# klindsay28/NK_ocn_tracer_jacobian_precond

Hardware: AMD Instinct MI355X
Metric: precond_solve_throughput_1deg_ocean_jacobian (higher is better)
Workload: dtype f64

## Files before the change

### include/nkp.h

```cpp
#ifndef NKP_H
#define NKP_H

#include <stdint.h>

#ifdef __cplusplus
extern "C" {
#endif

#define NKP_VERSION 1

typedef struct nkp_solver nkp_solver;

enum nkp_precond {
   NKP_PRECOND_NONE = 0,
   NKP_PRECOND_COLUMN_JACOBI = 1,
   NKP_PRECOND_MULTILEVEL = 3
};

enum nkp_krylov { NKP_KRYLOV_FGMRES = 0, NKP_KRYLOV_BICGSTAB = 1 };

enum {
   NKP_OK = 0,
   NKP_NOT_CONVERGED = 1,
   NKP_BREAKDOWN = 2,
   NKP_OK_BERR = 3,
   NKP_EINVAL = -1,
   NKP_ENOMEM = -2,
   NKP_EDEVICE = -3,
   NKP_ESINGULAR = -4,
   NKP_ECOMM = -5
};

typedef struct nkp_tuning {
   int struct_size;
   int ml_split;
   int ml_pocket;
   int ml_big_from;
   int ml_coarsest_rows;
   int ml_dense_max;
   double ml_theta;
   double ml_tau;
   int64_t ml_device_min;
   int ml_smooth_coarse;
   int ml_coarse_from;
   int ml_gamma_from, ml_gamma_to;
   int ml_f32;
   int ml_host_inverse;
   int ml_fused;
   int ml_fused_max_cols;
   int ml_wave_fused;
   int ml_coarsest_sweeps;
   int64_t ml_tail_rows;
   double ml_omega;
   int col_ldsres;
   int col_stream;
   int col_stream_min;
   int col_stream_gw;
   int col_wave_max;
   int col_w3;
   int col_group;
   int col_pipe_min;
   int col_ldsres_early;
   int col_ldsres_packed;
   int spmv_variant;
   int spmv_compress;
   int spmv_pipe_min;
   int spmv_run;
   int spmv_wgs;
   int rhs_batch;
   int precond_steps;
   int equil;
   int dist_overlap;
   int dist_ras;
   int force_dist;
   int setup_threads;
   int plan_times;
   int ml_drop_intertracer;
   int dist_one_reduce;
   int ml_huge_from;
   int col_ldsres_min;
   int col_sort_groups;
   int batch_spmv_rows;
   int dist_ras_rings;
   int ml_diag;
   int spmv_diag;
   int ml_lane_fused;
} nkp_tuning;

int nkp_default_tuning (nkp_tuning *t);

typedef struct nkp_options {
   int struct_size;
   int precond;
   int krylov;
   int restart;
   int max_iters;
   double rtol;
   double atol;
   int device;
   int verbose;
   int rank;
   int reorth;
   int ml_levels;
   int ml_smooth;
   int basis_f32;
   int precond_steps;
   int equil;
   int reserved[4];
   const int32_t *col_i;
   const int32_t *col_j;
   const int32_t *col_t;
   const nkp_tuning *tuning;
} nkp_options;

int nkp_default_options (nkp_options *opt);

int nkp_device_count (void);

int nkp_create (nkp_solver **out, const nkp_options *opt, int64_t n, int64_t nnz,
                const int32_t *rowptr, const int32_t *colind, const double *val,
                const int32_t *blk_start, int64_t nblk, int coupled_tracer_cnt);

int nkp_create64 (nkp_solver **out, const nkp_options *opt, int64_t n, const int64_t *rowptr ,
                  const int32_t *colind, const double *val, const int32_t *blk_start, int64_t nblk, int coupled_tracer_cnt);

int nkp_solve (nkp_solver *s, double *b_in_x_out, int nrhs, int64_t ldb,
               double *berr, int *iters, double *relres);

int nkp_solve_batch_device (nkp_solver *s, int nrhs, const void *d_B, void *d_X, int64_t ldb, double *berr, int *iters, double *relres);

int nkp_solve_device (nkp_solver *s, const void *d_b, void *d_x, int use_guess,
                      double *berr, int *iters, double *relres);

int nkp_spmv (nkp_solver *s, const double *x, double *y);
int nkp_spmv_device (nkp_solver *s, const void *d_x, void *d_y);

int nkp_precond_apply (nkp_solver *s, const double *r, double *z);

int nkp_multi_dot (nkp_solver *s, const double *V, int64_t ld, int k, const double *w, double *out);

int nkp_time_kernel (nkp_solver *s, int which, int arg, int reps, double *avg_ms);

int64_t nkp_get_int (nkp_solver *s, const char *key);

#define NKP_REFACTOR_REBUILD 1
int nkp_refactor (nkp_solver *s, const double *val, int flags);
int nkp_refactor_device (nkp_solver *s, const void *d_val, int flags);

int nkp_refactor_dist (nkp_solver *s, const double *val_loc, int flags);
int nkp_refactor_dist_device (nkp_solver *s, const void *d_val_loc, int flags);

int nkp_set_stream (nkp_solver *s, void *hip_stream);

void nkp_destroy (nkp_solver *s);

const char *nkp_last_error (void);


typedef struct nkp_comm_ops {
   void *ctx;
   int rank, nranks;
   int (*allreduce) (void *ctx, void *dev_buf, int count, int op, void *hip_stream);
   int (*alltoallv) (void *ctx, const void *dev_send, const int *send_counts, void *dev_recv, const int *recv_counts, void *hip_stream);
   int (*alltoallv_i32_host) (void *ctx, const int32_t *send, const int *send_counts, int32_t *recv, const int *recv_counts);
   int (*allgather_i64_host) (void *ctx, int64_t mine, int64_t *all );
} nkp_comm_ops;

int nkp_comm_unique_id (void *id128);
int nkp_comm_rccl_init (nkp_comm_ops *ops, const void *id128, int rank, int nranks);
void nkp_comm_rccl_free (nkp_comm_ops *ops);
int nkp_comm_file_init (nkp_comm_ops *ops, const char *dir, int rank, int nranks);
void nkp_comm_file_free (nkp_comm_ops *ops);

int nkp_create_dist (nkp_solver **out, const nkp_options *opt, int64_t n_global, int64_t fst_row,
                     int64_t m_loc, int64_t nnz_loc, const int32_t *rowptr_loc,
                     const int32_t *colind_glob, const double *val,
                     const int32_t *blk_start_loc, int64_t nblk_loc, int coupled_tracer_cnt,
                     const nkp_comm_ops *comm);

int nkp_cell_major_order (int64_t nblk, const int32_t *blk_start, int cnt, int32_t *perm, int32_t *blk_start_new,
                          int32_t *col_t, int32_t *col_src);
int nkp_permuted_rows (int64_t n, const int32_t *rowptr, const int32_t *colind, const double *val, const int32_t *perm,
                       const int32_t *inv, int64_t r0, int64_t r1, int32_t *rowptr_loc, int32_t *colind_loc, double *val_loc);

int nkp_clone (nkp_solver *src, nkp_solver **out);

int nkp_transpose (nkp_solver *s, nkp_solver **out);

int nkp_transpose_dist (nkp_solver *s, nkp_solver **out);

int nkp_value_gradient_device (nkp_solver *s, int nrhs, const void *d_lambda, const void *d_x, int64_t ld, double alpha, int accumulate, void *d_gval);
int nkp_value_gradient (nkp_solver *s, int nrhs, const double *lambda, const double *x, int64_t ld, double alpha, int accumulate, double *gval);

int nkp_values_product_device (nkp_solver *s, int nrhs, const void *d_val, const void *d_x, int64_t ldx, double alpha, int accumulate, void *d_y, int64_t ldy);
int nkp_values_product (nkp_solver *s, int nrhs, const double *val, const double *x, int64_t ldx, double alpha, int accumulate, double *y, int64_t ldy);

int nkp_solve_tangent_device (nkp_solver *s, int nrhs, const void *d_dval, const void *d_x, int64_t ldx, const void *d_db, void *d_dx, int64_t ld,
                              double *berr, int *iters, double *relres);

int nkp_set_device (int device);

int nkp_gather_root (nkp_solver *s, const double *x_loc, double *x_global);

typedef struct nkp_dist_plan nkp_dist_plan;
int nkp_dist_overlap_plan_host (nkp_dist_plan **out, const nkp_options *opt, int64_t n_global, int64_t fst_row, int64_t m_loc,
                                int64_t nnz_loc, const int32_t *rowptr_loc, const int32_t *colind_glob, const double *val,
                                const int32_t *blk_start_loc, int64_t nblk_loc, int coupled_tracer_cnt, const nkp_comm_ops *comm);
int64_t nkp_dist_plan_size (const nkp_dist_plan *p, const char *what);
int nkp_dist_plan_copy (const nkp_dist_plan *p, const char *what, void *dst);
void nkp_dist_plan_free (nkp_dist_plan *p);

int nkp_dist_plan_host (int64_t m_loc, int64_t nnz_loc, const int32_t *rowptr_loc, const int32_t *colind_glob,
                        int rank, int nranks, const int64_t *starts, int32_t *colind_ext, int32_t *halo_rows,
                        int64_t *n_halo, int32_t *need_counts);

int64_t nkp_ml_level_array (nkp_solver *s, int level, const char *what, void *dst, int64_t capacity_bytes);

int64_t nkp_matrix_array (nkp_solver *s, const char *what, void *dst, int64_t capacity_bytes);

int nkp_ml_plan_host (int64_t n, const int32_t *rowptr, const int32_t *colind, const double *val, const int32_t *blk_start,
                      int64_t nblk, const int32_t *col_i, const int32_t *col_j, int coupled_tracer_cnt, int max_levels,
                      int coarsest_rows, int64_t capacity, int *n_levels, int64_t *rows, int32_t *cmap, int32_t *col_of);

#ifdef __cplusplus
}
#endif
#endif
```

### nk_ocn_tracer_jacobian_precond_amd/csrc/blas1.hip

```cpp
#include "nkp_dev.h"

#include <stdint.h>

#define B1_THREADS 256

__device__ __forceinline__ double wave_sum (double v)
{
#pragma unroll
   for (int off = NKP_WAVE / 2; off > 0; off >>= 1) v += __shfl_down (v, off);
   return v;
}

__device__ __forceinline__ double block_sum (double v, double *sh )
{
   v = wave_sum (v);
   const int lane = threadIdx.x & (NKP_WAVE - 1), wv = threadIdx.x / NKP_WAVE;
   __syncthreads ();
   if (lane == 0) sh[wv] = v;
   __syncthreads ();
   double s = 0.0;
   if (threadIdx.x == 0) {
#pragma unroll
      for (int w = 0; w < B1_THREADS / NKP_WAVE; w++) s += sh[w];
   }
   return s;
}

static inline int red_grid (int64_t n)
{
   int64_t g = (n + 2 * B1_THREADS - 1) / (2 * B1_THREADS);
   if (g < 1) g = 1;
   if (g > NKP_RED_BLOCKS) g = NKP_RED_BLOCKS;
   return (int) g;
}

template <class VT, class VT2>
__device__ __forceinline__ void multi_dot_body (const VT *__restrict__ V, int64_t ld, int k, const double *__restrict__ w,
                                                int64_t n, double *__restrict__ partial, double *sh)
{
   const int chunk = blockIdx.y;
   const int j0 = chunk * NKP_DOT_CHUNK;
   const int kc = (k - j0) < NKP_DOT_CHUNK ? (k - j0) : NKP_DOT_CHUNK;
   const VT *Vc = V + (int64_t) j0 * ld;
   double acc[NKP_DOT_CHUNK];
#pragma unroll
   for (int c = 0; c < NKP_DOT_CHUNK; c++) acc[c] = 0.0;
   double accw = 0.0;
   const int64_t stride = (int64_t) gridDim.x * B1_THREADS * 2;
   for (int64_t i = ((int64_t) blockIdx.x * B1_THREADS + threadIdx.x) * 2; i < n; i += stride) {
      if (i + 1 < n) {
         const double2 w2 = *reinterpret_cast<const double2 *> (w + i);
         accw += w2.x * w2.x + w2.y * w2.y;
#pragma unroll
         for (int c = 0; c < NKP_DOT_CHUNK; c++)
            if (c < kc) {
               const VT2 v2 = *reinterpret_cast<const VT2 *> (Vc + (int64_t) c * ld + i);
               acc[c] += (double) v2.x * w2.x + (double) v2.y * w2.y;
            }
      } else {
         const double w1 = w[i];
         accw += w1 * w1;
#pragma unroll
         for (int c = 0; c < NKP_DOT_CHUNK; c++)
            if (c < kc) acc[c] += (double) Vc[(int64_t) c * ld + i] * w1;
      }
   }
   double *out = partial + ((int64_t) chunk * gridDim.x + blockIdx.x) * (NKP_DOT_CHUNK + 1);
#pragma unroll
   for (int c = 0; c < NKP_DOT_CHUNK; c++) {
      const double s = block_sum (acc[c], sh);
      if (threadIdx.x == 0) out[c] = s;
   }
   const double sw = block_sum (accw, sh);
   if (threadIdx.x == 0) out[NKP_DOT_CHUNK] = sw;
}

template <class VT, class VT2>
__global__ __launch_bounds__ (B1_THREADS)
void multi_dot_kernel (const VT *__restrict__ V, int64_t ld, int k, const double *__restrict__ w,
                       int64_t n, double *__restrict__ partial)
{
   __shared__ double sh[B1_THREADS / NKP_WAVE];
   multi_dot_body<VT, VT2> (V, ld, k, w, n, partial, sh);
}

__global__ __launch_bounds__ (B1_THREADS)
void multi_dot_group_kernel (GsGroup G, int64_t ld, int k, int64_t n)
{
   __shared__ double sh[B1_THREADS / NKP_WAVE];
   const int r = blockIdx.z;
   multi_dot_body<double, double2> (G.V[r], ld, k, G.w[r], n, G.partial[r], sh);
}

__device__ __forceinline__ void multi_dot_finish_body (const double *__restrict__ partial, int nblk, int k, double *__restrict__ out)
{
   const int j = blockIdx.x;
   const int chunk = (j < k) ? j / NKP_DOT_CHUNK : 0;
   const int c = (j < k) ? j % NKP_DOT_CHUNK : NKP_DOT_CHUNK;
   const double *p = partial + (int64_t) chunk * nblk * (NKP_DOT_CHUNK + 1) + c;
   double s = 0.0;
   for (int b = threadIdx.x; b < nblk; b += NKP_WAVE) s += p[(int64_t) b * (NKP_DOT_CHUNK + 1)];
   s = wave_sum (s);
   if (threadIdx.x == 0) out[j] = s;
}

__global__ __launch_bounds__ (NKP_WAVE)
void multi_dot_finish_kernel (const double *__restrict__ partial, int nblk, int k, double *__restrict__ out)
{
   multi_dot_finish_body (partial, nblk, k, out);
}

__global__ __launch_bounds__ (NKP_WAVE)
void multi_dot_finish_group_kernel (GsGroup G, int nblk, int k, double *__restrict__ msg)
{
   multi_dot_finish_body (G.partial[blockIdx.y], nblk, k, msg + (int64_t) blockIdx.y * (k + 1));
}

void launch_multi_dot (const void *V, int v_f32, int64_t ld, int k, const double *w, int64_t n, double *partial, double *out, hipStream_t st)
{
   const int g = red_grid (n);
   const int nchunk = k > 0 ? (k + NKP_DOT_CHUNK - 1) / NKP_DOT_CHUNK : 1;
   if (v_f32) hipLaunchKernelGGL ((multi_dot_kernel<float, float2>), dim3 (g, nchunk), dim3 (B1_THREADS), 0, st, (const float *) V, ld, k, w, n, partial);
   else hipLaunchKernelGGL ((multi_dot_kernel<double, double2>), dim3 (g, nchunk), dim3 (B1_THREADS), 0, st, (const double *) V, ld, k, w, n, partial);
   hipLaunchKernelGGL (multi_dot_finish_kernel, dim3 (k + 1), dim3 (NKP_WAVE), 0, st, partial, g, k, out);
}

void launch_multi_dot_group (int R, const GsGroup &G, int64_t ld, int k, int64_t n, double *msg, hipStream_t st)
{
   if (R <= 0) return;
   const int g = red_grid (n);
   const int nchunk = k > 0 ? (k + NKP_DOT_CHUNK - 1) / NKP_DOT_CHUNK : 1;
   hipLaunchKernelGGL (multi_dot_group_kernel, dim3 (g, nchunk, R), dim3 (B1_THREADS), 0, st, G, ld, k, n);
   hipLaunchKernelGGL (multi_dot_finish_group_kernel, dim3 (k + 1, R), dim3 (NKP_WAVE), 0, st, G, g, k, msg);
}

#define B1_MAX_K NKP_MAX_K
template <class VT, class VT2>
__device__ __forceinline__ void update_w_body (const VT *__restrict__ V, int64_t ld, int k, const double *__restrict__ h,
                                               double *__restrict__ w, int64_t n, double *__restrict__ partial, double sign, double *hs, double *sh)
{
   for (int j = threadIdx.x; j < k; j += B1_THREADS) hs[j] = sign * h[j];
   __syncthreads ();
   double nrm = 0.0;
   const int64_t stride = (int64_t) gridDim.x * B1_THREADS * 2;
   for (int64_t i = ((int64_t) blockIdx.x * B1_THREADS + threadIdx.x) * 2; i < n; i += stride) {
      if (i + 1 < n) {
         double2 a = *reinterpret_cast<const double2 *> (w + i);
         int j = 0;
         for (; j + 4 <= k; j += 4) {
            const VT2 v0 = *reinterpret_cast<const VT2 *> (V + (int64_t) (j + 0) * ld + i);
            const VT2 v1 = *reinterpret_cast<const VT2 *> (V + (int64_t) (j + 1) * ld + i);
            const VT2 v2 = *reinterpret_cast<const VT2 *> (V + (int64_t) (j + 2) * ld + i);
            const VT2 v3 = *reinterpret_cast<const VT2 *> (V + (int64_t) (j + 3) * ld + i);
            a.x += hs[j] * v0.x; a.y += hs[j] * v0.y;
            a.x += hs[j + 1] * v1.x; a.y += hs[j + 1] * v1.y;
            a.x += hs[j + 2] * v2.x; a.y += hs[j + 2] * v2.y;
            a.x += hs[j + 3] * v3.x; a.y += hs[j + 3] * v3.y;
         }
         for (; j < k; j++) {
            const VT2 v0 = *reinterpret_cast<const VT2 *> (V + (int64_t) j * ld + i);
            a.x += hs[j] * v0.x; a.y += hs[j] * v0.y;
         }
         *reinterpret_cast<double2 *> (w + i) = a;
         nrm += a.x * a.x + a.y * a.y;
      } else {
         double a = w[i];
         for (int j = 0; j < k; j++) a += hs[j] * V[(int64_t) j * ld + i];
         w[i] = a;
         nrm += a * a;
      }
   }
   if (partial) {
      const double s = block_sum (nrm, sh);
      if (threadIdx.x == 0) partial[blockIdx.x] = s;
   }
}

template <class VT, class VT2>
__global__ __launch_bounds__ (B1_THREADS)
void update_w_kernel (const VT *__restrict__ V, int64_t ld, int k, const double *__restrict__ h,
                      double *__restrict__ w, int64_t n, double *__restrict__ partial, double sign)
{
   __shared__ double hs[B1_MAX_K];
   __shared__ double sh[B1_THREADS / NKP_WAVE];
   update_w_body<VT, VT2> (V, ld, k, h, w, n, partial, sign, hs, sh);
}

__global__ __launch_bounds__ (B1_THREADS)
void update_w_group_kernel (GsGroup G, int64_t ld, int k, const double *__restrict__ msg, int64_t n)
{
   __shared__ double hs[B1_MAX_K];
   __shared__ double sh[B1_THREADS / NKP_WAVE];
   const int r = blockIdx.y;
   update_w_body<double, double2> (G.V[r], ld, k, msg + (int64_t) r * (k + 1), G.w[r], n, G.partial[r], -1.0, hs, sh);
}

__device__ __forceinline__ void sum_partials_body (const double *__restrict__ partial, int nblk, double *__restrict__ out)
{
   double s = 0.0;
   for (int b = threadIdx.x; b < nblk; b += NKP_WAVE) s += partial[b];
   s = wave_sum (s);
   if (threadIdx.x == 0) out[0] = s;
}

__global__ __launch_bounds__ (NKP_WAVE)
void sum_partials_kernel (const double *__restrict__ partial, int nblk, double *__restrict__ out)
{
   sum_partials_body (partial, nblk, out);
}

__global__ __launch_bounds__ (NKP_WAVE)
void sum_partials_group_kernel (GsGroup G, int nblk, double *__restrict__ out)
{
   sum_partials_body (G.partial[blockIdx.x], nblk, out + blockIdx.x);
}

void launch_update_w (const void *V, int v_f32, int64_t ld, int k, const double *h, double *w, int64_t n, double *partial, double *out_nrm2, hipStream_t st)
{
   const int g = red_grid (n);
   if (v_f32) hipLaunchKernelGGL ((update_w_kernel<float, float2>), dim3 (g), dim3 (B1_THREADS), 0, st, (const float *) V, ld, k, h, w, n, partial, -1.0);
   else hipLaunchKernelGGL ((update_w_kernel<double, double2>), dim3 (g), dim3 (B1_THREADS), 0, st, (const double *) V, ld, k, h, w, n, partial, -1.0);
   hipLaunchKernelGGL (sum_partials_kernel, dim3 (1), dim3 (NKP_WAVE), 0, st, partial, g, out_nrm2);
}

void launch_update_w_group (int R, const GsGroup &G, int64_t ld, int k, const double *msg, int64_t n, double *nrm2, hipStream_t st)
{
   if (R <= 0) return;
   const int g = red_grid (n);
   hipLaunchKernelGGL (update_w_group_kernel, dim3 (g, R), dim3 (B1_THREADS), 0, st, G, ld, k, msg, n);
   hipLaunchKernelGGL (sum_partials_group_kernel, dim3 (R), dim3 (NKP_WAVE), 0, st, G, g, nrm2);
}

void launch_axpy_multi (const double *Z, int64_t ld, int k, const double *c, double *x, int64_t n, hipStream_t st)
{
   const int g = red_grid (n);
   hipLaunchKernelGGL ((update_w_kernel<double, double2>), dim3 (g), dim3 (B1_THREADS), 0, st, Z, ld, k, c, x, n, (double *) nullptr, 1.0);
}

__device__ __forceinline__ void scale_to_body (const double *__restrict__ x, const double *__restrict__ alpha, double *__restrict__ y, float *__restrict__ yf, int64_t n)
{
   const double a = alpha[0];
   const int64_t stride = (int64_t) gridDim.x * B1_THREADS * 2;
   for (int64_t i = ((int64_t) blockIdx.x * B1_THREADS + threadIdx.x) * 2; i < n; i += stride) {
      if (i + 1 < n) {
         double2 v = *reinterpret_cast<const double2 *> (x + i);
         v.x *= a; v.y *= a;
         *reinterpret_cast<double2 *> (y + i) = v;
         if (yf) *reinterpret_cast<float2 *> (yf + i) = make_float2 ((float) v.x, (float) v.y);
      } else {
         y[i] = a * x[i];
         if (yf) yf[i] = (float) (a * x[i]);
      }
   }
}

__global__ __launch_bounds__ (B1_THREADS)
void scale_to_kernel (const double *__restrict__ x, const double *__restrict__ alpha, double *__restrict__ y, float *__restrict__ yf, int64_t n)
{
   scale_to_body (x, alpha, y, yf, n);
}

__global__ __launch_bounds__ (B1_THREADS)
void scale_to_group_kernel (GsGroup G, const double *__restrict__ inv, int64_t n)
{
   const int r = blockIdx.y;
   scale_to_body (G.w[r], inv + r, G.vnext[r], nullptr, n);
}

void launch_scale_to (const double *x, const double *alpha_dev, double *y, float *yf, int64_t n, hipStream_t st)
{
   hipLaunchKernelGGL (scale_to_kernel, dim3 (red_grid (n)), dim3 (B1_THREADS), 0, st, x, alpha_dev, y, yf, n);
}

void launch_scale_to_group (int R, const GsGroup &G, const double *inv, int64_t n, hipStream_t st)
{
   if (R > 0) hipLaunchKernelGGL (scale_to_group_kernel, dim3 (red_grid (n), R), dim3 (B1_THREADS), 0, st, G, inv, n);
}

__global__ __launch_bounds__ (B1_THREADS)
void axpby_kernel (double a, const double *__restrict__ x, double b, double *__restrict__ y, int64_t n)
{
   const int64_t stride = (int64_t) gridDim.x * B1_THREADS;
   for (int64_t i = (int64_t) blockIdx.x * B1_THREADS + threadIdx.x; i < n; i += stride)
      y[i] = (b == 0.0 ? 0.0 : b * y[i]) + (x ? a * x[i] : a);
}

void launch_axpby (double a, const double *x, double b, double *y, int64_t n, hipStream_t st)
{
   hipLaunchKernelGGL (axpby_kernel, dim3 (red_grid (n) * 2), dim3 (B1_THREADS), 0, st, a, x, b, y, n);
}

__global__ __launch_bounds__ (B1_THREADS)
void vmul_kernel (const double *x, const double *__restrict__ w, double *y, int64_t n)
{
   const int64_t stride = (int64_t) gridDim.x * B1_THREADS;
   for (int64_t i = (int64_t) blockIdx.x * B1_THREADS + threadIdx.x; i < n; i += stride) y[i] = x[i] * w[i];
}

void launch_vmul (const double *x, const double *w, double *y, int64_t n, hipStream_t st)
{
   hipLaunchKernelGGL (vmul_kernel, dim3 (red_grid (n) * 2), dim3 (B1_THREADS), 0, st, x, w, y, n);
}

void launch_copy (const double *x, double *y, int64_t n, hipStream_t st)
{
   (void) hipMemcpyAsync (y, x, (size_t) n * sizeof (double), hipMemcpyDeviceToDevice, st);
}

__global__ __launch_bounds__ (B1_THREADS)
void zero_kernel (double *__restrict__ y, int64_t n)
{
   const int64_t stride = (int64_t) gridDim.x * B1_THREADS * 2;
   for (int64_t i = ((int64_t) blockIdx.x * B1_THREADS + threadIdx.x) * 2; i < n; i += stride) {
      if (i + 1 < n) *reinterpret_cast<double2 *> (y + i) = make_double2 (0.0, 0.0);
      else y[i] = 0.0;
   }
}

void launch_fill (double *y, double v, int64_t n, hipStream_t st)
{
   if (n <= 0) return;
   if (v == 0.0) {
      if ((reinterpret_cast<uintptr_t> (y) & 15) == 0) hipLaunchKernelGGL (zero_kernel, dim3 (red_grid (n) * 2), dim3 (B1_THREADS), 0, st, y, n);
      else (void) hipMemsetAsync (y, 0, (size_t) n * sizeof (double), st);
   } else
      launch_axpby (v, nullptr, 0.0, y, n, st);
}

__global__ __launch_bounds__ (B1_THREADS)
void dot_kernel (const double *__restrict__ x, const double *__restrict__ y, int64_t n, double *__restrict__ partial)
{
   __shared__ double sh[B1_THREADS / NKP_WAVE];
   double acc = 0.0;
   const int64_t stride = (int64_t) gridDim.x * B1_THREADS * 2;
   for (int64_t i = ((int64_t) blockIdx.x * B1_THREADS + threadIdx.x) * 2; i < n; i += stride) {
      if (i + 1 < n) {
         const double2 a = *reinterpret_cast<const double2 *> (x + i);
         const double2 b = *reinterpret_cast<const double2 *> (y + i);
         acc += a.x * b.x + a.y * b.y;
      } else
         acc += x[i] * y[i];
   }
   const double s = block_sum (acc, sh);
   if (threadIdx.x == 0) partial[blockIdx.x] = s;
}

void launch_dot (const double *x, const double *y, int64_t n, double *partial, double *out, hipStream_t st)
{
   const int g = red_grid (n);
   hipLaunchKernelGGL (dot_kernel, dim3 (g), dim3 (B1_THREADS), 0, st, x, y, n, partial);
   hipLaunchKernelGGL (sum_partials_kernel, dim3 (1), dim3 (NKP_WAVE), 0, st, partial, g, out);
}

__global__ __launch_bounds__ (B1_THREADS)
void berr_kernel (const double *__restrict__ r, const double *__restrict__ den, int64_t n, double *__restrict__ partial)
{
   __shared__ double sh[B1_THREADS / NKP_WAVE];
   double m = 0.0;
   const int64_t stride = (int64_t) gridDim.x * B1_THREADS;
   for (int64_t i = (int64_t) blockIdx.x * B1_THREADS + threadIdx.x; i < n; i += stride) {
      const double a = fabs (r[i]), d = den[i];
      const double q = (d > 0.0) ? a / d : (a > 0.0 ? 1.0e300 : 0.0);
      m = q > m ? q : m;
   }
   for (int off = NKP_WAVE / 2; off > 0; off >>= 1) {
      const double o = __shfl_down (m, off);
      m = o > m ? o : m;
   }
   const int lane = threadIdx.x & (NKP_WAVE - 1), wv = threadIdx.x / NKP_WAVE;
   if (lane == 0) sh[wv] = m;
   __syncthreads ();
   if (threadIdx.x == 0) {
      for (int w = 1; w < B1_THREADS / NKP_WAVE; w++) m = sh[w] > m ? sh[w] : m;
      partial[blockIdx.x] = m;
   }
}

__global__ __launch_bounds__ (NKP_WAVE)
void max_partials_kernel (const double *__restrict__ partial, int nblk, double *__restrict__ out)
{
   double m = 0.0;
   for (int b = threadIdx.x; b < nblk; b += NKP_WAVE) m = partial[b] > m ? partial[b] : m;
   for (int off = NKP_WAVE / 2; off > 0; off >>= 1) {
      const double o = __shfl_down (m, off);
      m = o > m ? o : m;
   }
   if (threadIdx.x == 0) out[0] = m;
}

void launch_berr (const double *r, const double *den, int64_t n, double *partial, double *out, hipStream_t st)
{
   const int g = red_grid (n);
   hipLaunchKernelGGL (berr_kernel, dim3 (g), dim3 (B1_THREADS), 0, st, r, den, n, partial);
   hipLaunchKernelGGL (max_partials_kernel, dim3 (1), dim3 (NKP_WAVE), 0, st, partial, g, out);
}

__device__ __forceinline__ void finish_column_body (double *__restrict__ h, const double *__restrict__ h2, int k,
                                                    const double *__restrict__ nrm2, double *__restrict__ inv)
{
   if (h2)
      for (int j = threadIdx.x; j < k; j += NKP_WAVE) h[j] += h2[j];
   if (threadIdx.x == 0) {
      const double t = sqrt (nrm2[0]);
      h[k] = t;
      inv[0] = (t > 0.0) ? 1.0 / t : 0.0;
   }
}

__global__ __launch_bounds__ (NKP_WAVE)
void finish_column_kernel (double *__restrict__ h, const double *__restrict__ h2, int k,
                           const double *__restrict__ nrm2, double *__restrict__ inv)
{
   finish_column_body (h, h2, k, nrm2, inv);
}

__device__ __forceinline__ void finish_column_pythagoras_body (double *__restrict__ h, int k, double *__restrict__ inv)
{
   double s = 0.0;
   for (int j = threadIdx.x; j < k; j += NKP_WAVE) s += h[j] * h[j];
   for (int off = NKP_WAVE / 2; off > 0; off >>= 1) s += __shfl_down (s, off);
   if (threadIdx.x == 0) {
      const double ww = h[k];
      double t2 = ww - s;
      const bool weak = !(t2 >= 1e-8 * ww);
      if (!(t2 > 0.0)) t2 = 0.0;
      const double t = sqrt (t2);
      h[k] = weak ? -t : t;
      inv[0] = (t > 0.0) ? 1.0 / t : 0.0;
   }
}

__global__ __launch_bounds__ (NKP_WAVE)
void finish_column_pythagoras_kernel (double *__restrict__ h, int k, double *__restrict__ inv)
{
   finish_column_pythagoras_body (h, k, inv);
}

__global__ __launch_bounds__ (NKP_WAVE)
void finish_column_group_kernel (double *__restrict__ msg, const double *__restrict__ msg2, int k, const double *__restrict__ nrm2, double *__restrict__ inv)
{
   const int64_t r = blockIdx.x;
   if (nrm2) finish_column_body (msg + r * (k + 1), msg2 ? msg2 + r * (k + 1) : nullptr, k, nrm2 + r, inv + r);
   else finish_column_pythagoras_body (msg + r * (k + 1), k, inv + r);
}

void launch_finish_column_group (int R, double *msg, const double *msg2, int k, const double *nrm2, double *inv, hipStream_t st)
{
   if (R > 0) hipLaunchKernelGGL (finish_column_group_kernel, dim3 (R), dim3 (NKP_WAVE), 0, st, msg, msg2, k, nrm2, inv);
}

void launch_finish_column_pythagoras (double *h, int k, double *inv, hipStream_t st)
{
   hipLaunchKernelGGL (finish_column_pythagoras_kernel, dim3 (1), dim3 (NKP_WAVE), 0, st, h, k, inv);
}

void launch_finish_column (double *h, const double *h2, int k, const double *nrm2, double *inv, hipStream_t st)
{
   hipLaunchKernelGGL (finish_column_kernel, dim3 (1), dim3 (NKP_WAVE), 0, st, h, h2, k, nrm2, inv);
}

__global__ __launch_bounds__ (B1_THREADS)
void restrict_sum_kernel (const int *__restrict__ rptr, const int *__restrict__ ridx, const double *__restrict__ fine,
                          double *__restrict__ coarse, int64_t nc)
{
   const int64_t stride = (int64_t) gridDim.x * B1_THREADS;
   for (int64_t I = (int64_t) blockIdx.x * B1_THREADS + threadIdx.x; I < nc; I += stride) {
      double acc = 0.0;
      for (int q = rptr[I]; q < rptr[I + 1]; q++) acc += fine[ridx[q]];
      coarse[I] = acc;
   }
}

void launch_restrict_sum (const int *rptr, const int *ridx, const double *fine, double *coarse, int64_t nc, hipStream_t st)
{
   if (nc <= 0) return;
   hipLaunchKernelGGL (restrict_sum_kernel, dim3 (red_grid (nc) * 2), dim3 (B1_THREADS), 0, st, rptr, ridx, fine, coarse, nc);
}

__global__ __launch_bounds__ (B1_THREADS)
void prolong_add_kernel (const int *__restrict__ cmap, const double *__restrict__ coarse, double *__restrict__ fine, int64_t nf, double omega)
{
   const int64_t stride = (int64_t) gridDim.x * B1_THREADS;
   for (int64_t i = (int64_t) blockIdx.x * B1_THREADS + threadIdx.x; i < nf; i += stride) fine[i] += omega * coarse[cmap[i]];
}

void launch_prolong_add (const int *cmap, const double *coarse, double *fine, int64_t nf, double omega, hipStream_t st)
{
   if (nf <= 0) return;
   hipLaunchKernelGGL (prolong_add_kernel, dim3 (red_grid (nf) * 2), dim3 (B1_THREADS), 0, st, cmap, coarse, fine, nf, omega);
}

__global__ __launch_bounds__ (B1_THREADS)
void gather_kernel (const int *__restrict__ perm, const double *__restrict__ in, double *__restrict__ out, int64_t n, int scatter)
{
   const int64_t stride = (int64_t) gridDim.x * B1_THREADS;
   for (int64_t i = (int64_t) blockIdx.x * B1_THREADS + threadIdx.x; i < n; i += stride) {
      if (scatter) out[perm[i]] = in[i];
      else out[i] = in[perm[i]];
   }
}

void launch_gather (const int *perm, const double *in, double *out, int64_t n, hipStream_t st)
{
   if (n <= 0) return;
   hipLaunchKernelGGL (gather_kernel, dim3 (red_grid (n) * 2), dim3 (B1_THREADS), 0, st, perm, in, out, n, 0);
}

void launch_scatter (const int *perm, const double *in, double *out, int64_t n, hipStream_t st)
{
   if (n <= 0) return;
   hipLaunchKernelGGL (gather_kernel, dim3 (red_grid (n) * 2), dim3 (B1_THREADS), 0, st, perm, in, out, n, 1);
}

__global__ __launch_bounds__ (B1_THREADS)
void dense_matvec_kernel (const double *__restrict__ M, const double *__restrict__ x, double *__restrict__ y, int n)
{
   const int row = (int) ((blockIdx.x * B1_THREADS + threadIdx.x) / NKP_WAVE);
   const int lane = threadIdx.x & (NKP_WAVE - 1);
   if (row >= n) return;
   const double *m = M + (int64_t) row * n;
   double acc = 0.0;
   for (int c = lane; c < n; c += NKP_WAVE) acc += m[c] * x[c];
   acc = wave_sum (acc);
   if (lane == 0) y[row] = acc;
}

void launch_dense_matvec (const double *Minv, const double *x, double *y, int n, hipStream_t st)
{
   if (n <= 0) return;
   const int waves_per_block = B1_THREADS / NKP_WAVE;
   hipLaunchKernelGGL (dense_matvec_kernel, dim3 ((n + waves_per_block - 1) / waves_per_block), dim3 (B1_THREADS), 0, st, Minv, x, y, n);
}
```

### nk_ocn_tracer_jacobian_precond_amd/csrc/create.hip

```cpp
#include "solver_impl.h"

#include <limits.h>
#include <math.h>
#include <stdlib.h>
#include <string.h>
#include <time.h>

#include <algorithm>
#include <thread>
#include <vector>

void drop_intertracer (int64_t n, int tracer_cnt, const int32_t *rowptr, const int32_t *colind, const double *val,
                       std::vector<int32_t> &f_rowptr, std::vector<int32_t> &f_colind, std::vector<double> &f_val)
{
   const int64_t tsl = n / tracer_cnt;
   f_rowptr.assign ((size_t) n + 1, 0);
   for (int64_t i = 0; i < n; i++) {
      for (int32_t e = rowptr[i]; e < rowptr[i + 1]; e++)
         if (colind[e] / tsl == i / tsl) { f_colind.push_back (colind[e]); f_val.push_back (val[e]); }
      f_rowptr[(size_t) i + 1] = (int32_t) f_colind.size ();
   }
}

static int alloc_work_vectors (nkp_solver *s, bool member = false)
{
   const size_t ld = (size_t) s->ld, m = (size_t) s->m, nscal = 3 * (m + 2) + 16 + 8;
   const struct { double **p; size_t count; } vec[] = {
      { &s->V, ld * (m + 1) }, { &s->vcur, ld }, { &s->Z, ld * m }, { &s->w, ld }, { &s->r, ld }, { &s->x, ld }, { &s->b, ld }, { &s->t1, ld }, { &s->t2, ld },
      { &s->p1, s->precond_steps > 1 ? ld : 0 }, { &s->p2, s->precond_steps > 1 && !member ? ld : 0 }, { &s->eqtmp, s->equil && !member ? ld : 0 },
      { &s->partial, ((m + 1 + NKP_DOT_CHUNK) / NKP_DOT_CHUNK + 1) * NKP_RED_BLOCKS * (NKP_DOT_CHUNK + 1) }, { &s->dscal, nscal } };
   int rc = NKP_OK;
   for (const auto &v : vec)
      if (v.count && (rc = dev_alloc (s, v.p, v.count))) return rc;
   if ((rc = dev_alloc (s, &s->dint, 8))) return rc;
   HIPCHK (hipHostMalloc ((void **) &s->hpin, (m + 16) * sizeof (double), hipHostMallocDefault));
   HIPCHK (hipMemset (s->dscal, 0, nscal * sizeof (double)));
   return NKP_OK;
}

static void build_matrix_diagonals (nkp_solver *s, const int32_t *blk_start, int64_t nblk)
{
   const int64_t n = s->n;
   if (s->tune.spmv_diag <= 0 || !blk_start || nblk <= 0 || nblk >= INT_MAX || n <= 0 || blk_start[0] != 0 || blk_start[nblk] != n) return;
   int max_len = 0;
   for (int64_t c = 0; c < nblk; c++) {
      const int len = blk_start[c + 1] - blk_start[c];
      if (len <= 0) return;
      max_len = std::max (max_len, len);
   }
   void *d_blk = nullptr;
   const size_t bytes = ((size_t) nblk + 1) * sizeof (int);
   if (hipMalloc (&d_blk, bytes) != hipSuccess || hipMemcpy (d_blk, blk_start, bytes, hipMemcpyHostToDevice) != hipSuccess) {
      if (d_blk) (void) hipFree (d_blk);
      (void) hipGetLastError ();
      return;
   }
   int color_tile[3];
   (void) diag_build (s->A, blk_start, (const int *) d_blk, (int) nblk, (int) nblk, max_len, s->tune.spmv_diag, color_tile, &s->device_bytes, s->stream);
   (void) hipFree (d_blk);
}

static int check_arguments (const nkp_options *opt_in, int64_t n, int64_t nnz, const int32_t *rowptr, const int32_t *colind, const double *val,
                            nkp_options &opt, nkp_tuning &tune)
{
   if (opt_in) {
      if (opt_in->struct_size != (int) sizeof (nkp_options)) return fail (NKP_EINVAL, "nkp_create: nkp_options.struct_size mismatch (%d != %zu)", opt_in->struct_size, sizeof (nkp_options));
      opt = *opt_in;
   } else
      nkp_default_options (&opt);
   if (n < 0 || nnz < 0 || !rowptr || (nnz > 0 && (!colind || !val))) return fail (NKP_EINVAL, "nkp_create: bad matrix arguments");
   if (n >= 2147483647LL || nnz >= 2147483647LL) return fail (NKP_EINVAL, "nkp_create: n/nnz exceed the int32 index schema");
   if (rowptr[0] != 0 || rowptr[n] != nnz) return fail (NKP_EINVAL, "nkp_create: rowptr[0]=%d rowptr[n]=%d inconsistent with nnz=%lld", rowptr[0], rowptr[n], (long long) nnz);
   if (opt.restart < 1) opt.restart = 1;
   if (opt.restart > NKP_MAX_K - 2) opt.restart = NKP_MAX_K - 2;
   if (opt.precond != NKP_PRECOND_NONE && opt.precond != NKP_PRECOND_COLUMN_JACOBI && opt.precond != NKP_PRECOND_MULTILEVEL)
      return fail (NKP_EINVAL, "nkp_create: unknown preconditioner %d", opt.precond);
   { const int trc = resolve_tuning (&opt, &tune); if (trc) return trc; }
   opt.tuning = nullptr;
   return NKP_OK;
}

static int check_rows (const nkp_options &opt, int64_t n, const int32_t *rowptr, const int32_t *colind, const double *val)
{
   struct Bad { int64_t row = -1; int kind = 0; int col = 0; };
   const int nt = (n >= 200000) ? (int) std::min (16u, std::max (1u, std::thread::hardware_concurrency ())) : 1;
   std::vector<Bad> bad ((size_t) nt);
   auto check = [&] (int t) {
      const int64_t r0 = n * t / nt, r1 = n * (t + 1) / nt;
      for (int64_t r = r0; r < r1 && bad[(size_t) t].row < 0; r++) {
         Bad b;
         if (rowptr[r + 1] < rowptr[r]) b.kind = 1;
         else {
            double diag = 0.0;
            for (int e = rowptr[r]; e < rowptr[r + 1] && !b.kind; e++) {
               if (colind[e] < 0 || colind[e] >= n) { b.kind = 2; b.col = colind[e]; }
               else if (opt.precond == NKP_PRECOND_MULTILEVEL && e > rowptr[r] && colind[e] <= colind[e - 1]) b.kind = 4;
               else if (colind[e] == r) diag += val[e];
            }
            if (!b.kind && opt.precond != NKP_PRECOND_NONE && !(diag != 0.0)) b.kind = 3;
         }
         if (b.kind) { b.row = r; bad[(size_t) t] = b; }
      }
   };
   if (nt == 1) check (0);
   else {
      std::vector<std::thread> pool;
      for (int t = 0; t < nt; t++) pool.emplace_back (check, t);
      for (std::thread &th : pool) th.join ();
   }
   for (const Bad &b : bad) {
      if (b.row < 0) continue;
      if (b.kind == 1) return fail (NKP_EINVAL, "nkp_create: rowptr decreases at row %lld", (long long) b.row);
      if (b.kind == 2) return fail (NKP_EINVAL, "nkp_create: column index %d out of range in row %lld", b.col, (long long) b.row);
      if (b.kind == 3) return fail (NKP_ESINGULAR, "nkp_create: row %lld has no (or a zero) diagonal entry; the water-column preconditioners need one (the reference only reports this: src/matrix.c:3692-3727)", (long long) b.row);
      return fail (NKP_EINVAL, "nkp_create: row %lld is not sorted by column (the multilevel setup needs the sorted rows gen_A writes)", (long long) b.row);
   }
   return NKP_OK;
}

static int check_blocks (const nkp_options &opt, int64_t n, const int32_t *&blk_start, int64_t &nblk, std::vector<int> &blk_default)
{
   if (opt.precond == NKP_PRECOND_NONE) return NKP_OK;
   if (!blk_start) {
      for (int64_t r = 0; r < n; r += NKP_WAVE) blk_default.push_back ((int) r);
      blk_default.push_back ((int) n);
      blk_start = blk_default.data ();
      nblk = (int64_t) blk_default.size () - 1;
   }
   if (nblk < 0 || blk_start[0] != 0 || blk_start[nblk] != n) return fail (NKP_EINVAL, "nkp_create: blk_start must run from 0 to n");
   for (int64_t b = 0; b < nblk; b++) {
      int len = blk_start[b + 1] - blk_start[b];
      if (len <= 0) return fail (NKP_EINVAL, "nkp_create: empty or descending block %lld", (long long) b);
      if (len > 2 * NKP_WAVE) return fail (NKP_EINVAL, "nkp_create: block %lld has %d rows; this build supports water columns of at most %d levels", (long long) b, len, 2 * NKP_WAVE);
   }
   return NKP_OK;
}

static int new_solver_on_device (const nkp_options &opt, const nkp_tuning &tune, nkp_solver **out)
{
   int ndev = 0;
   if (hipGetDeviceCount (&ndev) != hipSuccess || ndev == 0) return fail (NKP_EDEVICE, "nkp_create: no HIP device available (this library has no CPU fallback)");
   nkp_solver *s = new nkp_solver;
   s->opt = opt;
   s->tune = tune;
   s->A.tune = &s->tune;
   s->B.tune = &s->tune;
   if (opt.device >= 0) {
      if (opt.device >= ndev) { delete s; return fail (NKP_EDEVICE, "nkp_create: device %d of %d does not exist", opt.device, ndev); }
      if (hipSetDevice (opt.device) != hipSuccess) { delete s; return fail (NKP_EDEVICE, "hipSetDevice(%d) failed", opt.device); }
   }
   (void) hipGetDevice (&s->device);
   {
      hipDeviceProp_t prop;
      if (hipGetDeviceProperties (&prop, s->device) == hipSuccess && strncmp (prop.gcnArchName, "gfx950", 6) != 0)
         msg (s, 1, "warning: device %d is %s, kernels are built and tuned for gfx950\n", s->device, prop.gcnArchName);
   }
   *out = s;
   return NKP_OK;
}

#define TRY(x) do { rc = (x); if (rc != NKP_OK) { solver_free (s); return rc; } } while (0)
#define TRYHIP(call) do { hipError_t e_ = (call); if (e_ != hipSuccess) { rc = fail (NKP_EDEVICE, "%s failed: %s", #call, hipGetErrorString (e_)); solver_free (s); return rc; } } while (0)

static int configure (nkp_solver *s, int64_t n)
{
   const nkp_options &opt = s->opt;
   const nkp_tuning &tune = s->tune;
   int rc = NKP_OK;
   TRYHIP (hipStreamCreateWithFlags (&s->stream, hipStreamNonBlocking));
   s->own_stream = true;
   s->n = n;
   s->ld = (n + 63) & ~(int64_t) 63;
   if (s->ld == 0) s->ld = 64;
   s->m = opt.restart;
   s->precond_steps = 1;
   if (opt.precond_steps > 0) s->precond_steps = opt.precond_steps;
   if (tune.precond_steps > 0) s->precond_steps = tune.precond_steps;
   s->steps_now = s->precond_steps;
   s->equil = opt.equil > 0;
   if (tune.equil >= 0 && opt.equil == 0) s->equil = tune.equil != 0;
   if (opt.krylov != NKP_KRYLOV_FGMRES) s->equil = false;
   return rc;
}

static void segmented_rowblocks (nkp_solver *s, const SpmvMatrixHost &M, int **rb, int *nrb)
{
   const int64_t n = s->n;
   int64_t lo = 0, hi = 0, run0 = 0;
// ... 104 lines not shown
   TRYHIP (hipMemcpy (s->B.blk_start, blk_start, ((size_t) nblk + 1) * sizeof (int), hipMemcpyHostToDevice));
   TRYHIP (hipMemsetAsync (s->dint, 0, 8 * sizeof (int), s->stream));
   launch_colblock_measure (s->A, s->B, s->dint, s->stream);
   int meas[3] = { 0, 0, 0 };
   TRYHIP (hipMemcpyAsync (meas, s->dint, sizeof meas, hipMemcpyDeviceToHost, s->stream));
   TRYHIP (hipStreamSynchronize (s->stream));
   if (meas[1] > 0) {
      rc = fail (NKP_ESINGULAR, "nkp_create: %d rows have no (or a zero) diagonal entry; the column-block preconditioner needs one (the reference only reports this: src/matrix.c:3692-3727)", meas[1]);
      solver_free (s);
      return rc;
   }
   s->B.max_len = meas[2];
   s->B.P = meas[0] <= 1 ? 1 : meas[0] <= 2 ? 2 : 4;
   TRY (dev_alloc (s, &s->B.fac, (size_t) (2 * s->B.P + 1) * (size_t) n));
   TRYHIP (hipMemsetAsync (s->dint, 0, 8 * sizeof (int), s->stream));
   launch_colblock_factor (s->A, s->B, s->dint, s->stream);
   int st2[2] = { 0, 0 };
   TRYHIP (hipMemcpyAsync (st2, s->dint, sizeof st2, hipMemcpyDeviceToHost, s->stream));
   TRYHIP (hipStreamSynchronize (s->stream));
   if (st2[0] != 0) {
      rc = fail (NKP_ESINGULAR, "nkp_create: zero pivot at row %d while factoring its water-column block", st2[0] - 1);
      solver_free (s);
      return rc;
   }
   s->B.dropped = st2[1];
   {
      const int ranges[2] = { 0, (int) nblk };
      int grp_first[2];
      const int lrc = colblock_build_lane_layout (s->B, blk_start, ranges, 1, grp_first, &s->device_bytes, s->stream);
      if (lrc != 0) {
         rc = fail (NKP_EDEVICE, "nkp_create: lane layout of the column blocks failed (HIP error %d)", lrc);
         solver_free (s);
         return rc;
      }
   }
   msg (s, 1, "column blocks: %lld blocks, longest %d rows, in-block half bandwidth %d stored as %d%s\n", (long long) nblk,
        s->B.max_len, meas[0], s->B.P, s->B.dropped ? " (entries beyond the band dropped)" : "");
   return NKP_OK;
}

int create_impl (nkp_solver **out, const nkp_options *opt_in, int64_t n, int64_t nnz,
                 const int32_t *rowptr, const int32_t *colind, const double *val,
                 const int32_t *blk_start, int64_t nblk, int coupled_tracer_cnt, const SpmvMatrixHost *spmv_mat,
                 const PrecondMatrixHost *pm)
{
   if (!out) return fail (NKP_EINVAL, "nkp_create: out is NULL");
   *out = nullptr;
   nkp_options opt;
   nkp_tuning tune;
   std::vector<int> blk_default;
   int rc;
   if ((rc = check_arguments (opt_in, n, nnz, rowptr, colind, val, opt, tune))) return rc;
   if ((rc = check_rows (opt, n, rowptr, colind, val))) return rc;
   if ((rc = check_blocks (opt, n, blk_start, nblk, blk_default))) return rc;

   nkp_solver *s = nullptr;
   if ((rc = new_solver_on_device (opt, tune, &s))) return rc;
   struct timespec ts0_;
   clock_gettime (CLOCK_MONOTONIC, &ts0_);
   auto since0 = [&] () { struct timespec t; clock_gettime (CLOCK_MONOTONIC, &t); return (double) (t.tv_sec - ts0_.tv_sec) + 1e-9 * (double) (t.tv_nsec - ts0_.tv_nsec); };
   if ((rc = configure (s, n))) return rc;

   const SpmvMatrixHost own = { nnz, n, rowptr, colind, val };
   const SpmvMatrixHost &M = spmv_mat ? *spmv_mat : own;
   if ((rc = upload_matrix (s, M, spmv_mat != nullptr))) return rc;
   if (!spmv_mat && blk_default.empty ()) build_matrix_diagonals (s, blk_start, nblk);
   if (s->equil && (rc = upload_row_scales (s, M))) return rc;

   const double t_matrix = since0 ();
   s->vf32 = opt.basis_f32 != 0;
   TRY (alloc_work_vectors (s));

   const double t_work = since0 ();
   if (opt.precond != NKP_PRECOND_NONE && !pm) {
      s->h_blk.assign (blk_start, blk_start + nblk + 1);
      s->tracer_cnt = coupled_tracer_cnt;
      if (blk_default.empty ()) {
         if (opt.col_i) s->h_col_i.assign (opt.col_i, opt.col_i + nblk);
         if (opt.col_j) s->h_col_j.assign (opt.col_j, opt.col_j + nblk);
         if (opt.col_t) s->h_col_t.assign (opt.col_t, opt.col_t + nblk);
      }
   }
   if (opt.precond == NKP_PRECOND_MULTILEVEL &&
       (rc = build_hierarchy (s, n, rowptr, colind, val, blk_start, nblk, blk_default.empty (), coupled_tracer_cnt, !spmv_mat, pm))) return rc;
   if (opt.precond == NKP_PRECOND_COLUMN_JACOBI && (rc = factor_columns (s, blk_start, nblk))) return rc;
   TRYHIP (hipStreamSynchronize (s->stream));
   TRYHIP (hipGetLastError ());
   msg (s, 1, "nkp_create: n = %lld, nnz = %lld, %d SpMV row blocks, %.1f MB on device %d; %.2f s matrix upload + row blocks, %.2f s work vectors, %.2f s preconditioner\n",
        (long long) n, (long long) M.nnz, s->A.nrowblk, (double) s->device_bytes / 1.0e6, s->device, t_matrix, t_work - t_matrix, since0 () - t_work);
   s->create_seconds = since0 ();
   *out = s;
   return NKP_OK;
}

extern "C" int nkp_create (nkp_solver **out, const nkp_options *opt, int64_t n, int64_t nnz,
                           const int32_t *rowptr, const int32_t *colind, const double *val,
                           const int32_t *blk_start, int64_t nblk, int coupled_tracer_cnt)
{
   return create_impl (out, opt, n, nnz, rowptr, colind, val, blk_start, nblk, coupled_tracer_cnt, nullptr);
}

extern "C" int nkp_create64 (nkp_solver **out, const nkp_options *opt, int64_t n, const int64_t *rowptr, const int32_t *colind, const double *val,
                             const int32_t *blk_start, int64_t nblk, int coupled_tracer_cnt)
{
   if (!out) return fail (NKP_EINVAL, "nkp_create64: out is NULL");
   *out = nullptr;
   if (n < 0 || !rowptr) return fail (NKP_EINVAL, "nkp_create64: bad matrix arguments");
   if (n >= 2147483647LL || rowptr[n] >= 2147483647LL || rowptr[n] < 0)
      return fail (NKP_EINVAL, "nkp_create64: %lld rows / %lld entries: one GPU stores entry offsets in 32 bits (at most 2^31 - 1 rows and entries); "
                   "row-partition the system with nkp_create_dist, where the limit applies per rank", (long long) n, (long long) rowptr[n]);
   std::vector<int32_t> rp ((size_t) n + 1);
   for (int64_t r = 0; r <= n; r++) {
      if (rowptr[r] < 0 || rowptr[r] > rowptr[n]) return fail (NKP_EINVAL, "nkp_create64: rowptr[%lld] = %lld out of range", (long long) r, (long long) rowptr[r]);
      rp[(size_t) r] = (int32_t) rowptr[r];
   }
   return create_impl (out, opt, n, rowptr[n], rp.data (), colind, val, blk_start, nblk, coupled_tracer_cnt, nullptr);
}

int clone_impl (nkp_solver *src, nkp_solver **out, bool member)
{
   if (!src || !out) return fail (NKP_EINVAL, "nkp_clone: NULL argument");
   *out = nullptr;
   if (src->dist.on && !member) return fail (NKP_EINVAL, "nkp_clone: not available for the row-distributed flavour");
   if (src->borrowed) return fail (NKP_EINVAL, "nkp_clone: clone the original solver, not a clone");
   if (src->trans_of && !member) return fail (NKP_EINVAL, "nkp_clone: not available on a transposed solver (its owner may free it at a refactor)");
   HIPCHK (hipSetDevice (src->device));
   nkp_solver *s = new (std::nothrow) nkp_solver (*src);
   if (!s) return fail (NKP_ENOMEM, "nkp_clone: out of host memory");
   s->borrowed = true;
   s->rf = nullptr;
   s->shared->clones++;
   s->stagnated = false;
   s->batch_members.clear ();
   s->bvin = s->bz = s->bw = nullptr;
   s->batch_K = 0;
   s->dist.bxe = s->dist.bsend = s->dist.gmsg = s->dist.ghpin = s->dist.bras_send = s->dist.bras_recv = nullptr;
   s->dist.bK = s->dist.agreed_K = 0;
   s->dplan = nullptr;
   s->trans = s->trans_of = nullptr;
   s->trans_src = nullptr;
   s->trans_val = nullptr;
   s->trans_map_bytes = 0;
   s->trans_ship = nullptr;
   s->trans_send = s->trans_recv = nullptr;
   s->vg = decltype (s->vg) ();
   s->vp = decltype (s->vp) ();
   s->A.tune = &s->tune;
   s->B.tune = &s->tune;
   s->ml.tune = &s->tune;
   for (MlLevel &L : s->ml.lev) L.L.tune = L.B.tune = &s->tune;
   s->stream = nullptr;
   s->own_stream = false;
   s->device_bytes = 0;
   s->V = s->vcur = s->Z = s->w = s->r = s->x = s->b = s->t1 = s->t2 = s->p1 = s->p2 = s->eqtmp = s->partial = s->dscal = s->hpin = nullptr;
   s->dint = nullptr;
   for (MlLevel &L : s->ml.lev) L.x = L.x2 = L.b = L.r = nullptr;
   int rc = NKP_OK;
   TRYHIP (hipStreamCreateWithFlags (&s->stream, hipStreamNonBlocking));
   s->own_stream = true;
   TRY (alloc_work_vectors (s, member));
   for (MlLevel &L : s->ml.lev) {
      TRY (dev_alloc (s, &L.x, (size_t) L.n));
      TRY (dev_alloc (s, &L.x2, (size_t) L.n));
      TRY (dev_alloc (s, &L.b, (size_t) L.n));
      TRY (dev_alloc (s, &L.r, (size_t) L.n));
      TRYHIP (hipMemset (L.x, 0, (size_t) (L.n ? L.n : 1) * sizeof (double)));
      TRYHIP (hipMemset (L.x2, 0, (size_t) (L.n ? L.n : 1) * sizeof (double)));
      TRYHIP (hipMemset (L.b, 0, (size_t) (L.n ? L.n : 1) * sizeof (double)));
      TRYHIP (hipMemset (L.r, 0, (size_t) (L.n ? L.n : 1) * sizeof (double)));
   }
   *out = s;
   return NKP_OK;
}

#undef TRY
#undef TRYHIP

extern "C" int nkp_clone (nkp_solver *src, nkp_solver **out) { return clone_impl (src, out, false); }
```

### nk_ocn_tracer_jacobian_precond_amd/csrc/inspect.hip

```cpp
#include "solver_impl.h"

#include <string.h>

#include <vector>

extern "C" int64_t nkp_ml_level_array (nkp_solver *s, int level, const char *what, void *dst, int64_t capacity_bytes)
{
   if (!s || !what || s->opt.precond != NKP_PRECOND_MULTILEVEL || level < 0 || level >= (int) s->ml.lev.size ()) return fail (NKP_EINVAL, "nkp_ml_level_array: bad argument");
   const MlLevel &V = s->ml.lev[(size_t) level];
   const bool last = level == (int) s->ml.lev.size () - 1;
   const void *src = nullptr;
   int64_t count = 0;
   size_t elem = 4;
   bool host = false;
   int col_kernel[11];
   if (!strcmp (what, "rowptr")) { src = V.L.rowptr; count = V.n + 1; }
   else if (!strcmp (what, "colind")) { src = V.L.colind; count = V.L.nnz; }
   else if (!strcmp (what, "valf")) { src = V.L.valf; count = V.L.valf ? V.L.nnz : 0; }
   else if (!strcmp (what, "val")) { src = V.L.val; count = V.L.val ? V.L.nnz : 0; elem = 8; }
   else if (!strcmp (what, "dg_ptr")) { src = V.L.dg_ptr; count = src ? V.L.dg_ncol + 1 : 0; }
   else if (!strcmp (what, "dg_key")) { src = V.L.dg_key; count = src ? (int64_t) V.L.dg_nkey : 0; }
   else if (!strcmp (what, "dg_voff")) { src = V.L.dg_voff; count = src ? V.L.dg_ncol : 0; elem = 8; }
   else if (!strcmp (what, "dg_val")) { src = V.L.dg_val; count = src ? V.L.dg_nval : 0; }
   else if (!strcmp (what, "dg_gptr")) { src = V.L.dg_gptr; count = src ? V.L.dg_ncol + 1 : 0; }
   else if (!strcmp (what, "dg_grp")) { src = V.L.dg_grp; count = src ? 2 * (int64_t) V.L.dg_ngrp : 0; }
   else if (!strcmp (what, "cmap")) { src = V.cmap; count = V.cmap ? V.n : 0; }
   else if (!strcmp (what, "rptr")) { src = V.rptr; count = V.rptr ? V.nc + 1 : 0; }
   else if (!strcmp (what, "ridx")) { src = V.ridx; count = V.ridx ? V.n : 0; }
   else if (!strcmp (what, "blk_start")) { src = V.B.blk_start; count = V.B.blk_start ? V.B.nblk + 1 : 0; }
   else if (!strcmp (what, "fac")) { src = V.B.fac; count = V.B.fac ? (int64_t) (2 * V.B.P + 1) * V.n : 0; elem = 8; }
   else if (!strcmp (what, "perm0")) { src = level == 0 ? s->ml.perm0 : nullptr; count = src ? V.n : 0; }
   else if (!strcmp (what, "coarse_inv")) { src = last ? s->ml.coarse_inv : nullptr; count = src ? V.n * V.n : 0; elem = 8; }
   else if (!strcmp (what, "color_blk")) { src = V.B.blk_start ? V.color_blk : nullptr; count = src ? 3 : 0; host = true; }
   else if (!strcmp (what, "col_kernel")) {
      const ColBlocksDev &B = V.B;
      const int v[11] = { V.wave_columns ? 1 : 0, V.wave_fused ? 1 : 0, B.stream ? 1 : 0, B.ldsres, B.gw, B.P, B.dropped, B.max_len, B.gs_ok, B.ngrp, B.lds_doubles };
      memcpy (col_kernel, v, sizeof v);
      src = B.blk_start ? col_kernel : nullptr; count = src ? 11 : 0; host = true;
   }
   else if (!strcmp (what, "wave_diag")) { src = &V.wave_diag; count = 1; host = true; }
   else if (!strcmp (what, "lane_diag")) { src = &V.lane_diag; count = 1; host = true; }
   else if (!strcmp (what, "grp_tile")) { src = V.B.grp_tile; count = src ? (int64_t) V.B.ngrp * V.B.gw : 0; }
   else return fail (NKP_EINVAL, "nkp_ml_level_array: unknown array '%s'", what);
   if (!dst) return count;
   if (count * (int64_t) elem > capacity_bytes) return fail (NKP_EINVAL, "nkp_ml_level_array: buffer too small");
   if (host) {
      if (count) memcpy (dst, src, (size_t) count * elem);
      return count;
   }
   HIPCHK (hipSetDevice (s->device));
   HIPCHK (hipStreamSynchronize (s->stream));
   if (count) HIPCHK (hipMemcpy (dst, src, (size_t) count * elem, hipMemcpyDeviceToHost));
   return count;
}

extern "C" int64_t nkp_matrix_array (nkp_solver *s, const char *what, void *dst, int64_t capacity_bytes)
{
   if (!s || !what) return fail (NKP_EINVAL, "nkp_matrix_array: bad argument");
   const CsrDev &A = s->A;
   const bool have = A.dg_vald != nullptr;
   const void *src = nullptr;
   int64_t count = 0;
   size_t elem = 4;
   if (!strcmp (what, "dg_ptr")) { src = A.dg_ptr; count = have ? A.dg_ncol + 1 : 0; }
   else if (!strcmp (what, "dg_key")) { src = A.dg_key; count = have ? (int64_t) A.dg_nkey : 0; }
   else if (!strcmp (what, "dg_voff")) { src = A.dg_voff; count = have ? A.dg_ncol : 0; elem = 8; }
   else if (!strcmp (what, "dg_val")) { src = A.dg_vald; count = have ? A.dg_nval : 0; elem = 8; }
   else if (!strcmp (what, "dg_gptr")) { src = A.dg_gptr; count = have ? A.dg_ncol + 1 : 0; }
   else if (!strcmp (what, "dg_grp")) { src = A.dg_grp; count = have ? 2 * (int64_t) A.dg_ngrp : 0; }
   else if (!strcmp (what, "rowptr")) { src = A.rowptr; count = src ? A.n + 1 : 0; }
   else if (!strcmp (what, "colind")) { src = A.colind; count = src ? A.nnz : 0; }
   else if (!strcmp (what, "val")) { src = A.val; count = src ? A.nnz : 0; elem = 8; }
   else if (!strcmp (what, "fac")) { src = s->opt.precond == NKP_PRECOND_COLUMN_JACOBI ? s->B.fac : nullptr; count = src ? (int64_t) (2 * s->B.P + 1) * s->B.n : 0; elem = 8; }
   else return fail (NKP_EINVAL, "nkp_matrix_array: unknown array '%s'", what);
   if (!dst) return count;
   if (count * (int64_t) elem > capacity_bytes) return fail (NKP_EINVAL, "nkp_matrix_array: buffer too small");
   HIPCHK (hipSetDevice (s->device));
   HIPCHK (hipStreamSynchronize (s->stream));
   if (count) HIPCHK (hipMemcpy (dst, src, (size_t) count * elem, hipMemcpyDeviceToHost));
   return count;
}

extern "C" int nkp_spmv_device (nkp_solver *s, const void *d_x, void *d_y)
{
   if (!s || !d_x || !d_y) return fail (NKP_EINVAL, "nkp_spmv_device: NULL argument");
   HIPCHK (hipSetDevice (s->device));
   spmv_op (s, (const double *) d_x, (double *) d_y, nullptr, 0);
   HIPCHK (hipStreamSynchronize (s->stream));
   HIPCHK (hipGetLastError ());
   return NKP_OK;
}

extern "C" int nkp_spmv (nkp_solver *s, const double *x, double *y)
{
   if (!s || !x || !y) return fail (NKP_EINVAL, "nkp_spmv: NULL argument");
   HIPCHK (hipSetDevice (s->device));
   const size_t bytes = (size_t) s->n * sizeof (double);
   HIPCHK (hipMemcpyAsync (s->t1, x, bytes, hipMemcpyHostToDevice, s->stream));
   spmv_op (s, s->t1, s->t2, nullptr, 0);
   HIPCHK (hipMemcpyAsync (y, s->t2, bytes, hipMemcpyDeviceToHost, s->stream));
   HIPCHK (hipStreamSynchronize (s->stream));
   HIPCHK (hipGetLastError ());
   return NKP_OK;
}

extern "C" int nkp_precond_apply (nkp_solver *s, const double *r, double *z)
{
   if (!s || !r || !z) return fail (NKP_EINVAL, "nkp_precond_apply: NULL argument");
   if (s->shared->broken) return refactor_broken (s);
   HIPCHK (hipSetDevice (s->device));
   const size_t bytes = (size_t) s->n * sizeof (double);
   HIPCHK (hipMemcpyAsync (s->t1, r, bytes, hipMemcpyHostToDevice, s->stream));
   apply_precond_once (s, s->t1, s->t2);
   HIPCHK (hipMemcpyAsync (z, s->t2, bytes, hipMemcpyDeviceToHost, s->stream));
   HIPCHK (hipStreamSynchronize (s->stream));
   HIPCHK (hipGetLastError ());
   return NKP_OK;
}

extern "C" int nkp_multi_dot (nkp_solver *s, const double *V, int64_t ld, int k, const double *w, double *out)
{
   if (!s || !V || !w || !out || k < 0 || k > s->m + 1 || ld < s->n) return fail (NKP_EINVAL, "nkp_multi_dot: bad argument (k must be <= restart+1)");
   HIPCHK (hipSetDevice (s->device));
   std::vector<float> vf;
   for (int j = 0; j < k; j++) {
      if (s->vf32) {
         vf.assign (V + (int64_t) j * ld, V + (int64_t) j * ld + s->n);
         HIPCHK (hipMemcpyAsync ((float *) s->V + (int64_t) j * s->ld, vf.data (), (size_t) s->n * sizeof (float), hipMemcpyHostToDevice, s->stream));
         HIPCHK (hipStreamSynchronize (s->stream));
      } else
         HIPCHK (hipMemcpyAsync (s->V + (int64_t) j * s->ld, V + (int64_t) j * ld, (size_t) s->n * sizeof (double), hipMemcpyHostToDevice, s->stream));
   }
   HIPCHK (hipMemcpyAsync (s->w, w, (size_t) s->n * sizeof (double), hipMemcpyHostToDevice, s->stream));
   launch_multi_dot (s->V, s->vf32, s->ld, k, s->w, s->n, s->partial, s->h_dev (), s->stream);
   allreduce_dev (s, s->h_dev (), k + 1, 0);
   HIPCHK (hipMemcpyAsync (out, s->h_dev (), (size_t) (k + 1) * sizeof (double), hipMemcpyDeviceToHost, s->stream));
   HIPCHK (hipStreamSynchronize (s->stream));
   HIPCHK (hipGetLastError ());
   return NKP_OK;
}

extern "C" int nkp_time_kernel (nkp_solver *s, int which, int arg, int reps, double *avg_ms)
{
   if (!s || !avg_ms || reps < 1) return fail (NKP_EINVAL, "nkp_time_kernel: bad argument");
   if (which == 8 && !s->A.dg_vald) return fail (NKP_EINVAL, "nkp_time_kernel: the matrix has no per-column diagonals (tuning spmv_diag)");
   HIPCHK (hipSetDevice (s->device));
   if (which == 5) {
      const int prc = valgrad_time_prepare (s, arg);
      if (prc) return prc;
   }
   if (which == 6 || which == 7) {
      const int prc = valprod_time_prepare (s, arg, which);
      if (prc) return prc;
   }
   hipEvent_t e0, e1;
   HIPCHK (hipEventCreate (&e0));
   HIPCHK (hipEventCreate (&e1));
   launch_fill (s->t1, 1.0, s->n, s->stream);
   if (which == 2) {
      if (arg < 0 || arg >= s->m) return fail (NKP_EINVAL, "nkp_time_kernel: restart position out of range");
      for (int j = 0; j <= arg + 1; j++) {
         launch_fill (s->t2, 1.0 / (1.0 + j), s->n, s->stream);
         s->hpin[0] = 1.0;
         HIPCHK (hipMemcpyAsync (s->misc_dev () + 1, s->hpin, sizeof (double), hipMemcpyHostToDevice, s->stream));
         if (s->vf32) launch_scale_to (s->t2, s->misc_dev () + 1, s->vcur, (float *) s->V + (int64_t) j * s->ld, s->n, s->stream);
         else launch_scale_to (s->t2, s->misc_dev () + 1, s->V + (int64_t) j * s->ld, nullptr, s->n, s->stream);
         HIPCHK (hipStreamSynchronize (s->stream));
      }
   }
   for (int pass = 0; pass < 2; pass++) {
      const int cnt = pass == 0 ? (reps < 3 ? reps : 3) : reps;
      HIPCHK (hipEventRecord (e0, s->stream));
      for (int i = 0; i < cnt; i++) {
         if (which == 0 && s->A.dg_vald) launch_csr_spmv (s->A, s->t1, s->t2, nullptr, 0, s->stream);
         else if (which == 0) spmv_op (s, s->t1, s->t2, nullptr, 0);
         else if (which == 8) launch_diag_spmv (s->A, s->t1, s->t2, nullptr, 0, s->stream);
         else if (which == 1) apply_precond_once (s, s->t1, s->t2);
         else if (which == 2) arnoldi_step_device (s, arg);
         else if (which == 5) valgrad_time_launch (s, arg);
         else if (which == 6) valprod_time_launch (s, arg);
         else if (which == 7) valprod_time_composition (s, arg);
         else if (s->opt.precond == NKP_PRECOND_MULTILEVEL) ml_time_piece (s->ml, which - 3, s->stream);
      }
      HIPCHK (hipEventRecord (e1, s->stream));
      HIPCHK (hipEventSynchronize (e1));
      float ms = 0.f;
      HIPCHK (hipEventElapsedTime (&ms, e0, e1));
      *avg_ms = (double) ms / cnt;
   }
   (void) hipEventDestroy (e0);
   (void) hipEventDestroy (e1);
   HIPCHK (hipGetLastError ());
   return NKP_OK;
}
```

### nk_ocn_tracer_jacobian_precond_amd/csrc/krylov.hip

```cpp
#include "solver_impl.h"

#include <math.h>

void apply_precond_once (nkp_solver *s, const double *rin, double *zout)
{
   if (s->opt.precond == NKP_PRECOND_NONE) launch_copy (rin, zout, s->n, s->stream);
   else if (s->opt.precond == NKP_PRECOND_MULTILEVEL && s->dist.ras) {
      if (s->dist.ras_sep) {
         if (s->dist.ras_nsend) launch_gather (s->dist.ras_send_idx, rin, s->dist.ras_sendbuf, s->dist.ras_nsend, s->stream);
         alltoallv_dev (s, s->dist.ras_sendbuf, s->dist.ras_send_counts.data (), s->dist.rext + s->n, s->dist.ras_recv_counts.data (), s->stream);
         launch_copy (rin, s->dist.rext, s->n, s->stream);
      } else {
         if (s->dist.nsend) launch_gather (s->dist.send_idx, rin, s->dist.sendbuf, s->dist.nsend, s->stream);
         alltoallv_dev (s, s->dist.sendbuf, s->dist.send_counts.data (), s->dist.xe + s->n, s->dist.recv_counts.data (), s->stream);
         launch_copy (rin, s->dist.rext, s->n, s->stream);
         if (s->dist.n_sel) launch_gather (s->dist.sel_idx, s->dist.xe + s->n, s->dist.rext + s->n, s->dist.n_sel, s->stream);
      }
      ml_apply (s->ml, s->dist.rext, s->dist.zext, s->stream);
      launch_copy (s->dist.zext, zout, s->n, s->stream);
   } else if (s->opt.precond == NKP_PRECOND_MULTILEVEL) ml_apply (s->ml, rin, zout, s->stream);
   else launch_colblock_apply_lanes (s->B, 0, s->B.ngrp, rin, zout, 0, s->stream);
}

void apply_precond (nkp_solver *s, const double *rin, double *zout)
{
   apply_precond_once (s, rin, zout);
   for (int k = 1; k < s->steps_now && s->p1 && s->p2; k++) {
      spmv_op (s, zout, s->p1, rin, 1);
      apply_precond_once (s, s->p1, s->p2);
      launch_axpby (1.0, s->p2, 1.0, zout, s->n, s->stream);
   }
}

void spmv_op (nkp_solver *s, const double *x, double *y, const double *b, int mode)
{
   const double *xin = x;
   if (s->dist.on) {
      launch_copy (x, s->dist.xe, s->n, s->stream);
      if (s->dist.nsend) launch_gather (s->dist.send_idx, x, s->dist.sendbuf, s->dist.nsend, s->stream);
      xin = s->dist.xe;
      if (s->dist.overlap) {
         (void) hipEventRecord (s->dist.ev_packed, s->stream);
         (void) hipStreamWaitEvent (s->dist.comm_stream, s->dist.ev_packed, 0);
         alltoallv_dev (s, s->dist.sendbuf, s->dist.send_counts.data (), s->dist.xe + s->n, s->dist.recv_counts.data (), s->dist.comm_stream);
         (void) hipEventRecord (s->dist.ev_halo, s->dist.comm_stream);
         launch_csr_spmv_range (s->A, s->dist.seg_rb[1], s->dist.seg_rb[2], xin, y, b, mode, s->stream);
         (void) hipStreamWaitEvent (s->stream, s->dist.ev_halo, 0);
         launch_csr_spmv_range (s->A, s->dist.seg_rb[0], s->dist.seg_rb[1], xin, y, b, mode, s->stream);
         launch_csr_spmv_range (s->A, s->dist.seg_rb[2], s->dist.seg_rb[3], xin, y, b, mode, s->stream);
         return;
      }
      alltoallv_dev (s, s->dist.sendbuf, s->dist.send_counts.data (), s->dist.xe + s->n, s->dist.recv_counts.data (), s->stream);
   }
   if (mode == 2) launch_csr_abs_spmv (s->A, xin, b, y, s->stream);
   else if (s->A.dg_vald) launch_diag_spmv (s->A, xin, y, b, mode, s->stream);
   else launch_csr_spmv (s->A, xin, y, b, mode, s->stream);
}

static int dot_host (nkp_solver *s, const double *x, const double *y, double *out)
{
   launch_dot (x, y, s->n, s->partial, s->misc_dev () + 2, s->stream);
   allreduce_dev (s, s->misc_dev () + 2, 1, 0);
   HIPCHK (hipMemcpyAsync (s->hpin, s->misc_dev () + 2, sizeof (double), hipMemcpyDeviceToHost, s->stream));
   HIPCHK (hipStreamSynchronize (s->stream));
   if (s->comm_failed) return fail (NKP_ECOMM, "nkp_solve: a collective of the distributed solve failed");
   *out = s->hpin[0];
   return NKP_OK;
}

void arnoldi_apply (nkp_solver *s, int j)
{
   const int64_t ld = s->ld;
   double *zj = s->Z + (int64_t) j * ld;
   const double *vj = s->vf32 ? s->vcur : s->V + (int64_t) j * ld;
   if (s->equil) {
      launch_vmul (vj, s->rinv, s->eqtmp, s->n, s->stream);
      apply_precond (s, s->eqtmp, zj);
      spmv_op (s, zj, s->w, nullptr, 0);
      launch_vmul (s->w, s->rscale, s->w, s->n, s->stream);
   } else {
      apply_precond (s, vj, zj);
      spmv_op (s, zj, s->w, nullptr, 0);
   }
}

void arnoldi_orthogonalise (nkp_solver *s, int j)
{
   const int64_t ld = s->ld;
   launch_multi_dot (s->V, s->vf32, ld, j + 1, s->w, s->n, s->partial, s->h_dev (), s->stream);
   allreduce_dev (s, s->h_dev (), j + 2, 0);
   launch_update_w (s->V, s->vf32, ld, j + 1, s->h_dev (), s->w, s->n, s->partial, s->misc_dev (), s->stream);
   if (s->opt.reorth) {
      launch_multi_dot (s->V, s->vf32, ld, j + 1, s->w, s->n, s->partial, s->h2_dev (), s->stream);
      allreduce_dev (s, s->h2_dev (), j + 2, 0);
      launch_update_w (s->V, s->vf32, ld, j + 1, s->h2_dev (), s->w, s->n, s->partial, s->misc_dev (), s->stream);
      allreduce_dev (s, s->misc_dev (), 1, 0);
      launch_finish_column (s->h_dev (), s->h2_dev (), j + 1, s->misc_dev (), s->misc_dev () + 1, s->stream);
   } else if (s->dist.on && s->tune.dist_one_reduce) {
      launch_finish_column_pythagoras (s->h_dev (), j + 1, s->misc_dev () + 1, s->stream);
   } else {
      allreduce_dev (s, s->misc_dev (), 1, 0);
      launch_finish_column (s->h_dev (), nullptr, j + 1, s->misc_dev (), s->misc_dev () + 1, s->stream);
   }
   if (s->vf32) launch_scale_to (s->w, s->misc_dev () + 1, s->vcur, (float *) s->V + (int64_t) (j + 1) * ld, s->n, s->stream);
   else launch_scale_to (s->w, s->misc_dev () + 1, s->V + (int64_t) (j + 1) * ld, nullptr, s->n, s->stream);
}

void arnoldi_step_device (nkp_solver *s, int j)
{
   arnoldi_apply (s, j);
   arnoldi_orthogonalise (s, j);
}

int fg_begin (nkp_solver *s, FgmresState &F)
{
   fg_init (F, s->m);
   double bnorm2 = 0.0;
   int rc = dot_host (s, s->b, s->b, &bnorm2);
   if (rc) return rc;
   F.bnorm = sqrt (bnorm2);
   s->stagnated = false;
   s->steps_now = s->precond_steps;
   if (!(F.bnorm > 0.0)) {
      launch_fill (s->x, 0.0, s->n, s->stream);
      F.finished = true;
      F.status = NKP_OK;
      F.relres = 0.0;
      return NKP_OK;
   }
   F.target = fmax (s->opt.rtol * F.bnorm, s->opt.atol);
   return NKP_OK;
}

int fg_restart (nkp_solver *s, FgmresState &F)
{
   hipStream_t st = s->stream;
   const int64_t n = s->n;
   int rc;
   spmv_op (s, s->x, s->r, s->b, 1);
   double r2 = 0.0;
   if ((rc = dot_host (s, s->r, s->r, &r2))) return rc;
   const double beta = sqrt (r2);
   const int todo = fg_restart_verdict (F, beta, s->opt.max_iters, s->steps_now);
   msg (s, 2, "fgmres: its = %d, true relres = %.3e\n", F.its, F.relres);
   if (s->comm_failed) return fail (NKP_ECOMM, "nkp_solve: a collective of the distributed solve failed");
   if (todo & FG_LOWER_STEPS) {
      msg (s, 1, "fgmres: no progress over a restart cycle with %d preconditioner cycles per iteration; continuing with one\n", s->steps_now);
      s->steps_now = 1;
   }
   if (todo & FG_STAGNATED) s->stagnated = true;
   if (todo & FG_STOP) return NKP_OK;
   if (s->equil) {
      launch_vmul (s->r, s->rscale, s->r, n, st);
      double q2 = 0.0;
      if ((rc = dot_host (s, s->r, s->r, &q2))) return rc;
      F.beta_it = sqrt (q2);
      if (!(F.beta_it > 0.0)) { F.status = NKP_BREAKDOWN; F.finished = true; return NKP_OK; }
      F.target_it = F.target * (F.beta_it / beta);
   }
   s->hpin[0] = 1.0 / F.beta_it;
   HIPCHK (hipMemcpyAsync (s->misc_dev () + 1, s->hpin, sizeof (double), hipMemcpyHostToDevice, st));
   if (s->vf32) launch_scale_to (s->r, s->misc_dev () + 1, s->vcur, (float *) s->V, n, st);
   else launch_scale_to (s->r, s->misc_dev () + 1, s->V, nullptr, n, st);
   HIPCHK (hipStreamSynchronize (st));
   fg_start_cycle (F);
   return NKP_OK;
}

bool fg_post_step (nkp_solver *s, FgmresState &F)
{
   const bool ends = fg_column_step (F, s->hpin, s->opt.max_iters);
   if (!F.breakdown_in_cycle) msg (s, 3, "fgmres: its = %d, est relres = %.3e\n", F.its, F.est / F.bnorm);
   return ends;
}

int fg_end_cycle (nkp_solver *s, FgmresState &F)
{
   const int k = F.j;
   hipStream_t st = s->stream;
   fg_back_substitute (F);
   for (int i = 0; i < k; i++) s->hpin[i] = F.y[i];
   HIPCHK (hipMemcpyAsync (s->y_dev (), s->hpin, (size_t) k * sizeof (double), hipMemcpyHostToDevice, st));
   launch_axpy_multi (s->Z, s->ld, k, s->y_dev (), s->x, s->n, st);
   HIPCHK (hipStreamSynchronize (st));
   if (F.breakdown_in_cycle) {
      int rc;
      double r2 = 0.0;
      spmv_op (s, s->x, s->r, s->b, 1);
      if ((rc = dot_host (s, s->r, s->r, &r2))) return rc;
      F.relres = sqrt (r2) / F.bnorm;
      F.status = sqrt (r2) <= F.target ? NKP_OK : NKP_BREAKDOWN;
      F.finished = true;
   }
   return NKP_OK;
}

static int fgmres (nkp_solver *s, int *iters_out, double *relres_out)
{
   FgmresState F;
   int rc = fg_begin (s, F);
   if (rc) return rc;
   while (!F.finished) {
      if ((rc = fg_restart (s, F))) return rc;
      if (F.finished) break;
      for (;;) {
         arnoldi_step_device (s, F.j);
         HIPCHK (hipMemcpyAsync (s->hpin, s->h_dev (), (size_t) (F.j + 2) * sizeof (double), hipMemcpyDeviceToHost, s->stream));
         HIPCHK (hipStreamSynchronize (s->stream));
         if (s->comm_failed) return fail (NKP_ECOMM, "nkp_solve: a collective of the distributed solve failed (Arnoldi step %d)", F.its + 1);
         if (fg_post_step (s, F)) break;
      }
      if ((rc = fg_end_cycle (s, F))) return rc;
   }
   HIPCHK (hipGetLastError ());
   *iters_out = F.its;
   *relres_out = F.relres;
   return F.status;
}

static int bicgstab (nkp_solver *s, int *iters_out, double *relres_out)
{
   const int64_t n = s->n, ld = s->ld;
   hipStream_t st = s->stream;
   if (s->m < 2) return fail (NKP_EINVAL, "bicgstab needs restart >= 2 (it borrows the Krylov basis storage)");
   double *r = s->r, *r0 = s->V, *p = s->V + ld, *v = s->V + 2 * ld;
   double *ph = s->Z, *sh = s->Z + ld, *t = s->t2, *sv = s->t1;
   int rc;
   double bnorm2, rho = 1.0, alpha = 1.0, omega = 1.0, tmp;
   if ((rc = dot_host (s, s->b, s->b, &bnorm2))) return rc;
   const double bnorm = sqrt (bnorm2);
   if (!(bnorm > 0.0)) { launch_fill (s->x, 0.0, n, st); *iters_out = 0; *relres_out = 0.0; return NKP_OK; }
   const double target = fmax (s->opt.rtol * bnorm, s->opt.atol);
   spmv_op (s, s->x, r, s->b, 1);
   launch_copy (r, r0, n, st);
   launch_fill (p, 0.0, n, st);
   launch_fill (v, 0.0, n, st);
   int its = 0, status = NKP_NOT_CONVERGED;
   double rn2;
   if ((rc = dot_host (s, r, r, &rn2))) return rc;
   double relres = sqrt (rn2) / bnorm;
   while (its < s->opt.max_iters) {
      if (sqrt (rn2) <= target) { status = NKP_OK; break; }
      double rho_new;
      if ((rc = dot_host (s, r0, r, &rho_new))) return rc;
      if (rho_new == 0.0 || !(rho_new == rho_new)) { status = NKP_BREAKDOWN; break; }
      const double beta = (rho_new / rho) * (alpha / omega);
      launch_axpby (-omega, v, 1.0, p, n, st);
      launch_axpby (1.0, r, beta, p, n, st);
      apply_precond (s, p, ph);
      spmv_op (s, ph, v, nullptr, 0);
      if ((rc = dot_host (s, r0, v, &tmp))) return rc;
      if (tmp == 0.0 || !(tmp == tmp)) { status = NKP_BREAKDOWN; break; }
      alpha = rho_new / tmp;
      launch_copy (r, sv, n, st);
      launch_axpby (-alpha, v, 1.0, sv, n, st);
      apply_precond (s, sv, sh);
      spmv_op (s, sh, t, nullptr, 0);
      double ts, tt;
      if ((rc = dot_host (s, t, sv, &ts))) return rc;
      if ((rc = dot_host (s, t, t, &tt))) return rc;
      if (tt == 0.0 || !(tt == tt)) { status = NKP_BREAKDOWN; break; }
      omega = ts / tt;
      launch_axpby (alpha, ph, 1.0, s->x, n, st);
      launch_axpby (omega, sh, 1.0, s->x, n, st);
      launch_copy (sv, r, n, st);
      launch_axpby (-omega, t, 1.0, r, n, st);
      rho = rho_new;
      its++;
      if ((rc = dot_host (s, r, r, &rn2))) return rc;
      relres = sqrt (rn2) / bnorm;
      msg (s, 3, "bicgstab: its = %d, recurrence relres = %.3e\n", its, relres);
      if (omega == 0.0) { status = NKP_BREAKDOWN; break; }
   }
   spmv_op (s, s->x, r, s->b, 1);
   if ((rc = dot_host (s, r, r, &rn2))) return rc;
   relres = sqrt (rn2) / bnorm;
   if (sqrt (rn2) <= target * 1.0001) status = NKP_OK;
   else if (status == NKP_OK) status = NKP_NOT_CONVERGED;
   HIPCHK (hipGetLastError ());
   *iters_out = its;
   *relres_out = relres;
   return status;
}

int backward_error (nkp_solver *s, double *berr)
{
   spmv_op (s, s->x, s->r, s->b, 1);
   spmv_op (s, s->x, s->t1, s->b, 2);
   launch_berr (s->r, s->t1, s->n, s->partial, s->misc_dev () + 3, s->stream);
   allreduce_dev (s, s->misc_dev () + 3, 1, 1);
   HIPCHK (hipMemcpyAsync (s->hpin, s->misc_dev () + 3, sizeof (double), hipMemcpyDeviceToHost, s->stream));
   HIPCHK (hipStreamSynchronize (s->stream));
   *berr = s->hpin[0];
   return NKP_OK;
}

static int solve_resident (nkp_solver *s, double *berr, int *iters, double *relres)
{
   if (s->shared->broken) return refactor_broken (s);
   int it = 0;
   double rr = 0.0;
   s->stagnated = false;
   int status = (s->opt.krylov == NKP_KRYLOV_BICGSTAB) ? bicgstab (s, &it, &rr) : fgmres (s, &it, &rr);
   if (status < 0) return status;
   double be = 0.0;
   if (berr || s->stagnated) {
      int rc = backward_error (s, &be);
      if (rc) return rc;
      if (berr) *berr = be;
   }
   if (s->comm_failed) return fail (NKP_ECOMM, "nkp_solve: a collective of the distributed solve failed");
   if (status == NKP_NOT_CONVERGED && s->stagnated && be <= fmax (NKP_BERR_ROUNDING_LEVEL, 1.0e-2 * s->opt.rtol)) {
      msg (s, 1, "nkp_solve: residual stagnated at %.3e (rtol %.1e) with backward error %.3e: NKP_OK_BERR\n", rr, s->opt.rtol, be);
      status = NKP_OK_BERR;
   }
   if (iters) *iters = it;
   if (relres) *relres = rr;
   msg (s, 1, "nkp_solve: %s after %d iterations, ||b-Ax||/||b|| = %.3e\n", status == NKP_OK ? "converged" : status == NKP_OK_BERR ? "at the attainable accuracy (backward error accepted)" : status == NKP_BREAKDOWN ? "breakdown" : "NOT converged", it, rr);
   if (status == NKP_OK_BERR) fail (status, "nkp_solve: ||b-Ax||/||b|| = %.3e stopped above rtol %.1e at the attainable accuracy after %d iterations; componentwise backward error %.3e", rr, s->opt.rtol, it, be);
   else if (status != NKP_OK) fail (status, "nkp_solve: %s after %d iterations (relres %.3e, rtol %.1e)", status == NKP_BREAKDOWN ? "breakdown" : s->stagnated ? "stagnated at the attainable accuracy, not converged" : "not converged", it, rr, s->opt.rtol);
   return status;
}

extern "C" int nkp_solve_device (nkp_solver *s, const void *d_b, void *d_x, int use_guess, double *berr, int *iters, double *relres)
{
   if (!s || !d_b || !d_x) return fail (NKP_EINVAL, "nkp_solve_device: NULL argument");
   HIPCHK (hipSetDevice (s->device));
   const size_t bytes = (size_t) s->n * sizeof (double);
   if (use_guess) HIPCHK (hipMemcpyAsync (s->x, d_x, bytes, hipMemcpyDeviceToDevice, s->stream));
   else HIPCHK (hipMemsetAsync (s->x, 0, bytes, s->stream));
   HIPCHK (hipMemcpyAsync (s->b, d_b, bytes, hipMemcpyDeviceToDevice, s->stream));
   int status = solve_resident (s, berr, iters, relres);
   if (status < 0) return status;
   HIPCHK (hipMemcpyAsync (d_x, s->x, bytes, hipMemcpyDeviceToDevice, s->stream));
   HIPCHK (hipStreamSynchronize (s->stream));
   return status;
}

extern "C" int nkp_solve (nkp_solver *s, double *b_in_x_out, int nrhs, int64_t ldb, double *berr, int *iters, double *relres)
{
   if (!s || (nrhs > 0 && !b_in_x_out)) return fail (NKP_EINVAL, "nkp_solve: NULL argument");
   if (nrhs < 0 || (nrhs > 0 && ldb < s->n)) return fail (NKP_EINVAL, "nkp_solve: bad nrhs/ldb");
   HIPCHK (hipSetDevice (s->device));
   const size_t bytes = (size_t) s->n * sizeof (double);
   int worst = NKP_OK;
   if (nrhs >= 2 && s->tune.rhs_batch && !batch_unsupported (s)) {
      double *dB = nullptr;
      const int64_t ldd = s->ld;
      int status = NKP_OK;
      if (hipMalloc ((void **) &dB, (size_t) ldd * (size_t) nrhs * sizeof (double)) != hipSuccess) {
         dB = nullptr;
         (void) hipGetLastError ();
         status = fail (NKP_ENOMEM, "nkp_solve: device memory for %d right-hand sides", nrhs);
      }
      for (int c = 0; c < nrhs && status == NKP_OK; c++)
         if (hipMemcpy (dB + (size_t) c * (size_t) ldd, b_in_x_out + (size_t) c * (size_t) ldb, bytes, hipMemcpyHostToDevice) != hipSuccess) status = fail (NKP_EDEVICE, "nkp_solve: upload of right-hand side %d failed", c);
      if (s->dist.on) status = dist_agree (s, status, "nkp_solve", "staging the right-hand sides on the device");
      if (status != NKP_OK) { if (dB) (void) hipFree (dB); return status; }
// ... 21 lines not shown
```

### nk_ocn_tracer_jacobian_precond_amd/csrc/mlcycle.hip

```cpp
#include "nkp_dev.h"
#include "multilevel.h"

static void column_solves (const MlHierarchy &H, MlLevel &V, int c, const double *rhs, double *x, int accumulate, hipStream_t st)
{
   if (V.wave_columns) {
      if (H.f32) launch_colblock_apply_range_r32 (V.B, V.color_blk[c], V.color_blk[c + 1], rhs, x, accumulate, st);
      else launch_colblock_apply_range (V.B, V.color_blk[c], V.color_blk[c + 1], rhs, x, accumulate, st);
   } else
      launch_colblock_apply_lanes (V.B, V.color_grp[c], V.color_grp[c + 1], rhs, x, accumulate, st);
}

static void gs_half (const MlHierarchy &H, MlLevel &V, int c, bool fused, hipStream_t st)
{
   if (fused) {
      const int out = (V.cur[0] != V.cur[1]) ? V.cur[1 - c] : 1 - V.cur[c];
      const int rows0 = (int) V.rows0;
      if (V.wave_diag) launch_gs_wave_diag (V.L, V.B, V.color_tile[c], V.color_tile[c + 1], V.xbuf (V.cur[0]), V.xbuf (V.cur[1]), rows0, V.b, V.xbuf (out), H.f32, st);
      else if (V.lane_diag) launch_gs_lanes_diag (V.L, V.B, V.color_grp[c], V.color_grp[c + 1], V.xbuf (V.cur[0]), V.xbuf (V.cur[1]), rows0, V.b, V.xbuf (out), st);
      else if (V.wave_fused) launch_gs_wave (V.L, V.B, V.color_blk[c], V.color_blk[c + 1], V.xbuf (V.cur[0]), V.xbuf (V.cur[1]), rows0, V.b, V.xbuf (out), H.f32, st);
      else (void) launch_gs_fused (V.L, V.B, V.color_grp[c], V.color_grp[c + 1], V.xbuf (V.cur[0]), V.xbuf (V.cur[1]), rows0, V.b, V.xbuf (out), st);
      V.cur[c] = out;
      return;
   }
   if (V.L.dg_val) launch_diag_residual (V.L, V.color_tile[c], V.color_tile[c + 1], V.x, V.b, V.r, st);
   else launch_csr_residual_range (V.L, V.color_rb[c], V.color_rb[c + 1], V.x, V.b, V.r, st);
   column_solves (H, V, c, V.r, V.x, 1, st);
}

static void gs_sweep (const MlHierarchy &H, MlLevel &V, bool reverse, bool fused, hipStream_t st)
{
   for (int step = 0; step < 2; step++) gs_half (H, V, reverse ? 1 - step : step, fused, st);
}

static void ml_cycle (MlHierarchy &H, int l, hipStream_t st)
{
   MlLevel &V = H.lev[l];
   V.cur[0] = V.cur[1] = 0;
   if (l == H.tail_from && H.coarse_inv && H.gamma_to <= H.gamma_from && ml_tail_launch (H, l, st) == 0) return;
   if (l == (int) H.lev.size () - 1) {
      if (H.coarse_inv) {
         if (H.coarse_invf) launch_dense_matvec_f32 (H.coarse_invf, H.coarse_ldf, V.b, V.x, (int) V.n, st);
         else launch_dense_matvec (H.coarse_inv, V.b, V.x, (int) V.n, st);
         return;
      }
      const int sweeps = H.tune->ml_coarsest_sweeps > 0 ? H.tune->ml_coarsest_sweeps : 30;
      launch_fill (V.x, 0.0, V.n, st);
      column_solves (H, V, 0, V.b, V.x, 0, st);
      gs_half (H, V, 1, false, st);
      for (int s = 1; s < sweeps; s++) gs_sweep (H, V, s & 1, false, st);
      return;
   }
   const bool fused = ml_level_fused (H, V);
   launch_fill (V.x, 0.0, V.n, st);
   if (fused) {
      if (V.wave_fused) column_solves (H, V, 0, V.b, V.x2, 0, st);
      else launch_colblock_apply_lanes (V.B, V.color_grp[0], V.color_grp[1], V.b, V.x2, 0, st);
      V.cur[0] = 1;
      gs_half (H, V, 1, true, st);
   } else {
      column_solves (H, V, 0, V.b, V.x, 0, st);
      gs_half (H, V, 1, false, st);
   }
   const int nu = (l >= H.coarse_from) ? H.nu_coarse : H.nu;
   for (int s = 1; s < nu; s++) gs_sweep (H, V, false, fused, st);
   MlLevel &C = H.lev[l + 1];
   const int gamma = (l >= H.gamma_from && l < H.gamma_to) ? 2 : 1;
   for (int g = 0; g < gamma; g++) {
      if (V.L.dg_val) launch_diag_residual (V.L, V.color_tile[0], V.color_tile[2], V.xnow (), V.b, V.r, st);
      else launch_csr_spmv (V.L, V.xnow (), V.r, V.b, 1, st);
      launch_restrict_sum (V.rptr, V.ridx, V.r, C.b, V.nc, st);
      ml_cycle (H, l + 1, st);
      launch_prolong_add (V.cmap, C.xnow (), V.xnow (), V.n, H.omega, st);
   }
   for (int s = 0; s < nu; s++) gs_sweep (H, V, true, fused, st);
}

void ml_apply (MlHierarchy &H, const double *r, double *z, hipStream_t st)
{
   MlLevel &V = H.lev[0];
   launch_gather (H.perm0, r, V.b, V.n, st);
   ml_cycle (H, 0, st);
   launch_scatter (H.perm0, V.xnow (), z, V.n, st);
}

int ml_batch_prepare (MlHierarchy &H, int K)
{
   if (K != 2 && K != 4 && K != 8) return -1;
   if (H.batch_K >= K) return 0;
   auto drop = [&H] () {
      for (MlLevel &V : H.lev)
         for (double **p : { &V.bx, &V.bx2, &V.bb, &V.br })
            if (*p) {
               (void) hipFree (*p);
               *p = nullptr;
               H.device_bytes -= (size_t) (V.n ? V.n : 1) * (size_t) H.batch_K * sizeof (double);
            }
      H.batch_K = 0;
   };
   drop ();
   for (MlLevel &V : H.lev) {
      for (double **p : { &V.bx, &V.bx2, &V.bb, &V.br }) {
         const size_t bytes = (size_t) (V.n ? V.n : 1) * (size_t) K * sizeof (double);
         void *q = nullptr;
         if (hipMalloc (&q, bytes) != hipSuccess || hipMemset (q, 0, bytes) != hipSuccess) {
            if (q) (void) hipFree (q);
            H.batch_K = K;
            drop ();
            (void) hipGetLastError ();
            return -2;
         }
         *p = (double *) q;
         H.device_bytes += bytes;
      }
   }
   H.batch_K = K;
   return 0;
}

static void column_solves_batch (const MlHierarchy &H, MlLevel &V, int K, int c, const double *rhs, double *x, int accumulate, hipStream_t st)
{
   if (launch_colblock_apply_lanes_batch (K, V.B, V.color_grp[c], V.color_grp[c + 1], rhs, x, accumulate, st) != 0)
      launch_colblock_apply_wave_batch (K, V.B, V.color_blk[c], V.color_blk[c + 1], rhs, x, accumulate, H.f32, st);
}

static void gs_half_batch (const MlHierarchy &H, MlLevel &V, int K, int c, hipStream_t st)
{
   if (V.wave_fused) {
      const int out = (V.bcur[0] != V.bcur[1]) ? V.bcur[1 - c] : 1 - V.bcur[c];
      launch_gs_wave_batch (K, V.L, V.B, V.color_blk[c], V.color_blk[c + 1], V.bxbuf (V.bcur[0]), V.bxbuf (V.bcur[1]), (int) V.rows0, V.bb, V.bxbuf (out), H.f32, st);
      V.bcur[c] = out;
      return;
   }
   launch_csr_spmv_batch (K, V.L, V.color_rb[c], V.color_rb[c + 1], V.bx, V.br, V.bb, 1, st);
   column_solves_batch (H, V, K, c, V.br, V.bx, 1, st);
}

static void ml_cycle_batch (MlHierarchy &H, int K, int l, hipStream_t st)
{
   MlLevel &V = H.lev[l];
   const int64_t nk = V.n * K;
   V.bcur[0] = V.bcur[1] = 0;
   if (l == (int) H.lev.size () - 1) {
      if (H.coarse_inv) {
         if (H.coarse_invf) launch_dense_matvec_f32_batch (K, H.coarse_invf, H.coarse_ldf, V.bb, V.bx, (int) V.n, st);
         else launch_dense_matvec_batch (K, H.coarse_inv, V.bb, V.bx, (int) V.n, st);
         return;
      }
      const int sweeps = H.tune->ml_coarsest_sweeps > 0 ? H.tune->ml_coarsest_sweeps : 30;
      launch_fill (V.bx, 0.0, nk, st);
      column_solves_batch (H, V, K, 0, V.bb, V.bx, 0, st);
      launch_csr_spmv_batch (K, V.L, V.color_rb[1], V.color_rb[2], V.bx, V.br, V.bb, 1, st);
      column_solves_batch (H, V, K, 1, V.br, V.bx, 1, st);
      for (int s = 1; s < sweeps; s++)
         for (int step = 0; step < 2; step++) {
            const int c = (s & 1) ? 1 - step : step;
            launch_csr_spmv_batch (K, V.L, V.color_rb[c], V.color_rb[c + 1], V.bx, V.br, V.bb, 1, st);
            column_solves_batch (H, V, K, c, V.br, V.bx, 1, st);
         }
      return;
   }
   launch_fill (V.bx, 0.0, nk, st);
   if (V.wave_fused) {
      column_solves_batch (H, V, K, 0, V.bb, V.bx2, 0, st);
      V.bcur[0] = 1;
      gs_half_batch (H, V, K, 1, st);
   } else {
      column_solves_batch (H, V, K, 0, V.bb, V.bx, 0, st);
      gs_half_batch (H, V, K, 1, st);
   }
   const int nu = (l >= H.coarse_from) ? H.nu_coarse : H.nu;
   for (int s = 1; s < nu; s++) { gs_half_batch (H, V, K, 0, st); gs_half_batch (H, V, K, 1, st); }
   MlLevel &C = H.lev[l + 1];
   const int gamma = (l >= H.gamma_from && l < H.gamma_to) ? 2 : 1;
   for (int g = 0; g < gamma; g++) {
      launch_csr_spmv_batch (K, V.L, 0, V.L.nrowblk, V.bxnow (), V.br, V.bb, 1, st);
      launch_restrict_sum_batch (K, V.rptr, V.ridx, V.br, C.bb, V.nc, st);
      ml_cycle_batch (H, K, l + 1, st);
      launch_prolong_add_batch (K, V.cmap, C.bxnow (), V.bxnow (), V.n, H.omega, st);
   }
   for (int s = 0; s < nu; s++) { gs_half_batch (H, V, K, 1, st); gs_half_batch (H, V, K, 0, st); }
}

void ml_apply_batch (MlHierarchy &H, int K, const double *r, double *z, hipStream_t st)
{
   MlLevel &V = H.lev[0];
   launch_gather_batch (K, H.perm0, r, V.bb, V.n, st);
   ml_cycle_batch (H, K, 0, st);
   launch_scatter_batch (K, H.perm0, V.bxnow (), z, V.n, st);
}

void ml_apply_batch_split (MlHierarchy &H, int K, const double *const *src, double *z, double *const *dst, hipStream_t st, const double *src_scale)
{
   MlLevel &V = H.lev[0];
   launch_gather_interleave (K, H.perm0, src, V.bb, V.n, st, src_scale);
   ml_cycle_batch (H, K, 0, st);
   launch_scatter_split (K, H.perm0, V.bxnow (), z, dst, V.n, st);
}

void ml_apply_batch_split_ext (MlHierarchy &H, int K, const double *const *src, const double *halo, const int *sel, int64_t n_own, double *z,
                               double *const *dst, hipStream_t st)
{
   MlLevel &V = H.lev[0];
   if (sel) launch_gather_interleave_ext (K, H.perm0, src, halo, sel, n_own, V.bb, V.n, st);
   else launch_gather_interleave_ext_block (K, H.perm0, src, halo, n_own, V.bb, V.n, st);
   ml_cycle_batch (H, K, 0, st);
   launch_scatter_split_own (K, H.perm0, V.bxnow (), z, dst, n_own, V.n, st);
}

void ml_time_piece (MlHierarchy &H, int which, hipStream_t st)
{
   MlLevel &V = H.lev[0];
   if (H.lev.size () < 2) return;
   if (which == 0) {
      if (V.L.dg_val) launch_diag_residual (V.L, V.color_tile[0], V.color_tile[1], V.x, V.b, V.r, st);
      else launch_csr_residual_range (V.L, V.color_rb[0], V.color_rb[1], V.x, V.b, V.r, st);
   }
   else launch_colblock_apply_lanes (V.B, V.color_grp[0], V.color_grp[1], V.r, V.x, 1, st);
}

int64_t ml_bytes (const MlHierarchy &H, int which)
{
   if (H.lev.size () < 2) return 0;
   auto level_piece = [&] (const MlLevel &V, int colour, int what) -> int64_t {
      const int64_t rows = colour == 0 ? V.rows0 : V.n - V.rows0;
      const int64_t vb = V.L.valf ? 4 : 8, fb = V.B.fac_tf ? 4 : 8;
      if (what == 0 && V.L.dg_val) {
         const double share = V.n ? (double) rows / (double) V.n : 0.0;
         return (int64_t) (share * ((double) V.L.dg_nval * 4.0 + (double) V.L.dg_ntile * (double) sizeof (DgTile) + (double) V.L.dg_ngrp * (double) sizeof (DgGroup))) + rows * (8 + 8) + V.n * 8;
      }
      if (what == 0) {
         const double per_row = V.n ? (double) V.L.nnz / (double) V.n : 0.0;
         return (int64_t) (per_row * (double) rows * (double) (vb + 4)) + rows * (4 + 8 + 8) + V.n * 8;
      }
      return rows * ((2 * V.B.P + 1) * fb + 8 + 8 + 8);
// ... 25 lines not shown
```

### nk_ocn_tracer_jacobian_precond_amd/csrc/nkp_dev.h

```cpp
#pragma once
#include <hip/hip_runtime.h>
#include <stdint.h>

#include "../../include/nkp.h"
#include "col_plan.h"
#include "tuning.h"

#include <type_traits>
#include <utility>
#include <vector>

#define NKP_WAVE 64
#define NKP_MAX_K 512
#define NKP_SPMV_LDS_NNZ 2048
#define NKP_SPMV_MAX_ROWS 256

struct alignas (16) DgTile {
   int row0, rows;
   int kl0, len;
   int k0, nk;
   int g0, ng;
   long long voff;
};
struct DgGroup {
// ... 62 lines not shown
   double *fac_t = nullptr;
   float *fac_tf = nullptr;
   int lds_doubles = 0;
   int gw = 64;
   int rhs_slots = 0;
   int stream = 0;
   int ldsres = 0;
   int gs_ok = 0;
   int gs_lds_bytes = 0;
   int *gs_rb_ptr = nullptr;
   int *gs_rb = nullptr;
   int *wave_desc = nullptr;
   int *grp_tile = nullptr;
   int grp_tile_cnt = 0;
   const nkp_tuning *tune = nullptr;
   int ml_level = 0;
   ColKernel kern;
   std::vector<int> *grp_cols = nullptr;
};


template <int V> using int_tag = std::integral_constant<int, V>;
template <int V0, int... Vs, class F>
inline auto with_int (int v, F &&f)
{
   if constexpr (sizeof... (Vs) == 0) return f (int_tag<V0> ());
   else {
      if (v == V0) return f (int_tag<V0> ());
      return with_int<Vs...> (v, f);
   }
}
template <class F> inline auto with_band (int P, F &&f) { return with_int<1, 2, 4> (P, f); }
template <class F> inline auto with_k (int K, F &&f) { return with_int<2, 4, 8> (K, f); }
template <class F> inline auto with_bool (bool b, F &&f) { return b ? f (std::true_type ()) : f (std::false_type ()); }
template <class F> inline auto with_storage (const float *vf, const double *vd, F &&f) { return vf ? f (vf) : f (vd); }
template <class PTR> using elem_t = std::remove_cv_t<std::remove_pointer_t<PTR>>;
template <class F>
inline auto with_band_rows (const ColBlocksDev &B, F &&f)
{
   return with_band (B.P, [&] (auto p) { return with_int<1, 2> (B.max_len <= NKP_WAVE ? 1 : 2, [&] (auto rpl) { return f (p, rpl); }); });
}

template <int... Is, class F>
__device__ __forceinline__ void static_for_seq (std::integer_sequence<int, Is...>, F &&f) { (f (int_tag<Is> ()), ...); }
template <int N, class F>
__device__ __forceinline__ void static_for (F &&f) { static_for_seq (std::make_integer_sequence<int, N> (), f); }

template <int LANE>
__device__ __forceinline__ double readlane_const_f64 (double v)
{
   int lo = __double2loint (v), hi = __double2hiint (v);
   lo = __builtin_amdgcn_readlane (lo, LANE);
   hi = __builtin_amdgcn_readlane (hi, LANE);
   return __hiloint2double (hi, lo);
}

template <int P, int RPL, int K>
__device__ __forceinline__ void wave_band_sweeps (int len, int lane, double (&y)[RPL][K], const double (&invd)[RPL], const double (&L)[RPL][P],
                                                  const double (&U)[RPL][P])
{
   constexpr int ROWS = RPL * NKP_WAVE;
   len = __builtin_amdgcn_readfirstlane (len);
   double bc[K];
#pragma unroll
   for (int j = 0; j < K; j++) bc[j] = readlane_const_f64<0> (y[0][j]);
   static_for<ROWS - 1> ([&] (auto kc) __attribute__ ((always_inline)) {
      constexpr int k = decltype (kc)::value;
      if (__builtin_expect (k < len - 1, 1)) {
         constexpr int s1 = (k + 1) / NKP_WAVE, l1 = (k + 1) % NKP_WAVE;
         double t[K], nb[K];
#pragma unroll
         for (int j = 0; j < K; j++) {
            t[j] = y[s1][j] - L[s1][0] * bc[j];
            nb[j] = readlane_const_f64<l1> (t[j]);
         }
#pragma unroll
         for (int j = 0; j < K; j++) y[s1][j] = lane == l1 ? t[j] : y[s1][j];
#pragma unroll
         for (int q = 2; q <= P; q++)
            if (k + q < ROWS) {
               const int s = (k + q) / NKP_WAVE, l = (k + q) % NKP_WAVE;
#pragma unroll
               for (int j = 0; j < K; j++) {
                  const double u = y[s][j] - L[s][q - 1] * bc[j];
                  y[s][j] = lane == l ? u : y[s][j];
               }
            }
#pragma unroll
         for (int j = 0; j < K; j++) bc[j] = nb[j];
      }
   });
   asm volatile ("" : "+s" (len));
   double c[K];
#pragma unroll
   for (int j = 0; j < K; j++) {
      c[j] = y[0][j];
      if (RPL == 2 && len > NKP_WAVE) c[j] = y[RPL - 1][j];
   }
   static_for<ROWS> ([&] (auto ic) __attribute__ ((always_inline)) {
      constexpr int k = ROWS - 1 - decltype (ic)::value;
      if (__builtin_expect (k < len, 1)) {
         constexpr int s0 = k / NKP_WAVE, l0 = k % NKP_WAVE;
         double v[K];
#pragma unroll
         for (int j = 0; j < K; j++) {
            v[j] = c[j] * invd[s0];
            bc[j] = readlane_const_f64<l0> (v[j]);
         }
         if (k > 0) {
            constexpr int s1 = (k > 0 ? k - 1 : 0) / NKP_WAVE;
#pragma unroll
            for (int j = 0; j < K; j++) c[j] = y[s1][j] - U[s1][0] * bc[j];
         }
#pragma unroll
         for (int j = 0; j < K; j++) y[s0][j] = lane == l0 ? v[j] : y[s0][j];
#pragma unroll
         for (int q = 2; q <= P; q++)
            if (k - q >= 0) {
               const int s = (k - q) / NKP_WAVE, l = (k - q) % NKP_WAVE;
#pragma unroll
               for (int j = 0; j < K; j++) {
                  const double u = y[s][j] - U[s][q - 1] * bc[j];
                  y[s][j] = lane == l ? u : y[s][j];
               }
            }
      }
   });
}

int colblock_build_lane_layout (ColBlocksDev &B, const int *h_blk_start, const int *ranges, int nranges,
                                int *grp_first, size_t *device_bytes, hipStream_t st, int f32 = 0, const int *h_rowptr = nullptr);
int colblock_repack_lane_layout (const ColBlocksDev &B, const int *d_gcols, hipStream_t st);
int launch_gs_fused (const CsrDev &L, const ColBlocksDev &B, int g0, int g1, const double *xa, const double *xb, int split,
                     const double *b, double *xout, hipStream_t st);
void launch_colblock_apply_lanes (const ColBlocksDev &B, int g0, int g1, const double *r, double *z, int accumulate, hipStream_t st);

void launch_colblock_measure (const CsrDev &A, const ColBlocksDev &B, int *d_out2 , hipStream_t st);
void launch_colblock_factor (const CsrDev &A, ColBlocksDev &B, int *d_status, hipStream_t st);
void launch_colblock_apply (const ColBlocksDev &B, const double *r, double *z, hipStream_t st);
void launch_colblock_apply_range (const ColBlocksDev &B, int b0, int b1, const double *r, double *z, int accumulate, hipStream_t st);
void launch_colblock_apply_range_r32 (const ColBlocksDev &B, int b0, int b1, const double *r, double *z, int accumulate, hipStream_t st);
void launch_build_wave_desc (const CsrDev &L, ColBlocksDev &B, hipStream_t st);
void launch_gs_wave (const CsrDev &L, const ColBlocksDev &B, int b0, int b1, const double *xa, const double *xb, int split, const double *b, double *xout,
                     int r32, hipStream_t st);
void launch_gs_wave_diag (const CsrDev &L, const ColBlocksDev &B, int tile0, int tile1, const double *xa, const double *xb, int split, const double *b,
                          double *xout, int r32, hipStream_t st);
void launch_gs_lanes_diag (const CsrDev &L, const ColBlocksDev &B, int g0, int g1, const double *xa, const double *xb, int split, const double *b,
                           double *xout, hipStream_t st);

#define NKP_BATCH_MAX 8
#define NKP_RED_BLOCKS 1024
#define NKP_DOT_CHUNK 8

void launch_multi_dot (const void *V, int v_f32, int64_t ld, int k, const double *w, int64_t n, double *partial, double *out, hipStream_t st);
void launch_update_w (const void *V, int v_f32, int64_t ld, int k, const double *h, double *w, int64_t n, double *partial, double *out_nrm2, hipStream_t st);
void launch_scale_to (const double *x, const double *alpha_dev, double *y, float *yf, int64_t n, hipStream_t st);
void launch_axpy_multi (const double *Z, int64_t ld, int k, const double *c, double *x, int64_t n, hipStream_t st);
void launch_dot (const double *x, const double *y, int64_t n, double *partial, double *out, hipStream_t st);
void launch_berr (const double *r, const double *den, int64_t n, double *partial, double *out, hipStream_t st);
void launch_finish_column (double *h, const double *h2, int k, const double *nrm2, double *inv, hipStream_t st);
void launch_finish_column_pythagoras (double *h, int k, double *inv, hipStream_t st);
struct GsGroup {
   const double *V[NKP_BATCH_MAX];
   double *w[NKP_BATCH_MAX];
   double *partial[NKP_BATCH_MAX];
   double *vnext[NKP_BATCH_MAX];
};
void launch_multi_dot_group (int R, const GsGroup &G, int64_t ld, int k, int64_t n, double *msg, hipStream_t st);
void launch_update_w_group (int R, const GsGroup &G, int64_t ld, int k, const double *msg, int64_t n, double *nrm2, hipStream_t st);
void launch_finish_column_group (int R, double *msg, const double *msg2, int k, const double *nrm2, double *inv, hipStream_t st);
void launch_scale_to_group (int R, const GsGroup &G, const double *inv, int64_t n, hipStream_t st);
void launch_axpby (double a, const double *x, double b, double *y, int64_t n, hipStream_t st);
void launch_copy (const double *x, double *y, int64_t n, hipStream_t st);
void launch_vmul (const double *x, const double *w, double *y, int64_t n, hipStream_t st);
void launch_fill (double *y, double v, int64_t n, hipStream_t st);

void launch_restrict_sum (const int *rptr, const int *ridx, const double *fine, double *coarse, int64_t nc, hipStream_t st);
void launch_prolong_add (const int *cmap, const double *coarse, double *fine, int64_t nf, double omega, hipStream_t st);
void launch_gather (const int *perm, const double *in, double *out, int64_t n, hipStream_t st);
void launch_scatter (const int *perm, const double *in, double *out, int64_t n, hipStream_t st);
void launch_dense_matvec (const double *Minv, const double *x, double *y, int n, hipStream_t st);
void launch_dense_matvec_f32 (const float *Minv, int ld, const double *x, double *y, int n, hipStream_t st);
void launch_dense_matvec_f32_batch (int K, const float *Minv, int ld, const double *x, double *y, int n, hipStream_t st);
int dense_inverse_blocked_device (int n, const int *h_rowptr, const int *h_col, const double *h_val, double **inv_out, float **invf_out, int *ldf_out,
                                  size_t *bytes, hipStream_t st);
bool dense_inverse_device (int n, const std::vector<double> &host_a, double **inv_out, size_t *bytes, hipStream_t st);

void launch_interleave (int K, const double *const *src , double *X, int64_t n, hipStream_t st, const double *scale = nullptr);
void launch_deinterleave (int K, const double *X, double *const *dst , int64_t n, hipStream_t st);
void launch_csr_spmv_batch (int K, const CsrDev &A, int rb0, int rb1, const double *x, double *y, const double *b, int mode, hipStream_t st,
                            const double *scale = nullptr );
void launch_restrict_sum_batch (int K, const int *rptr, const int *ridx, const double *fine, double *coarse, int64_t nc, hipStream_t st);
void launch_prolong_add_batch (int K, const int *cmap, const double *coarse, double *fine, int64_t nf, double omega, hipStream_t st);
void launch_gather_batch (int K, const int *perm, const double *in, double *out, int64_t n, hipStream_t st);
void launch_scatter_batch (int K, const int *perm, const double *in, double *out, int64_t n, hipStream_t st);
void launch_gather_interleave (int K, const int *perm, const double *const *src, double *out, int64_t n, hipStream_t st, const double *scale = nullptr);
void launch_scatter_split (int K, const int *perm, const double *in, double *z, double *const *dst, int64_t n, hipStream_t st);
void launch_csr_spmv_batch_split (int K, const CsrDev &A, const double *x, double *const *dst, hipStream_t st, const double *scale = nullptr);
void launch_csr_spmv_batch_split_range (int K, const CsrDev &A, int rb0, int rb1, const double *x, double *const *dst, hipStream_t st, const double *scale = nullptr);
void launch_csr_residual_batch_split_range (int K, const CsrDev &A, int rb0, int rb1, const double *x, const double *const *b, const double *bscale,
                                            double *const *dst, hipStream_t st);
void launch_add_split (int K, const double *p, double *z, double *const *dst, int64_t n, hipStream_t st);
void launch_pack_rows_split (int K, const int *idx, const double *const *src, double *out, int64_t nrows, hipStream_t st);
void launch_gather_interleave_ext (int K, const int *perm, const double *const *src, const double *halo, const int *sel, int64_t n_own, double *out, int64_t n,
                                   hipStream_t st);
void launch_gather_interleave_ext_block (int K, const int *perm, const double *const *src, const double *recv, int64_t n_own, double *out, int64_t n, hipStream_t st);
void launch_scatter_split_own (int K, const int *perm, const double *in, double *z, double *const *dst, int64_t n_own, int64_t n, hipStream_t st);
void launch_dense_matvec_batch (int K, const double *Minv, const double *x, double *y, int n, hipStream_t st);
void launch_colblock_apply_wave_batch (int K, const ColBlocksDev &B, int b0, int b1, const double *r, double *z, int accumulate, int r32, hipStream_t st);
void launch_gs_wave_batch (int K, const CsrDev &L, const ColBlocksDev &B, int b0, int b1, const double *xa, const double *xb, int split, const double *b, double *xout,
                           int r32, hipStream_t st);
int launch_colblock_apply_lanes_batch (int K, const ColBlocksDev &B, int g0, int g1, const double *r, double *z, int accumulate, hipStream_t st);
```

### nk_ocn_tracer_jacobian_precond_amd/csrc/solver.hip

```cpp
#include "solver_impl.h"

#include <stdarg.h>
#include <stdio.h>
#include <string.h>

extern "C" int nkp_device_count (void)
{
   int n = 0;
   if (hipGetDeviceCount (&n) != hipSuccess) return 0;
   return n;
}

void solver_free (nkp_solver *s)
{
   if (!s) return;
   if (s->borrowed) {
      void *own[] = { s->V, s->vcur, s->Z, s->w, s->r, s->x, s->b, s->t1, s->t2, s->p1, s->p2, s->eqtmp, s->partial, s->dscal, s->dint };
      for (void *p : own)
         if (p) (void) hipFree (p);
      for (MlLevel &L : s->ml.lev) {
         void *lv[] = { L.x, L.x2, L.b, L.r };
         for (void *p : lv)
            if (p) (void) hipFree (p);
      }
      valgrad_release (s);
      valprod_release (s);
      if (s->hpin) (void) hipHostFree (s->hpin);
      if (s->own_stream && s->stream) (void) hipStreamDestroy (s->stream);
      s->shared->clones--;
      delete s;
      return;
   }
   if (s->trans_of) trans_detach (s);
   if (s->trans) trans_release (s);
   valgrad_release (s);
   valprod_release (s);
   for (nkp_solver *c : s->batch_members) solver_free (c);
   s->batch_members.clear ();
   for (double *p : { s->bvin, s->bz, s->bw })
      if (p) (void) hipFree (p);
   void *ptrs[] = { s->A.rowptr, s->A.colind, s->A.val, s->A.rowblk, s->A.codes, s->A.dict, s->A.dict_ptr, s->A.dg_ptr, s->A.dg_key, s->A.dg_voff, s->A.dg_vald, s->A.dg_tile, s->A.dg_gptr, s->A.dg_grp, s->B.blk_start, s->B.fac, s->B.grp_b0, s->B.grp_nb, s->B.grp_maxlen, s->B.grp_base, s->B.grp_row0, s->B.col_slot, s->B.fac_t, s->B.gs_rb_ptr, s->B.gs_rb, s->V, s->vcur, s->Z, s->w, s->r,
                    s->x, s->b, s->t1, s->t2, s->p1, s->p2, s->partial, s->dscal, s->dint, s->rscale, s->rinv, s->eqtmp };
   for (void *p : ptrs)
      if (p) (void) hipFree (p);
   delete s->B.grp_cols;
   ml_free (s->ml);
   if (s->rf) { rf_free (*s->rf); delete s->rf; }
   if (s->dplan) { rf_dist_free (*s->dplan); delete s->dplan; }
   if (s->dist.send_idx) (void) hipFree (s->dist.send_idx);
   if (s->dist.sendbuf) (void) hipFree (s->dist.sendbuf);
   if (s->dist.xe) (void) hipFree (s->dist.xe);
   if (s->dist.sel_idx) (void) hipFree (s->dist.sel_idx);
   if (s->dist.ras_send_idx) (void) hipFree (s->dist.ras_send_idx);
   if (s->dist.ras_sendbuf) (void) hipFree (s->dist.ras_sendbuf);
   if (s->dist.rext) (void) hipFree (s->dist.rext);
   if (s->dist.zext) (void) hipFree (s->dist.zext);
   for (double *p : { s->dist.bxe, s->dist.bsend, s->dist.gmsg, s->dist.bras_send, s->dist.bras_recv })
      if (p) (void) hipFree (p);
   if (s->dist.ghpin) (void) hipHostFree (s->dist.ghpin);
   if (s->dist.ev_packed) (void) hipEventDestroy (s->dist.ev_packed);
   if (s->dist.ev_halo) (void) hipEventDestroy (s->dist.ev_halo);
   if (s->dist.comm_stream) (void) hipStreamDestroy (s->dist.comm_stream);
   if (s->hpin) (void) hipHostFree (s->hpin);
   if (s->own_stream && s->stream) (void) hipStreamDestroy (s->stream);
   delete s;
}

extern "C" void nkp_destroy (nkp_solver *s) { solver_free (s); }

void msg (const nkp_solver *s, int lvl, const char *fmt, ...)
{
   if (s->opt.verbose < lvl) return;
   va_list ap;
   va_start (ap, fmt);
   printf ("(%d) ", s->opt.rank);
   vprintf (fmt, ap);
   va_end (ap);
   fflush (stdout);
}

extern "C" int nkp_set_stream (nkp_solver *s, void *hip_stream)
{
   if (!s) return fail (NKP_EINVAL, "nkp_set_stream: NULL solver");
   if (s->trans_of) return fail (NKP_EINVAL, "nkp_set_stream: a transposed solver runs on the stream of the solver it was transposed from; set that one's stream");
   if (s->own_stream && s->stream) { (void) hipStreamSynchronize (s->stream); (void) hipStreamDestroy (s->stream); }
   s->stream = (hipStream_t) hip_stream;
   s->own_stream = false;
   for (nkp_solver *c : s->batch_members) c->stream = s->stream;
   trans_set_stream (s);
   return NKP_OK;
}

extern "C" int64_t nkp_get_int (nkp_solver *s, const char *key)
{
   if (!s || !key) return -1;
   if (!strcmp (key, "n")) return s->n;
   if (!strcmp (key, "nnz")) return s->A.nnz;
   if (!strcmp (key, "nblk")) return s->B.nblk;
   if (!strcmp (key, "band")) return s->B.P;
   if (!strcmp (key, "band_dropped")) return s->B.dropped;
   if (!strcmp (key, "col_stream")) return s->B.stream ? 1 : 0;
   if (!strcmp (key, "col_ldsres")) return s->B.ldsres;
   if (!strcmp (key, "col_gw")) return s->B.gw;
   if (!strcmp (key, "col_max_len")) return s->B.max_len;
   if (!strcmp (key, "col_lds_bytes")) return (int64_t) s->B.lds_doubles * (int64_t) sizeof (double);
   if (!strcmp (key, "levels")) return s->opt.precond == NKP_PRECOND_MULTILEVEL ? (int64_t) s->ml.lev.size () : 1;
   if (!strcmp (key, "ml_rows")) { int64_t t = 0; for (auto &v : s->ml.lev) t += v.n; return t; }
   if (!strcmp (key, "ml_nnz")) { int64_t t = 0; for (auto &v : s->ml.lev) t += v.L.nnz; return t; }
   if (!strcmp (key, "rowblocks")) return s->A.nrowblk;
   if (!strcmp (key, "spmv_bytes")) return 12 * s->A.nnz + 4 * (s->n + 1) + 16 * s->n;
   if (!strcmp (key, "spmv_diag")) return s->A.dg_vald ? 1 : 0;
   if (!strcmp (key, "spmv_diag_bytes"))
      return s->A.dg_vald ? 8 * s->A.dg_nval + (int64_t) s->A.dg_ntile * (int64_t) sizeof (DgTile) + (int64_t) s->A.dg_ngrp * (int64_t) sizeof (DgGroup) + 16 * s->n : 0;
   if (!strcmp (key, "precond_bytes")) return s->opt.precond == NKP_PRECOND_NONE ? 16 * s->n : (int64_t) (2 * s->B.P + 1) * 8 * s->n + 16 * s->n;
   if (!strcmp (key, "device_bytes")) return (int64_t) s->device_bytes;
   if (!strcmp (key, "precond_steps")) return s->precond_steps;
   if (!strcmp (key, "equil")) return s->equil ? 1 : 0;
   if (!strcmp (key, "dist_overlap")) return s->dist.overlap ? 1 : 0;
   if (!strcmp (key, "dist_ras")) return s->dist.ras ? 1 : 0;
   if (!strcmp (key, "dist_ras_rows")) return s->dist.n_sel;
   if (!strcmp (key, "dist_ras_rings")) return s->dist.ras ? s->dist.ras_rings : 0;
   if (!strcmp (key, "dist_halo_rows")) return s->dist.n_halo;
   if (!strcmp (key, "dist_ras_recv_rows")) return !s->dist.ras ? 0 : s->dist.ras_sep ? s->dist.n_sel : s->dist.n_halo;
   if (!strcmp (key, "dist_interior_rowblocks")) return s->dist.seg_rb[2] - s->dist.seg_rb[1];
   if (!strcmp (key, "smoother_spmv_bytes")) return s->opt.precond == NKP_PRECOND_MULTILEVEL ? ml_bytes (s->ml, 0) : 0;
   if (!strcmp (key, "column_solve_bytes")) return s->opt.precond == NKP_PRECOND_MULTILEVEL ? ml_bytes (s->ml, 1) : 0;
   if (!strcmp (key, "cycle_bytes")) return s->opt.precond == NKP_PRECOND_MULTILEVEL ? ml_bytes (s->ml, 2) : 0;
   if (!strcmp (key, "ml_levels_on_device")) return s->ml.levels_on_device;
   if (!strcmp (key, "ml_inverse_pivoted")) return s->ml.inverse_pivoted;
   if (!strcmp (key, "ml_setup_us")) return (int64_t) (s->ml.setup_seconds * 1.0e6);
   if (!strcmp (key, "create_us")) return (int64_t) (s->create_seconds * 1.0e6);
   if (!strcmp (key, "refactor_count")) return s->refactor_count;
   if (!strcmp (key, "refactor_rebuilt")) return s->refactor_rebuilt;
   if (!strcmp (key, "refactor_us")) return (int64_t) (s->refactor_seconds * 1.0e6);
   if (!strcmp (key, "refactor_halo_values")) return s->refactor_halo_values;
   if (!strcmp (key, "is_transpose")) return s->trans_of ? 1 : 0;
   if (!strcmp (key, "trans_device_bytes")) return trans_device_bytes (s);
   if (!strcmp (key, "trans_us")) return (int64_t) (s->trans_seconds * 1.0e6);
   if (!strcmp (key, "trans_kernel_us")) return (int64_t) (s->trans_kernel_seconds * 1.0e6);
   if (!strcmp (key, "trans_sent_entries")) return s->trans_sent;
   if (!strcmp (key, "trans_recv_entries")) return s->trans_received;
   if (!strcmp (key, "dist_alltoallv_calls")) return s->shared->alltoallv_calls.load ();
   if (!strcmp (key, "dist_allreduce_calls")) return s->shared->allreduce_calls.load ();
   if (!strcmp (key, "value_gradient_calls")) return s->vg.calls;
   if (!strcmp (key, "value_gradient_us")) return (int64_t) (s->vg.seconds * 1.0e6);
   if (!strcmp (key, "values_product_calls")) return s->vp.calls;
   if (!strcmp (key, "values_product_us")) return (int64_t) (s->vp.seconds * 1.0e6);
   if (!strcmp (key, "tangent_calls")) return s->vp.tangent_calls;
   if (!strcmp (key, "batch_steps")) return s->batch_steps;
   if (!strcmp (key, "batch_width")) return s->batch_width;
   if (!strcmp (key, "batch_member_bytes")) {
      size_t sum = 0;
      for (const nkp_solver *c : s->batch_members) sum += c->device_bytes;
      return (int64_t) sum;
   }
   return -1;
}

extern "C" int nkp_set_device (int device)
{
   HIPCHK (hipSetDevice (device));
   return NKP_OK;
}
```

### nk_ocn_tracer_jacobian_precond_amd/csrc/solver_impl.h

```cpp
#pragma once
#include "../../include/nkp.h"
#include "nkp_dev.h"
#include "multilevel.h"
#include "refactor.h"
#include "dist_plan.h"
#include "krylov_host.h"

#include <atomic>
#include <initializer_list>
#include <memory>
#include <string>
#include <vector>

#define HIPCHK(call)                                                                             \
   do {                                                                                          \
      hipError_t e_ = (call);                                                                    \
      if (e_ != hipSuccess) return fail (NKP_EDEVICE, "%s failed: %s (%s:%d)", #call, hipGetErrorString (e_), __FILE__, __LINE__); \
   } while (0)

struct nkp_solver {
   nkp_options opt;
   nkp_tuning tune;
   int device = 0;
   bool stagnated = false;
   bool borrowed = false;
   hipStream_t stream = nullptr;
   bool own_stream = false;
   CsrDev A;
   ColBlocksDev B;
   MlHierarchy ml;
   struct {
      bool on = false;
      nkp_comm_ops ops;
      int64_t n_global = 0, fst = 0, n_halo = 0, nsend = 0;
      std::vector<int> send_counts, recv_counts;
      int *send_idx = nullptr;
      double *sendbuf = nullptr;
      double *xe = nullptr;
      int seg_rb[4] = { 0, 0, 0, 0 };
      bool overlap = false;
      hipStream_t comm_stream = nullptr;
      hipEvent_t ev_packed = nullptr, ev_halo = nullptr;
      bool ras = false;
      int64_t n_ext = 0, n_sel = 0;
      int *sel_idx = nullptr;
      double *rext = nullptr, *zext = nullptr;
      int ras_rings = 0;
      bool ras_sep = false;
      int64_t ras_nsend = 0;
      int *ras_send_idx = nullptr;
      double *ras_sendbuf = nullptr, *bras_send = nullptr, *bras_recv = nullptr;
      std::vector<int> ras_send_counts, ras_recv_counts, ras_send_counts_k, ras_recv_counts_k;
      double *bxe = nullptr, *bsend = nullptr, *gmsg = nullptr, *ghpin = nullptr;
      int bK = 0;
      int agreed_K = 0;
      std::vector<int> send_counts_k, recv_counts_k;
      std::vector<int64_t> starts;
      std::vector<int32_t> h_halo_rows, h_send_rows, own_blk, own_ci, own_cj, own_ct;
      bool own_has_blk = false;
      int own_tracer_cnt = 1;
   } dist;
   int64_t n = 0, ld = 0;
   int m = 0;
   bool vf32 = false;
   double *vcur = nullptr;
   double *V = nullptr, *Z = nullptr, *w = nullptr, *r = nullptr, *x = nullptr, *b = nullptr, *t1 = nullptr, *t2 = nullptr;
   double *p1 = nullptr, *p2 = nullptr;
   int precond_steps = 1;
   int steps_now = 1;
   bool equil = false;
   double *rscale = nullptr, *rinv = nullptr;
   double *eqtmp = nullptr;
   bool comm_failed = false;
   double *partial = nullptr;
   double *dscal = nullptr;
   double *hpin = nullptr;
   int *dint = nullptr;
   std::vector<nkp_solver *> batch_members;
   double *bvin = nullptr, *bz = nullptr, *bw = nullptr;
   int batch_K = 0;
   int64_t batch_steps = 0;
   int batch_width = 0;
   size_t device_bytes = 0;
   double create_seconds = 0.0;
   struct Shared {
      std::atomic<int> clones { 0 };
      std::atomic<int64_t> alltoallv_calls { 0 }, allreduce_calls { 0 };
      bool broken = false;
      std::string why;
   };
   std::shared_ptr<Shared> shared = std::make_shared<Shared> ();
   RefactorWork *rf = nullptr;
   std::vector<int> h_blk, h_col_i, h_col_j, h_col_t;
   int tracer_cnt = 1;
   int64_t refactor_count = 0;
   int refactor_rebuilt = 0;
   double refactor_seconds = 0.0;
   DistRefactorPlan *dplan = nullptr;
   int64_t refactor_halo_values = 0;
   nkp_solver *trans = nullptr, *trans_of = nullptr;
   int *trans_src = nullptr;
   double *trans_val = nullptr;
   size_t trans_map_bytes = 0;
   double trans_seconds = 0.0, trans_kernel_seconds = 0.0;
   int *trans_ship = nullptr;
   double *trans_send = nullptr, *trans_recv = nullptr;
   std::vector<int> trans_send_counts, trans_recv_counts;
   int64_t trans_nnz = 0, trans_sent = 0, trans_received = 0;
   struct {
      double *lam = nullptr, *x = nullptr, *stage = nullptr, *g = nullptr;
      size_t lam_cap = 0, x_cap = 0, stage_cap = 0, g_cap = 0;
      int64_t calls = 0;
      double seconds = 0.0;
   } vg;
   struct {
      double *x = nullptr, *stage = nullptr, *r = nullptr;
      size_t x_cap = 0, stage_cap = 0, r_cap = 0;
      int64_t calls = 0, tangent_calls = 0;
      double seconds = 0.0;
   } vp;
   double *h_dev () { return dscal; }
   double *h2_dev () { return dscal + (m + 2); }
   double *misc_dev () { return dscal + 2 * (m + 2); }
   double *y_dev () { return dscal + 2 * (m + 2) + 16; }
};

template <class T>
static int dev_alloc (nkp_solver *s, T **p, size_t count)
{
   void *q = nullptr;
   size_t bytes = (count ? count : 1) * sizeof (T);
   hipError_t e = hipMalloc (&q, bytes);
   if (e != hipSuccess) return fail (NKP_ENOMEM, "hipMalloc of %zu bytes failed: %s", bytes, hipGetErrorString (e));
   *p = (T *) q;
   s->device_bytes += bytes;
   return NKP_OK;
}


struct Want {
   double **p;
   size_t *cap;
   size_t need;
};

inline int reserve (nkp_solver *s, std::initializer_list<Want> set, const char *who)
{
   double *fresh[8] = {};
   int rc = NKP_OK;
   size_t i = 0;
   for (const Want &w : set) {
      if (w.need > *w.cap) {
         void *q = nullptr;
         if (hipMalloc (&q, w.need * sizeof (double)) != hipSuccess) {
            rc = fail (NKP_ENOMEM, "%s: hipMalloc of %zu bytes of work space failed", who, w.need * sizeof (double));
            break;
         }
         fresh[i] = (double *) q;
      }
      i++;
   }
   if (rc) {
      for (double *q : fresh)
         if (q) (void) hipFree (q);
      (void) hipGetLastError ();
      return rc;
   }
   i = 0;
   for (const Want &w : set) {
      if (fresh[i]) {
         if (*w.p) {
            (void) hipFree (*w.p);
            s->device_bytes -= *w.cap * sizeof (double);
         }
         *w.p = fresh[i];
         *w.cap = w.need;
         s->device_bytes += w.need * sizeof (double);
      }
      i++;
   }
   return NKP_OK;
}

inline int width_of (int nrhs) { return nrhs <= 1 ? 1 : nrhs <= 2 ? 2 : nrhs <= 4 ? 4 : 8; }

inline void alltoallv_dev (nkp_solver *s, const double *send, const int *send_counts, double *recv, const int *recv_counts, hipStream_t st)
{
   s->shared->alltoallv_calls++;
   if (s->dist.ops.alltoallv (s->dist.ops.ctx, send, send_counts, recv, recv_counts, (void *) st)) s->comm_failed = true;
}

inline void allreduce_dev (nkp_solver *s, double *dev, int count, int op)
{
   if (!s->dist.on) return;
   s->shared->allreduce_calls++;
   if (s->dist.ops.allreduce (s->dist.ops.ctx, dev, count, op, (void *) s->stream)) s->comm_failed = true;
}

inline int refactor_broken (const nkp_solver *s) { return fail (NKP_ESINGULAR, "%s", s->shared->why.c_str ()); }

inline int sev_of (int c) { return c == NKP_OK ? 0 : c == NKP_OK_BERR ? 1 : c == NKP_NOT_CONVERGED ? 2 : 3; }

#define NKP_BERR_ROUNDING_LEVEL 1.0e-14

NKP_PRIVATE void solver_free (nkp_solver *s);
NKP_PRIVATE void msg (const nkp_solver *s, int lvl, const char *fmt, ...);
struct SpmvMatrixHost {
   int64_t nnz, ncols;
   const int32_t *rowptr, *colind;
   const double *val;
};
struct PrecondMatrixHost {
   int64_t n, nblk;
   const int32_t *rowptr, *colind;
   const double *val;
   const int32_t *blk_start, *col_i, *col_j, *col_t;
};
NKP_PRIVATE int create_impl (nkp_solver **out, const nkp_options *opt_in, int64_t n, int64_t nnz,
                             const int32_t *rowptr, const int32_t *colind, const double *val,
                             const int32_t *blk_start, int64_t nblk, int coupled_tracer_cnt, const SpmvMatrixHost *spmv_mat,
                             const PrecondMatrixHost *pm = nullptr);
NKP_PRIVATE int clone_impl (nkp_solver *src, nkp_solver **out, bool member);
NKP_PRIVATE void drop_intertracer (int64_t n, int tracer_cnt, const int32_t *rowptr, const int32_t *colind, const double *val,
                                   std::vector<int32_t> &f_rowptr, std::vector<int32_t> &f_colind, std::vector<double> &f_val);
NKP_PRIVATE void apply_precond_once (nkp_solver *s, const double *rin, double *zout);
NKP_PRIVATE void apply_precond (nkp_solver *s, const double *rin, double *zout);
NKP_PRIVATE void spmv_op (nkp_solver *s, const double *x, double *y, const double *b, int mode);
NKP_PRIVATE void arnoldi_apply (nkp_solver *s, int j);
NKP_PRIVATE void arnoldi_orthogonalise (nkp_solver *s, int j);
NKP_PRIVATE void arnoldi_step_device (nkp_solver *s, int j);
NKP_PRIVATE int fg_begin (nkp_solver *s, FgmresState &F);
NKP_PRIVATE int fg_restart (nkp_solver *s, FgmresState &F);
NKP_PRIVATE bool fg_post_step (nkp_solver *s, FgmresState &F);
NKP_PRIVATE int fg_end_cycle (nkp_solver *s, FgmresState &F);
NKP_PRIVATE int backward_error (nkp_solver *s, double *berr);
NKP_PRIVATE const char *batch_unsupported (const nkp_solver *s);
NKP_PRIVATE void note_fallback (const nkp_solver *s, const char *who, const char *why, int nrhs);
NKP_PRIVATE int batch_prepare_exchange (nkp_solver *s, int K);
NKP_PRIVATE int dist_agree (nkp_solver *s, int local_rc, const char *who, const char *where);
NKP_PRIVATE void valgrad_release (nkp_solver *s);
NKP_PRIVATE int valgrad_time_prepare (nkp_solver *s, int K);
NKP_PRIVATE void valgrad_time_launch (nkp_solver *s, int K);
NKP_PRIVATE int fetch_x_operand (nkp_solver *s, int K, const double *const *xp, double *il, const double **x_in, const char *who);
NKP_PRIVATE void valprod_release (nkp_solver *s);
NKP_PRIVATE int valprod_time_prepare (nkp_solver *s, int K, int which);
NKP_PRIVATE void valprod_time_launch (nkp_solver *s, int K);
NKP_PRIVATE void valprod_time_composition (nkp_solver *s, int K);
NKP_PRIVATE void trans_release (nkp_solver *s);
NKP_PRIVATE void trans_detach (nkp_solver *t);
NKP_PRIVATE void trans_set_stream (nkp_solver *s);
NKP_PRIVATE int64_t trans_device_bytes (const nkp_solver *s);
NKP_PRIVATE int trans_gather_values (nkp_solver *s, const double **d_valT);
NKP_PRIVATE int trans_dist_follow (nkp_solver *s, int flags, const char *who, int (*refactor) (nkp_solver *t, const void *d_val, int flags, const char *who));
```

### nk_ocn_tracer_jacobian_precond_amd/csrc/tuning.cpp

```cpp
#include "tuning.h"

#include <stdarg.h>
#include <stdio.h>
#include <stdlib.h>
#include <string.h>

static thread_local std::string g_last_error;

int fail (int code, const char *fmt, ...)
{
   char buf[512];
   va_list ap;
   va_start (ap, fmt);
   vsnprintf (buf, sizeof buf, fmt, ap);
   va_end (ap);
   g_last_error = buf;
   return code;
}

extern "C" const char *nkp_last_error (void) { return g_last_error.c_str (); }
std::string last_error_message () { return g_last_error; }
void restore_error_message (const std::string &text) { g_last_error = text; }

extern "C" int nkp_default_options (nkp_options *opt)
{
   if (!opt) return NKP_EINVAL;
   memset (opt, 0, sizeof *opt);
   opt->struct_size = (int) sizeof (nkp_options);
   opt->precond = NKP_PRECOND_MULTILEVEL;
   opt->krylov = NKP_KRYLOV_FGMRES;
   opt->restart = 200;
   opt->max_iters = 20000;
   opt->rtol = 1.0e-10;
   opt->atol = 0.0;
   opt->device = -1;
   opt->verbose = 0;
   opt->rank = 0;
   opt->reorth = 0;
   opt->ml_levels = 0;
   opt->ml_smooth = 3;
   opt->precond_steps = 0;
   opt->equil = 0;
   opt->basis_f32 = 0;
   return NKP_OK;
}

static void builtin_tuning (nkp_tuning *t)
{
   memset (t, 0, sizeof *t);
   t->struct_size = (int) sizeof (nkp_tuning);
   t->ml_split = 1; t->ml_pocket = 4; t->ml_big_from = -3; t->ml_coarsest_rows = 8000; t->ml_dense_max = 8192;
   t->ml_theta = 0.0; t->ml_tau = 0.01; t->ml_device_min = 100000;
   t->ml_smooth_coarse = 0; t->ml_coarse_from = 2; t->ml_gamma_from = 0; t->ml_gamma_to = 0; t->ml_f32 = 1; t->ml_host_inverse = 0;
   t->ml_fused = 0; t->ml_fused_max_cols = 0; t->ml_wave_fused = 1; t->ml_coarsest_sweeps = 30; t->ml_tail_rows = 0; t->ml_omega = 1.1;
   t->col_ldsres = 2; t->col_stream = 1; t->col_stream_min = -1; t->col_stream_gw = 32; t->col_wave_max = 8192; t->col_w3 = 1;
   t->col_group = 8; t->col_pipe_min = 0; t->col_ldsres_early = 0; t->col_ldsres_packed = 1; t->col_sort_groups = 1;
   t->spmv_variant = 4; t->spmv_compress = 0; t->spmv_pipe_min = 1024; t->spmv_run = 1; t->spmv_wgs = 256;
   t->rhs_batch = 1; t->batch_spmv_rows = 1; t->precond_steps = 0; t->equil = -1; t->dist_overlap = 1; t->dist_ras = 1; t->dist_one_reduce = 0; t->force_dist = 0; t->setup_threads = 0; t->plan_times = 0;
   t->ml_drop_intertracer = 0; t->ml_huge_from = -1; t->dist_ras_rings = 1; t->ml_diag = 32; t->spmv_diag = 32;
   t->ml_lane_fused = 50000;
}

const nkp_tuning &nkp_builtin_tuning ()
{
   static const nkp_tuning t = [] { nkp_tuning q; builtin_tuning (&q); return q; } ();
   return t;
}

extern "C" int nkp_default_tuning (nkp_tuning *t)
{
   if (!t) return NKP_EINVAL;
   builtin_tuning (t);
   const char *e;
#define ENV_INT(name, field) do { if ((e = getenv (name)) && *e) t->field = atoi (e); } while (0)
#define ENV_POS(name, field) do { if ((e = getenv (name)) && atoi (e) > 0) t->field = atoi (e); } while (0)
#define ENV_FLAG(name, field) do { if ((e = getenv (name)) && *e) t->field = atoi (e) != 0; } while (0)
   ENV_FLAG ("NKP_ML_SPLIT", ml_split); ENV_INT ("NKP_ML_POCKET", ml_pocket); ENV_INT ("NKP_ML_BIG_FROM", ml_big_from);
   ENV_INT ("NKP_ML_COARSEST_ROWS", ml_coarsest_rows); ENV_INT ("NKP_ML_DENSE_MAX", ml_dense_max);
   if ((e = getenv ("NKP_ML_THETA")) && *e) t->ml_theta = atof (e);
   if ((e = getenv ("NKP_ML_TAU")) && *e) t->ml_tau = atof (e);
   if ((e = getenv ("NKP_ML_DEVICE_MIN")) && *e) t->ml_device_min = atoll (e);
   ENV_POS ("NKP_ML_SMOOTH_COARSE", ml_smooth_coarse); ENV_POS ("NKP_ML_COARSE_FROM", ml_coarse_from);
   ENV_INT ("NKP_ML_GAMMA_FROM", ml_gamma_from); ENV_INT ("NKP_ML_GAMMA_TO", ml_gamma_to);
   ENV_FLAG ("NKP_ML_F32", ml_f32); ENV_FLAG ("NKP_ML_HOST_INVERSE", ml_host_inverse); ENV_FLAG ("NKP_ML_FUSED", ml_fused);
   ENV_INT ("NKP_ML_FUSED_MAX_COLS", ml_fused_max_cols); ENV_INT ("NKP_ML_WAVE_FUSED", ml_wave_fused); ENV_POS ("NKP_ML_COARSEST_SWEEPS", ml_coarsest_sweeps);
   if ((e = getenv ("NKP_ML_TAIL_ROWS")) && *e) t->ml_tail_rows = atoll (e);
   if ((e = getenv ("NKP_ML_OMEGA")) && atof (e) > 0.0) t->ml_omega = atof (e);
   ENV_INT ("NKP_COL_LDSRES", col_ldsres); ENV_FLAG ("NKP_COLSTREAM", col_stream); ENV_INT ("NKP_COLSTREAM_MIN", col_stream_min);
   if ((e = getenv ("NKP_COLSTREAM_GW")) && *e) t->col_stream_gw = atoi (e) == 64 ? 64 : 32;
   ENV_INT ("NKP_COLWAVE_MAX", col_wave_max); ENV_FLAG ("NKP_COL_W3", col_w3); ENV_INT ("NKP_COLGROUP", col_group);
   ENV_INT ("NKP_COLPIPE_MIN", col_pipe_min); ENV_FLAG ("NKP_LDSRES_EARLY", col_ldsres_early); ENV_FLAG ("NKP_COL_PACKED", col_ldsres_packed); ENV_FLAG ("NKP_COL_SORT_GROUPS", col_sort_groups); ENV_INT ("NKP_COL_LDSRES_MIN", col_ldsres_min); ENV_INT ("NKP_ML_HUGE_FROM", ml_huge_from);
   ENV_INT ("NKP_SPMV_VARIANT", spmv_variant); ENV_FLAG ("NKP_SPMV_COMPRESS", spmv_compress); ENV_INT ("NKP_SPMV_PIPE_MIN", spmv_pipe_min);
   ENV_POS ("NKP_SPMV_RUN", spmv_run); ENV_POS ("NKP_SPMV_WGS", spmv_wgs);
   ENV_INT ("NKP_RHS_BATCH", rhs_batch); ENV_FLAG ("NKP_BATCH_SPMV_ROWS", batch_spmv_rows);
   ENV_POS ("NKP_PRECOND_STEPS", precond_steps); ENV_FLAG ("NKP_EQUIL", equil);
   ENV_FLAG ("NKP_DIST_OVERLAP", dist_overlap); ENV_FLAG ("NKP_DIST_RAS", dist_ras); ENV_FLAG ("NKP_DIST_ONE_REDUCE", dist_one_reduce);
   if (getenv ("NKP_FORCE_DIST")) t->force_dist = 1;
   ENV_POS ("NKP_SETUP_THREADS", setup_threads);
   if (getenv ("NKP_ML_PLAN_TIMES")) t->plan_times = 1;
   ENV_FLAG ("NKP_ML_DROP_INTERTRACER", ml_drop_intertracer);
   ENV_INT ("NKP_DIST_RAS_RINGS", dist_ras_rings);
   ENV_INT ("NKP_ML_DIAG", ml_diag);
   ENV_INT ("NKP_SPMV_DIAG", spmv_diag);
   ENV_INT ("NKP_ML_LANE_FUSED", ml_lane_fused);
#undef ENV_INT
#undef ENV_POS
#undef ENV_FLAG
   if (t->spmv_variant < 0 || t->spmv_variant > 9) t->spmv_variant = 4;
   return NKP_OK;
}

int resolve_tuning (const nkp_options *opt, nkp_tuning *out, bool *range_error)
{
   if (range_error) *range_error = false;
   if (opt && opt->tuning) {
      if (opt->tuning->struct_size != (int) sizeof (nkp_tuning)) return fail (NKP_EINVAL, "nkp_tuning.struct_size mismatch (%d != %zu)", opt->tuning->struct_size, sizeof (nkp_tuning));
      *out = *opt->tuning;
   } else {
      const int rc = nkp_default_tuning (out);
      if (rc) return rc;
   }
   if (out->dist_ras_rings < 0 || out->dist_ras_rings > 4) {
      if (range_error) *range_error = true;
      return fail (NKP_EINVAL, "nkp_tuning.dist_ras_rings = %d is out of range (0 = default, 1 .. 4 rings)", out->dist_ras_rings);
   }
   return NKP_OK;
}
```

### nk_ocn_tracer_jacobian_precond_amd/solver.py

```python
from __future__ import annotations

import ctypes as C
import os

import numpy as np

_HERE = os.path.dirname(os.path.abspath(__file__))
HIP_LIB_PATH = os.path.join(_HERE, "csrc", "libnkp_hip.so")
HOST_LIB_PATH = os.path.join(_HERE, "host", "libnkp_host.so")

PRECOND_NONE, PRECOND_COLUMN_JACOBI, PRECOND_MULTILEVEL = 0, 1, 3
KRYLOV_FGMRES, KRYLOV_BICGSTAB = 0, 1
NKP_OK, NKP_NOT_CONVERGED, NKP_BREAKDOWN, NKP_OK_BERR = 0, 1, 2, 3
REFACTOR_REBUILD = 1

ABI_SYMBOLS = [
    "nkp_default_options", "nkp_device_count", "nkp_create", "nkp_solve", "nkp_solve_device",
    "nkp_spmv", "nkp_spmv_device", "nkp_precond_apply", "nkp_multi_dot", "nkp_time_kernel",
    "nkp_get_int", "nkp_set_stream", "nkp_destroy", "nkp_last_error", "nkp_comm_unique_id",
    "nkp_comm_rccl_init", "nkp_comm_rccl_free", "nkp_create_dist", "nkp_dist_plan_host", "nkp_set_device",
    "nkp_gather_root", "nkp_clone", "nkp_ml_plan_host", "nkp_comm_file_init", "nkp_comm_file_free",
    "nkp_create64", "nkp_cell_major_order", "nkp_permuted_rows", "nkp_dist_overlap_plan_host", "nkp_dist_plan_size",
    "nkp_dist_plan_copy", "nkp_dist_plan_free", "nkp_ml_level_array", "nkp_default_tuning", "nkp_solve_batch_device",
    "nkp_refactor", "nkp_refactor_device", "nkp_refactor_dist", "nkp_refactor_dist_device", "nkp_transpose", "nkp_transpose_dist",
    "nkp_value_gradient", "nkp_value_gradient_device",
    "nkp_values_product", "nkp_values_product_device", "nkp_solve_tangent_device", "nkp_matrix_array",
]

_ALLREDUCE_FN = C.CFUNCTYPE(C.c_int, C.c_void_p, C.c_void_p, C.c_int, C.c_int, C.c_void_p)
_ALLTOALLV_FN = C.CFUNCTYPE(C.c_int, C.c_void_p, C.c_void_p, C.POINTER(C.c_int), C.c_void_p, C.POINTER(C.c_int), C.c_void_p)
_ALLTOALLV_I32_FN = C.CFUNCTYPE(C.c_int, C.c_void_p, C.POINTER(C.c_int32), C.POINTER(C.c_int), C.POINTER(C.c_int32), C.POINTER(C.c_int))
_ALLGATHER_I64_FN = C.CFUNCTYPE(C.c_int, C.c_void_p, C.c_int64, C.POINTER(C.c_int64))


class NkpCommOps(C.Structure):
    _fields_ = [("ctx", C.c_void_p), ("rank", C.c_int), ("nranks", C.c_int), ("allreduce", _ALLREDUCE_FN),
                ("alltoallv", _ALLTOALLV_FN), ("alltoallv_i32_host", _ALLTOALLV_I32_FN),
                ("allgather_i64_host", _ALLGATHER_I64_FN)]


class NkpTuning(C.Structure):
    _fields_ = [
        ("struct_size", C.c_int), ("ml_split", C.c_int), ("ml_pocket", C.c_int), ("ml_big_from", C.c_int), ("ml_coarsest_rows", C.c_int),
        ("ml_dense_max", C.c_int), ("ml_theta", C.c_double), ("ml_tau", C.c_double), ("ml_device_min", C.c_int64),
        ("ml_smooth_coarse", C.c_int), ("ml_coarse_from", C.c_int), ("ml_gamma_from", C.c_int), ("ml_gamma_to", C.c_int), ("ml_f32", C.c_int),
        ("ml_host_inverse", C.c_int), ("ml_fused", C.c_int), ("ml_fused_max_cols", C.c_int), ("ml_wave_fused", C.c_int), ("ml_coarsest_sweeps", C.c_int),
        ("ml_tail_rows", C.c_int64), ("ml_omega", C.c_double),
        ("col_ldsres", C.c_int), ("col_stream", C.c_int), ("col_stream_min", C.c_int), ("col_stream_gw", C.c_int), ("col_wave_max", C.c_int),
        ("col_w3", C.c_int), ("col_group", C.c_int), ("col_pipe_min", C.c_int), ("col_ldsres_early", C.c_int), ("col_ldsres_packed", C.c_int),
        ("spmv_variant", C.c_int), ("spmv_compress", C.c_int), ("spmv_pipe_min", C.c_int), ("spmv_run", C.c_int), ("spmv_wgs", C.c_int),
        ("rhs_batch", C.c_int), ("precond_steps", C.c_int), ("equil", C.c_int), ("dist_overlap", C.c_int), ("dist_ras", C.c_int), ("force_dist", C.c_int),
        ("setup_threads", C.c_int), ("plan_times", C.c_int), ("ml_drop_intertracer", C.c_int), ("dist_one_reduce", C.c_int), ("ml_huge_from", C.c_int), ("col_ldsres_min", C.c_int), ("col_sort_groups", C.c_int), ("batch_spmv_rows", C.c_int),
        ("dist_ras_rings", C.c_int), ("ml_diag", C.c_int), ("spmv_diag", C.c_int), ("ml_lane_fused", C.c_int),
    ]


class NkpOptions(C.Structure):
    _fields_ = [
        ("struct_size", C.c_int), ("precond", C.c_int), ("krylov", C.c_int), ("restart", C.c_int),
        ("max_iters", C.c_int), ("rtol", C.c_double), ("atol", C.c_double), ("device", C.c_int),
        ("verbose", C.c_int), ("rank", C.c_int), ("reorth", C.c_int), ("ml_levels", C.c_int),
        ("ml_smooth", C.c_int), ("basis_f32", C.c_int), ("precond_steps", C.c_int), ("equil", C.c_int), ("reserved", C.c_int * 4),
        ("col_i", C.POINTER(C.c_int32)), ("col_j", C.POINTER(C.c_int32)), ("col_t", C.POINTER(C.c_int32)),
        ("tuning", C.POINTER(NkpTuning)),
    ]


class NkpError(RuntimeError):
    def __init__(self, code, message):
        super().__init__(f"nkp error {code}: {message}")
        self.code = code


_lib = None


def load_library(path=None):
    global _lib
    if _lib is not None and path is None:
        return _lib
    path = path or HIP_LIB_PATH
    if not os.path.exists(path):
        raise FileNotFoundError(
            f"{path} not found: build it with `python -c 'import __graft_entry__ as g; g.build()'` "
            "(there is no CPU fallback for the solve path)")
    lib = C.CDLL(path, mode=C.RTLD_GLOBAL)
    i32p, f64p, vp = C.POINTER(C.c_int32), C.POINTER(C.c_double), C.c_void_p
    lib.nkp_default_options.argtypes = [C.POINTER(NkpOptions)]
    lib.nkp_device_count.restype = C.c_int
    lib.nkp_create.argtypes = [C.POINTER(vp), C.POINTER(NkpOptions), C.c_int64, C.c_int64, i32p, i32p, f64p, i32p, C.c_int64, C.c_int]
    lib.nkp_create64.argtypes = [C.POINTER(vp), C.POINTER(NkpOptions), C.c_int64, C.POINTER(C.c_int64), i32p, f64p, i32p, C.c_int64, C.c_int]
    lib.nkp_solve.argtypes = [vp, f64p, C.c_int, C.c_int64, f64p, C.POINTER(C.c_int), f64p]
    lib.nkp_solve_device.argtypes = [vp, vp, vp, C.c_int, f64p, C.POINTER(C.c_int), f64p]
    lib.nkp_solve_batch_device.argtypes = [vp, C.c_int, vp, vp, C.c_int64, f64p, C.POINTER(C.c_int), f64p]
    lib.nkp_spmv.argtypes = [vp, f64p, f64p]
    lib.nkp_spmv_device.argtypes = [vp, vp, vp]
    lib.nkp_precond_apply.argtypes = [vp, f64p, f64p]
    lib.nkp_multi_dot.argtypes = [vp, f64p, C.c_int64, C.c_int, f64p, f64p]
    lib.nkp_time_kernel.argtypes = [vp, C.c_int, C.c_int, C.c_int, f64p]
    lib.nkp_get_int.argtypes = [vp, C.c_char_p]
    lib.nkp_get_int.restype = C.c_int64
    lib.nkp_ml_level_array.argtypes = [vp, C.c_int, C.c_char_p, vp, C.c_int64]
    lib.nkp_ml_level_array.restype = C.c_int64
    lib.nkp_matrix_array.argtypes = [vp, C.c_char_p, vp, C.c_int64]
    lib.nkp_matrix_array.restype = C.c_int64
    lib.nkp_set_stream.argtypes = [vp, vp]
    lib.nkp_destroy.argtypes = [vp]
    lib.nkp_destroy.restype = None
    lib.nkp_last_error.restype = C.c_char_p
    lib.nkp_comm_unique_id.argtypes = [vp]
    lib.nkp_comm_rccl_init.argtypes = [C.POINTER(NkpCommOps), vp, C.c_int, C.c_int]
    lib.nkp_comm_rccl_free.argtypes = [C.POINTER(NkpCommOps)]
    lib.nkp_comm_rccl_free.restype = None
    lib.nkp_create_dist.argtypes = [C.POINTER(vp), C.POINTER(NkpOptions), C.c_int64, C.c_int64, C.c_int64, C.c_int64,
                                    i32p, i32p, f64p, i32p, C.c_int64, C.c_int, C.POINTER(NkpCommOps)]
    lib.nkp_set_device.argtypes = [C.c_int]
    lib.nkp_gather_root.argtypes = [vp, f64p, f64p]
    lib.nkp_clone.argtypes = [vp, C.POINTER(vp)]
    lib.nkp_transpose.argtypes = [vp, C.POINTER(vp)]
    lib.nkp_transpose_dist.argtypes = [vp, C.POINTER(vp)]
    lib.nkp_value_gradient.argtypes = [vp, C.c_int, f64p, f64p, C.c_int64, C.c_double, C.c_int, f64p]
    lib.nkp_value_gradient_device.argtypes = [vp, C.c_int, vp, vp, C.c_int64, C.c_double, C.c_int, vp]
    lib.nkp_values_product.argtypes = [vp, C.c_int, f64p, f64p, C.c_int64, C.c_double, C.c_int, f64p, C.c_int64]
    lib.nkp_values_product_device.argtypes = [vp, C.c_int, vp, vp, C.c_int64, C.c_double, C.c_int, vp, C.c_int64]
    lib.nkp_solve_tangent_device.argtypes = [vp, C.c_int, vp, vp, C.c_int64, vp, vp, C.c_int64, f64p, C.POINTER(C.c_int), f64p]
    lib.nkp_refactor.argtypes = [vp, f64p, C.c_int]
    lib.nkp_refactor_device.argtypes = [vp, vp, C.c_int]
    lib.nkp_refactor_dist.argtypes = [vp, f64p, C.c_int]
    lib.nkp_refactor_dist_device.argtypes = [vp, vp, C.c_int]
    lib.nkp_dist_plan_host.argtypes = [C.c_int64, C.c_int64, i32p, i32p, C.c_int, C.c_int, C.POINTER(C.c_int64), i32p, i32p,
                                       C.POINTER(C.c_int64), i32p]
    lib.nkp_ml_plan_host.argtypes = [C.c_int64, i32p, i32p, f64p, i32p, C.c_int64, i32p, i32p, C.c_int, C.c_int, C.c_int, C.c_int64,
                                     C.POINTER(C.c_int), C.POINTER(C.c_int64), i32p, i32p]
    if path == HIP_LIB_PATH:
        _lib = lib
    return lib


def ml_plan_host(rowptr, colind, val, blk_start, col_i=None, col_j=None, coupled_tracer_cnt=1, max_levels=0, coarsest_rows=8000):
    lib = load_library()
    rowptr = np.ascontiguousarray(rowptr, np.int32)
    colind = np.ascontiguousarray(colind, np.int32)
    val = np.ascontiguousarray(val, np.float64)
    blk_start = np.ascontiguousarray(blk_start, np.int32)
    n = rowptr.size - 1
    ip = lambda a: None if a is None else _p(np.ascontiguousarray(a, np.int32), C.c_int32)
    ci = None if col_i is None else np.ascontiguousarray(col_i, np.int32)
    cj = None if col_j is None else np.ascontiguousarray(col_j, np.int32)
    cap = 2 * n + 64
    cmap, colof = np.empty(cap, np.int32), np.empty(cap, np.int32)
    rows = np.zeros(64, np.int64)
    nlev = C.c_int()
    rc = lib.nkp_ml_plan_host(n, _p(rowptr, C.c_int32), _p(colind, C.c_int32), _p(val, C.c_double), _p(blk_start, C.c_int32), blk_start.size - 1,
                              None if ci is None else _p(ci, C.c_int32), None if cj is None else _p(cj, C.c_int32), coupled_tracer_cnt, max_levels,
                              coarsest_rows, cap, C.byref(nlev), _p(rows, C.c_int64), _p(cmap, C.c_int32), _p(colof, C.c_int32))
    if rc != 0:
        raise NkpError(rc, "nkp_ml_plan_host failed")
    rows = rows[:nlev.value]
    cmaps, colofs, qc, qo = [], [], 0, 0
    for l in range(nlev.value - 1):
        cmaps.append(cmap[qc:qc + rows[l]].copy())
        colofs.append(colof[qo:qo + rows[l + 1]].copy())
        qc += rows[l]
        qo += rows[l + 1]
    return rows, cmaps, colofs


def default_options(**overrides):
    lib = load_library()
    o = NkpOptions()
    lib.nkp_default_options(C.byref(o))
    for k, v in overrides.items():
        if not hasattr(o, k):
            raise AttributeError(f"nkp_options has no field {k}")
        setattr(o, k, v)
    return o


def default_tuning(**overrides):
    lib = load_library()
    t = NkpTuning()
    lib.nkp_default_tuning.argtypes = [C.POINTER(NkpTuning)]
    lib.nkp_default_tuning(C.byref(t))
    for k, v in overrides.items():
        if not hasattr(t, k):
            raise AttributeError(f"nkp_tuning has no field {k}")
        setattr(t, k, v)
    return t


def _p(a, t):
    return a.ctypes.data_as(C.POINTER(t))


def cell_major_order(blk_start, coupled_tracer_cnt):
    lib = load_library()
    blk = np.ascontiguousarray(blk_start, np.int32)
    nblk, n = blk.size - 1, int(blk[-1])
    perm = np.empty(max(n, 1), np.int32)
    blk_new = np.empty(nblk + 1, np.int32)
    col_t = np.empty(max(nblk, 1), np.int32)
    col_src = np.empty(max(nblk, 1), np.int32)
    lib.nkp_cell_major_order.argtypes = [C.c_int64, C.POINTER(C.c_int32), C.c_int] + [C.POINTER(C.c_int32)] * 4
    rc = lib.nkp_cell_major_order(nblk, _p(blk, C.c_int32), int(coupled_tracer_cnt), _p(perm, C.c_int32), _p(blk_new, C.c_int32),
                                  _p(col_t, C.c_int32), _p(col_src, C.c_int32))
    if rc != 0:
# ... 336 lines not shown
```

Measured before the change: 33.95 million.

## Fold reduction finishes into last-block tickets and mirror Hessenberg column to host

Adds an iter_fold tuning knob, on by default with value 5. The multi-dot and update_w kernels gain a last-block-ticket path: the final block to finish sums the per-block partials and, for update_w, computes the norm, the subdiagonal entry and its inverse. This removes the separate finish kernels. The finished Hessenberg column is also written to coherent pinned host memory with a sequence word, so the host can poll it instead of doing a device-to-host copy and sync. Gather and restrict kernels can now zero an auxiliary vector in the same pass. This trades kernel launches and host round trips for atomics, system-scope stores and more complex memory-ordering logic.

Measured after the change: 34.25 million, median of 6. About the same (+0.9%).

```diff
diff --git a/include/nkp.h b/include/nkp.h
--- a/include/nkp.h
+++ b/include/nkp.h
@@ -85,6 +85,7 @@
    int ml_diag;
    int spmv_diag;
    int ml_lane_fused;
+   int iter_fold;
 } nkp_tuning;
 
 int nkp_default_tuning (nkp_tuning *t);
diff --git a/nk_ocn_tracer_jacobian_precond_amd/csrc/blas1.hip b/nk_ocn_tracer_jacobian_precond_amd/csrc/blas1.hip
--- a/nk_ocn_tracer_jacobian_precond_amd/csrc/blas1.hip
+++ b/nk_ocn_tracer_jacobian_precond_amd/csrc/blas1.hip
@@ -34,9 +34,43 @@
    return (int) g;
 }
 
+__device__ __forceinline__ void store_partial (double *p, double v, bool publish)
+{
+   if (publish) __hip_atomic_store (p, v, __ATOMIC_RELAXED, __HIP_MEMORY_SCOPE_AGENT);
+   else *p = v;
+}
+
+__device__ __forceinline__ bool draws_last_ticket (unsigned *ticket, unsigned count, double *sh)
+{
+   if (threadIdx.x == 0) {
+      asm volatile ("s_waitcnt vmcnt(0)" ::: "memory");
+      const bool last = __hip_atomic_fetch_add (ticket, 1u, __ATOMIC_RELAXED, __HIP_MEMORY_SCOPE_AGENT) == count - 1u;
+      if (last) __hip_atomic_store (ticket, 0u, __ATOMIC_RELAXED, __HIP_MEMORY_SCOPE_AGENT);
+      asm volatile ("" ::: "memory");
+      sh[0] = last ? 1.0 : 0.0;
+   }
+   __syncthreads ();
+   return sh[0] != 0.0;
+}
+
+__device__ __forceinline__ double lane_sum_partials (const double *p, int64_t stride, int nblk, int lane)
+{
+   double v[NKP_RED_BLOCKS / NKP_WAVE];
+#pragma unroll
+   for (int i = 0; i < NKP_RED_BLOCKS / NKP_WAVE; i++) {
+      const int b = lane + i * NKP_WAVE;
+      v[i] = b < nblk ? __hip_atomic_load (p + (int64_t) b * stride, __ATOMIC_RELAXED, __HIP_MEMORY_SCOPE_AGENT) : 0.0;
+   }
+   double s = 0.0;
+#pragma unroll
+   for (int i = 0; i < NKP_RED_BLOCKS / NKP_WAVE; i++)
+      if (lane + i * NKP_WAVE < nblk) s += v[i];
+   return s;
+}
+
 template <class VT, class VT2>
 __device__ __forceinline__ void multi_dot_body (const VT *__restrict__ V, int64_t ld, int k, const double *__restrict__ w,
-                                                int64_t n, double *__restrict__ partial, double *sh)
+                                                int64_t n, double *__restrict__ partial, double *sh, bool publish = false)
 {
    const int chunk = blockIdx.y;
    const int j0 = chunk * NKP_DOT_CHUNK;
@@ -69,19 +103,32 @@
 #pragma unroll
    for (int c = 0; c < NKP_DOT_CHUNK; c++) {
       const double s = block_sum (acc[c], sh);
-      if (threadIdx.x == 0) out[c] = s;
+      if (threadIdx.x == 0) store_partial (out + c, s, publish);
    }
    const double sw = block_sum (accw, sh);
-   if (threadIdx.x == 0) out[NKP_DOT_CHUNK] = sw;
-}
-
-template <class VT, class VT2>
+   if (threadIdx.x == 0) store_partial (out + NKP_DOT_CHUNK, sw, publish);
+}
+
+template <class VT, class VT2, bool FOLD>
 __global__ __launch_bounds__ (B1_THREADS)
 void multi_dot_kernel (const VT *__restrict__ V, int64_t ld, int k, const double *__restrict__ w,
-                       int64_t n, double *__restrict__ partial)
+                       int64_t n, double *partial, unsigned *tickets, double *out)
 {
    __shared__ double sh[B1_THREADS / NKP_WAVE];
-   multi_dot_body<VT, VT2> (V, ld, k, w, n, partial, sh);
+   multi_dot_body<VT, VT2> (V, ld, k, w, n, partial, sh, FOLD);
+   if (FOLD) {
+      const int chunk = blockIdx.y, nblk = gridDim.x;
+      if (!draws_last_ticket (tickets + chunk, (unsigned) nblk, sh)) return;
+      const int j0 = chunk * NKP_DOT_CHUNK;
+      const int kc = (k - j0) < NKP_DOT_CHUNK ? (k - j0) : NKP_DOT_CHUNK;
+      const int lane = threadIdx.x & (NKP_WAVE - 1), wv = threadIdx.x / NKP_WAVE;
+      for (int c = wv; c <= NKP_DOT_CHUNK; c += B1_THREADS / NKP_WAVE) {
+         if (c < NKP_DOT_CHUNK ? c >= kc : chunk != 0) continue;
+         const double *p = partial + (int64_t) chunk * nblk * (NKP_DOT_CHUNK + 1) + c;
+         const double s = wave_sum (lane_sum_partials (p, NKP_DOT_CHUNK + 1, nblk, lane));
+         if (lane == 0) out[c < NKP_DOT_CHUNK ? j0 + c : k] = s;
+      }
+   }
 }
 
 __global__ __launch_bounds__ (B1_THREADS)
@@ -116,12 +163,16 @@
    multi_dot_finish_body (G.partial[blockIdx.y], nblk, k, msg + (int64_t) blockIdx.y * (k + 1));
 }
 
-void launch_multi_dot (const void *V, int v_f32, int64_t ld, int k, const double *w, int64_t n, double *partial, double *out, hipStream_t st)
+void launch_multi_dot (const void *V, int v_f32, int64_t ld, int k, const double *w, int64_t n, double *partial, double *out, hipStream_t st, unsigned *tickets)
 {
    const int g = red_grid (n);
    const int nchunk = k > 0 ? (k + NKP_DOT_CHUNK - 1) / NKP_DOT_CHUNK : 1;
-   if (v_f32) hipLaunchKernelGGL ((multi_dot_kernel<float, float2>), dim3 (g, nchunk), dim3 (B1_THREADS), 0, st, (const float *) V, ld, k, w, n, partial);
-   else hipLaunchKernelGGL ((multi_dot_kernel<double, double2>), dim3 (g, nchunk), dim3 (B1_THREADS), 0, st, (const double *) V, ld, k, w, n, partial);
+   if (tickets && !v_f32) {
+      hipLaunchKernelGGL ((multi_dot_kernel<double, double2, true>), dim3 (g, nchunk), dim3 (B1_THREADS), 0, st, (const double *) V, ld, k, w, n, partial, tickets, out);
+      return;
+   }
+   if (v_f32) hipLaunchKernelGGL ((multi_dot_kernel<float, float2, false>), dim3 (g, nchunk), dim3 (B1_THREADS), 0, st, (const float *) V, ld, k, w, n, partial, (unsigned *) nullptr, (double *) nullptr);
+   else hipLaunchKernelGGL ((multi_dot_kernel<double, double2, false>), dim3 (g, nchunk), dim3 (B1_THREADS), 0, st, (const double *) V, ld, k, w, n, partial, (unsigned *) nullptr, (double *) nullptr);
    hipLaunchKernelGGL (multi_dot_finish_kernel, dim3 (k + 1), dim3 (NKP_WAVE), 0, st, partial, g, k, out);
 }
 
@@ -137,7 +188,8 @@
 #define B1_MAX_K NKP_MAX_K
 template <class VT, class VT2>
 __device__ __forceinline__ void update_w_body (const VT *__restrict__ V, int64_t ld, int k, const double *__restrict__ h,
-                                               double *__restrict__ w, int64_t n, double *__restrict__ partial, double sign, double *hs, double *sh)
+                                               double *__restrict__ w, int64_t n, double *__restrict__ partial, double sign, double *hs, double *sh,
+                                               bool publish = false)
 {
    for (int j = threadIdx.x; j < k; j += B1_THREADS) hs[j] = sign * h[j];
    __syncthreads ();
@@ -172,18 +224,42 @@
    }
    if (partial) {
       const double s = block_sum (nrm, sh);
-      if (threadIdx.x == 0) partial[blockIdx.x] = s;
-   }
-}
-
-template <class VT, class VT2>
+      if (threadIdx.x == 0) store_partial (partial + blockIdx.x, s, publish);
+   }
+}
+
+__device__ __forceinline__ void mirror_column (const double *h, int k, double hk, const ColumnMirror &M, int lane)
+{
+   for (int j = lane; j < k; j += NKP_WAVE) __hip_atomic_store (M.col + j, h[j], __ATOMIC_RELAXED, __HIP_MEMORY_SCOPE_SYSTEM);
+   if (lane == 0) __hip_atomic_store (M.col + k, hk, __ATOMIC_RELAXED, __HIP_MEMORY_SCOPE_SYSTEM);
+   asm volatile ("s_waitcnt vmcnt(0)" ::: "memory");
+   __builtin_amdgcn_fence (__ATOMIC_RELEASE, "");
+   asm volatile ("s_waitcnt vmcnt(0)" ::: "memory");
+   if (lane == 0) __hip_atomic_store (M.seq_word, M.seq, __ATOMIC_RELAXED, __HIP_MEMORY_SCOPE_SYSTEM);
+}
+
+template <class VT, class VT2, bool FOLD>
 __global__ __launch_bounds__ (B1_THREADS)
 void update_w_kernel (const VT *__restrict__ V, int64_t ld, int k, const double *__restrict__ h,
-                      double *__restrict__ w, int64_t n, double *__restrict__ partial, double sign)
+                      double *__restrict__ w, int64_t n, double *partial, double sign, double *out_nrm2, ColumnFinish fin)
 {
    __shared__ double hs[B1_MAX_K];
    __shared__ double sh[B1_THREADS / NKP_WAVE];
-   update_w_body<VT, VT2> (V, ld, k, h, w, n, partial, sign, hs, sh);
+   update_w_body<VT, VT2> (V, ld, k, h, w, n, partial, sign, hs, sh, FOLD);
+   if (FOLD) {
+      const int nblk = gridDim.x;
+      if (!draws_last_ticket (fin.ticket, (unsigned) nblk, sh) || threadIdx.x >= NKP_WAVE) return;
+      const int lane = threadIdx.x;
+      const double s = wave_sum (lane_sum_partials (partial, 1, nblk, lane));
+      double t = 0.0;
+      if (lane == 0) {
+         out_nrm2[0] = s;
+         t = sqrt (s);
+         fin.hcol[k] = t;
+         fin.inv[0] = (t > 0.0) ? 1.0 / t : 0.0;
+      }
+      if (fin.mirror.col) mirror_column (fin.hcol, k, t, fin.mirror, lane);
+   }
 }
 
 __global__ __launch_bounds__ (B1_THREADS)
@@ -215,11 +291,16 @@
    sum_partials_body (G.partial[blockIdx.x], nblk, out + blockIdx.x);
 }
 
-void launch_update_w (const void *V, int v_f32, int64_t ld, int k, const double *h, double *w, int64_t n, double *partial, double *out_nrm2, hipStream_t st)
+void launch_update_w (const void *V, int v_f32, int64_t ld, int k, const double *h, double *w, int64_t n, double *partial, double *out_nrm2, hipStream_t st, const ColumnFinish *fin)
 {
    const int g = red_grid (n);
-   if (v_f32) hipLaunchKernelGGL ((update_w_kernel<float, float2>), dim3 (g), dim3 (B1_THREADS), 0, st, (const float *) V, ld, k, h, w, n, partial, -1.0);
-   else hipLaunchKernelGGL ((update_w_kernel<double, double2>), dim3 (g), dim3 (B1_THREADS), 0, st, (const double *) V, ld, k, h, w, n, partial, -1.0);
+   if (fin && !v_f32) {
+      hipLaunchKernelGGL ((update_w_kernel<double, double2, true>), dim3 (g), dim3 (B1_THREADS), 0, st, (const double *) V, ld, k, h, w, n, partial, -1.0, out_nrm2, *fin);
+      return;
+   }
+   const ColumnFinish none = { nullptr, nullptr, nullptr, ColumnMirror () };
+   if (v_f32) hipLaunchKernelGGL ((update_w_kernel<float, float2, false>), dim3 (g), dim3 (B1_THREADS), 0, st, (const float *) V, ld, k, h, w, n, partial, -1.0, (double *) nullptr, none);
+   else hipLaunchKernelGGL ((update_w_kernel<double, double2, false>), dim3 (g), dim3 (B1_THREADS), 0, st, (const double *) V, ld, k, h, w, n, partial, -1.0, (double *) nullptr, none);
    hipLaunchKernelGGL (sum_partials_kernel, dim3 (1), dim3 (NKP_WAVE), 0, st, partial, g, out_nrm2);
 }
 
@@ -234,7 +315,8 @@
 void launch_axpy_multi (const double *Z, int64_t ld, int k, const double *c, double *x, int64_t n, hipStream_t st)
 {
    const int g = red_grid (n);
-   hipLaunchKernelGGL ((update_w_kernel<double, double2>), dim3 (g), dim3 (B1_THREADS), 0, st, Z, ld, k, c, x, n, (double *) nullptr, 1.0);
+   const ColumnFinish none = { nullptr, nullptr, nullptr, ColumnMirror () };
+   hipLaunchKernelGGL ((update_w_kernel<double, double2, false>), dim3 (g), dim3 (B1_THREADS), 0, st, Z, ld, k, c, x, n, (double *) nullptr, 1.0, (double *) nullptr, none);
 }
 
 __device__ __forceinline__ void scale_to_body (const double *__restrict__ x, const double *__restrict__ alpha, double *__restrict__ y, float *__restrict__ yf, int64_t n)
@@ -409,9 +491,10 @@
 
 __global__ __launch_bounds__ (NKP_WAVE)
 void finish_column_kernel (double *__restrict__ h, const double *__restrict__ h2, int k,
-                           const double *__restrict__ nrm2, double *__restrict__ inv)
+                           const double *__restrict__ nrm2, double *__restrict__ inv, ColumnMirror mirror)
 {
    finish_column_body (h, h2, k, nrm2, inv);
+   if (mirror.col) mirror_column (h, k, threadIdx.x == 0 ? h[k] : 0.0, mirror, (int) threadIdx.x);
 }
 
 __device__ __forceinline__ void finish_column_pythagoras_body (double *__restrict__ h, int k, double *__restrict__ inv)
@@ -454,27 +537,28 @@
    hipLaunchKernelGGL (finish_column_pythagoras_kernel, dim3 (1), dim3 (NKP_WAVE), 0, st, h, k, inv);
 }
 
-void launch_finish_column (double *h, const double *h2, int k, const double *nrm2, double *inv, hipStream_t st)
-{
-   hipLaunchKernelGGL (finish_column_kernel, dim3 (1), dim3 (NKP_WAVE), 0, st, h, h2, k, nrm2, inv);
+void launch_finish_column (double *h, const double *h2, int k, const double *nrm2, double *inv, hipStream_t st, const ColumnMirror *mirror)
+{
+   hipLaunchKernelGGL (finish_column_kernel, dim3 (1), dim3 (NKP_WAVE), 0, st, h, h2, k, nrm2, inv, mirror ? *mirror : ColumnMirror ());
 }
 
 __global__ __launch_bounds__ (B1_THREADS)
 void restrict_sum_kernel (const int *__restrict__ rptr, const int *__restrict__ ridx, const double *__restrict__ fine,
-                          double *__restrict__ coarse, int64_t nc)
+                          double *__restrict__ coarse, int64_t nc, double *__restrict__ zero)
 {
    const int64_t stride = (int64_t) gridDim.x * B1_THREADS;
    for (int64_t I = (int64_t) blockIdx.x * B1_THREADS + threadIdx.x; I < nc; I += stride) {
       double acc = 0.0;
       for (int q = rptr[I]; q < rptr[I + 1]; q++) acc += fine[ridx[q]];
       coarse[I] = acc;
-   }
-}
-
-void launch_restrict_sum (const int *rptr, const int *ridx, const double *fine, double *coarse, int64_t nc, hipStream_t st)
+      if (zero) zero[I] = 0.0;
+   }
+}
+
+void launch_restrict_sum (const int *rptr, const int *ridx, const double *fine, double *coarse, int64_t nc, hipStream_t st, double *zero)
 {
    if (nc <= 0) return;
-   hipLaunchKernelGGL (restrict_sum_kernel, dim3 (red_grid (nc) * 2), dim3 (B1_THREADS), 0, st, rptr, ridx, fine, coarse, nc);
+   hipLaunchKernelGGL (restrict_sum_kernel, dim3 (red_grid (nc) * 2), dim3 (B1_THREADS), 0, st, rptr, ridx, fine, coarse, nc, zero);
 }
 
 __global__ __launch_bounds__ (B1_THREADS)
@@ -491,25 +575,26 @@
 }
 
 __global__ __launch_bounds__ (B1_THREADS)
-void gather_kernel (const int *__restrict__ perm, const double *__restrict__ in, double *__restrict__ out, int64_t n, int scatter)
+void gather_kernel (const int *__restrict__ perm, const double *__restrict__ in, double *__restrict__ out, int64_t n, int scatter, double *__restrict__ zero)
 {
    const int64_t stride = (int64_t) gridDim.x * B1_THREADS;
    for (int64_t i = (int64_t) blockIdx.x * B1_THREADS + threadIdx.x; i < n; i += stride) {
       if (scatter) out[perm[i]] = in[i];
       else out[i] = in[perm[i]];
-   }
-}
-
-void launch_gather (const int *perm, const double *in, double *out, int64_t n, hipStream_t st)
+      if (zero) zero[i] = 0.0;
+   }
+}
+
+void launch_gather (const int *perm, const double *in, double *out, int64_t n, hipStream_t st, double *zero)
 {
    if (n <= 0) return;
-   hipLaunchKernelGGL (gather_kernel, dim3 (red_grid (n) * 2), dim3 (B1_THREADS), 0, st, perm, in, out, n, 0);
+   hipLaunchKernelGGL (gather_kernel, dim3 (red_grid (n) * 2), dim3 (B1_THREADS), 0, st, perm, in, out, n, 0, zero);
 }
 
 void launch_scatter (const int *perm, const double *in, double *out, int64_t n, hipStream_t st)
 {
    if (n <= 0) return;
-   hipLaunchKernelGGL (gather_kernel, dim3 (red_grid (n) * 2), dim3 (B1_THREADS), 0, st, perm, in, out, n, 1);
+   hipLaunchKernelGGL (gather_kernel, dim3 (red_grid (n) * 2), dim3 (B1_THREADS), 0, st, perm, in, out, n, 1, (double *) nullptr);
 }
 
 __global__ __launch_bounds__ (B1_THREADS)
diff --git a/nk_ocn_tracer_jacobian_precond_amd/csrc/create.hip b/nk_ocn_tracer_jacobian_precond_amd/csrc/create.hip
--- a/nk_ocn_tracer_jacobian_precond_amd/csrc/create.hip
+++ b/nk_ocn_tracer_jacobian_precond_amd/csrc/create.hip
@@ -33,7 +33,13 @@
    for (const auto &v : vec)
       if (v.count && (rc = dev_alloc (s, v.p, v.count))) return rc;
    if ((rc = dev_alloc (s, &s->dint, 8))) return rc;
+   if ((rc = dev_alloc (s, &s->tickets, NKP_MAX_K / NKP_DOT_CHUNK + 4))) return rc;
+   HIPCHK (hipMemset (s->tickets, 0, (NKP_MAX_K / NKP_DOT_CHUNK + 4) * sizeof (unsigned)));
    HIPCHK (hipHostMalloc ((void **) &s->hpin, (m + 16) * sizeof (double), hipHostMallocDefault));
+   HIPCHK (hipHostMalloc ((void **) &s->hcol, (m + 4) * sizeof (double), hipHostMallocMapped | hipHostMallocCoherent));
+   memset (s->hcol, 0, (m + 4) * sizeof (double));
+   HIPCHK (hipHostGetDevicePointer ((void **) &s->hcol_dev, s->hcol, 0));
+   s->col_seq = 0;
    HIPCHK (hipMemset (s->dscal, 0, nscal * sizeof (double)));
    return NKP_OK;
 }
@@ -444,8 +450,9 @@
    s->stream = nullptr;
    s->own_stream = false;
    s->device_bytes = 0;
-   s->V = s->vcur = s->Z = s->w = s->r = s->x = s->b = s->t1 = s->t2 = s->p1 = s->p2 = s->eqtmp = s->partial = s->dscal = s->hpin = nullptr;
+   s->V = s->vcur = s->Z = s->w = s->r = s->x = s->b = s->t1 = s->t2 = s->p1 = s->p2 = s->eqtmp = s->partial = s->dscal = s->hpin = s->hcol = s->hcol_dev = nullptr;
    s->dint = nullptr;
+   s->tickets = nullptr;
    for (MlLevel &L : s->ml.lev) L.x = L.x2 = L.b = L.r = nullptr;
    int rc = NKP_OK;
    TRYHIP (hipStreamCreateWithFlags (&s->stream, hipStreamNonBlocking));
diff --git a/nk_ocn_tracer_jacobian_precond_amd/csrc/inspect.hip b/nk_ocn_tracer_jacobian_precond_amd/csrc/inspect.hip
--- a/nk_ocn_tracer_jacobian_precond_amd/csrc/inspect.hip
+++ b/nk_ocn_tracer_jacobian_precond_amd/csrc/inspect.hip
@@ -132,7 +132,7 @@
          HIPCHK (hipMemcpyAsync (s->V + (int64_t) j * s->ld, V + (int64_t) j * ld, (size_t) s->n * sizeof (double), hipMemcpyHostToDevice, s->stream));
    }
    HIPCHK (hipMemcpyAsync (s->w, w, (size_t) s->n * sizeof (double), hipMemcpyHostToDevice, s->stream));
-   launch_multi_dot (s->V, s->vf32, s->ld, k, s->w, s->n, s->partial, s->h_dev (), s->stream);
+   launch_multi_dot (s->V, s->vf32, s->ld, k, s->w, s->n, s->partial, s->h_dev (), s->stream, (s->tune.iter_fold & 2) && !s->dist.on ? s->tickets : nullptr);
    allreduce_dev (s, s->h_dev (), k + 1, 0);
    HIPCHK (hipMemcpyAsync (out, s->h_dev (), (size_t) (k + 1) * sizeof (double), hipMemcpyDeviceToHost, s->stream));
    HIPCHK (hipStreamSynchronize (s->stream));
diff --git a/nk_ocn_tracer_jacobian_precond_amd/csrc/krylov.hip b/nk_ocn_tracer_jacobian_precond_amd/csrc/krylov.hip
--- a/nk_ocn_tracer_jacobian_precond_amd/csrc/krylov.hip
+++ b/nk_ocn_tracer_jacobian_precond_amd/csrc/krylov.hip
@@ -84,9 +84,18 @@
    }
 }
 
-void arnoldi_orthogonalise (nkp_solver *s, int j)
+static bool folds_reductions (const nkp_solver *s) { return (s->tune.iter_fold & 2) && !s->opt.reorth && !s->dist.on && !s->vf32; }
+
+void arnoldi_orthogonalise (nkp_solver *s, int j, const ColumnMirror *mirror)
 {
    const int64_t ld = s->ld;
+   if (folds_reductions (s)) {
+      launch_multi_dot (s->V, 0, ld, j + 1, s->w, s->n, s->partial, s->h_dev (), s->stream, s->tickets);
+      const ColumnFinish fin = { s->update_ticket (), s->h_dev (), s->misc_dev () + 1, mirror ? *mirror : ColumnMirror () };
+      launch_update_w (s->V, 0, ld, j + 1, s->h_dev (), s->w, s->n, s->partial, s->misc_dev (), s->stream, &fin);
+      launch_scale_to (s->w, s->misc_dev () + 1, s->V + (int64_t) (j + 1) * ld, nullptr, s->n, s->stream);
+      return;
+   }
    launch_multi_dot (s->V, s->vf32, ld, j + 1, s->w, s->n, s->partial, s->h_dev (), s->stream);
    allreduce_dev (s, s->h_dev (), j + 2, 0);
    launch_update_w (s->V, s->vf32, ld, j + 1, s->h_dev (), s->w, s->n, s->partial, s->misc_dev (), s->stream);
@@ -95,21 +104,21 @@
       allreduce_dev (s, s->h2_dev (), j + 2, 0);
       launch_update_w (s->V, s->vf32, ld, j + 1, s->h2_dev (), s->w, s->n, s->partial, s->misc_dev (), s->stream);
       allreduce_dev (s, s->misc_dev (), 1, 0);
-      launch_finish_column (s->h_dev (), s->h2_dev (), j + 1, s->misc_dev (), s->misc_dev () + 1, s->stream);
+      launch_finish_column (s->h_dev (), s->h2_dev (), j + 1, s->misc_dev (), s->misc_dev () + 1, s->stream, mirror);
    } else if (s->dist.on && s->tune.dist_one_reduce) {
       launch_finish_column_pythagoras (s->h_dev (), j + 1, s->misc_dev () + 1, s->stream);
    } else {
       allreduce_dev (s, s->misc_dev (), 1, 0);
-      launch_finish_column (s->h_dev (), nullptr, j + 1, s->misc_dev (), s->misc_dev () + 1, s->stream);
+      launch_finish_column (s->h_dev (), nullptr, j + 1, s->misc_dev (), s->misc_dev () + 1, s->stream, mirror);
    }
    if (s->vf32) launch_scale_to (s->w, s->misc_dev () + 1, s->vcur, (float *) s->V + (int64_t) (j + 1) * ld, s->n, s->stream);
    else launch_scale_to (s->w, s->misc_dev () + 1, s->V + (int64_t) (j + 1) * ld, nullptr, s->n, s->stream);
 }
 
-void arnoldi_step_device (nkp_solver *s, int j)
+void arnoldi_step_device (nkp_solver *s, int j, const ColumnMirror *mirror)
 {
    arnoldi_apply (s, j);
-   arnoldi_orthogonalise (s, j);
+   arnoldi_orthogonalise (s, j, mirror);
 }
 
 int fg_begin (nkp_solver *s, FgmresState &F)
@@ -167,9 +176,9 @@
    return NKP_OK;
 }
 
-bool fg_post_step (nkp_solver *s, FgmresState &F)
-{
-   const bool ends = fg_column_step (F, s->hpin, s->opt.max_iters);
+bool fg_post_step (nkp_solver *s, FgmresState &F, const double *col)
+{
+   const bool ends = fg_column_step (F, col ? col : s->hpin, s->opt.max_iters);
    if (!F.breakdown_in_cycle) msg (s, 3, "fgmres: its = %d, est relres = %.3e\n", F.its, F.est / F.bnorm);
    return ends;
 }
@@ -195,15 +204,52 @@
    return NKP_OK;
 }
 
+static inline void cpu_pause ()
+{
+#if defined(__x86_64__) || defined(__i386__)
+   __builtin_ia32_pause ();
+#elif defined(__aarch64__)
+   __asm__ volatile ("yield");
+#endif
+}
+
+static int wait_for_column (nkp_solver *s, unsigned long long seq)
+{
+   const unsigned long long *word = s->hcol_seq_word ();
+   for (unsigned spin = 1;; spin++) {
+      if (__atomic_load_n (word, __ATOMIC_ACQUIRE) == seq) return NKP_OK;
+      if ((spin & 1023u) == 0) {
+         const hipError_t e = hipStreamQuery (s->stream);
+         if (e == hipSuccess) {
+            if (__atomic_load_n (word, __ATOMIC_ACQUIRE) == seq) return NKP_OK;
+            return fail (NKP_EDEVICE, "nkp_solve: the stream drained without the Hessenberg column of Arnoldi step %llu arriving (last seen %llu): %s",
+                         seq, __atomic_load_n (word, __ATOMIC_ACQUIRE), hipGetErrorString (hipGetLastError ()));
+         }
+         if (e != hipErrorNotReady) return fail (NKP_EDEVICE, "nkp_solve: hipStreamQuery failed while waiting for a Hessenberg column: %s", hipGetErrorString (e));
+      }
+      cpu_pause ();
+   }
+}
+
 static int fgmres (nkp_solver *s, int *iters_out, double *relres_out)
 {
    FgmresState F;
    int rc = fg_begin (s, F);
    if (rc) return rc;
+   const bool polls = (s->tune.iter_fold & 4) && !s->dist.on && s->hcol;
    while (!F.finished) {
       if ((rc = fg_restart (s, F))) return rc;
       if (F.finished) break;
-      for (;;) {
+      for (; polls;) {
+         ColumnMirror mirror;
+         mirror.col = s->hcol_dev;
+         mirror.seq_word = reinterpret_cast<unsigned long long *> (s->hcol_dev + (s->m + 3));
+         mirror.seq = ++s->col_seq;
+         arnoldi_step_device (s, F.j, &mirror);
+         if ((rc = wait_for_column (s, mirror.seq))) return rc;
+         if (fg_post_step (s, F, s->hcol)) break;
+      }
+      for (; !polls;) {
          arnoldi_step_device (s, F.j);
          HIPCHK (hipMemcpyAsync (s->hpin, s->h_dev (), (size_t) (F.j + 2) * sizeof (double), hipMemcpyDeviceToHost, s->stream));
          HIPCHK (hipStreamSynchronize (s->stream));
diff --git a/nk_ocn_tracer_jacobian_precond_amd/csrc/mlcycle.hip b/nk_ocn_tracer_jacobian_precond_amd/csrc/mlcycle.hip
--- a/nk_ocn_tracer_jacobian_precond_amd/csrc/mlcycle.hip
+++ b/nk_ocn_tracer_jacobian_precond_amd/csrc/mlcycle.hip
@@ -32,7 +32,14 @@
    for (int step = 0; step < 2; step++) gs_half (H, V, reverse ? 1 - step : step, fused, st);
 }
 
-static void ml_cycle (MlHierarchy &H, int l, hipStream_t st)
+static bool ml_zero_rides (const MlHierarchy &H, int l)
+{
+   if (!(H.tune->iter_fold & 1)) return false;
+   if (l == H.tail_from && H.coarse_inv && H.gamma_to <= H.gamma_from) return false;
+   return !(l == (int) H.lev.size () - 1 && H.coarse_inv);
+}
+
+static void ml_cycle (MlHierarchy &H, int l, hipStream_t st, bool x_zeroed)
 {
    MlLevel &V = H.lev[l];
    V.cur[0] = V.cur[1] = 0;
@@ -44,14 +51,14 @@
          return;
       }
       const int sweeps = H.tune->ml_coarsest_sweeps > 0 ? H.tune->ml_coarsest_sweeps : 30;
-      launch_fill (V.x, 0.0, V.n, st);
+      if (!x_zeroed) launch_fill (V.x, 0.0, V.n, st);
       column_solves (H, V, 0, V.b, V.x, 0, st);
       gs_half (H, V, 1, false, st);
       for (int s = 1; s < sweeps; s++) gs_sweep (H, V, s & 1, false, st);
       return;
    }
    const bool fused = ml_level_fused (H, V);
-   launch_fill (V.x, 0.0, V.n, st);
+   if (!x_zeroed) launch_fill (V.x, 0.0, V.n, st);
    if (fused) {
       if (V.wave_fused) column_solves (H, V, 0, V.b, V.x2, 0, st);
       else launch_colblock_apply_lanes (V.B, V.color_grp[0], V.color_grp[1], V.b, V.x2, 0, st);
@@ -68,8 +75,9 @@
    for (int g = 0; g < gamma; g++) {
       if (V.L.dg_val) launch_diag_residual (V.L, V.color_tile[0], V.color_tile[2], V.xnow (), V.b, V.r, st);
       else launch_csr_spmv (V.L, V.xnow (), V.r, V.b, 1, st);
-      launch_restrict_sum (V.rptr, V.ridx, V.r, C.b, V.nc, st);
-      ml_cycle (H, l + 1, st);
+      const bool rides = ml_zero_rides (H, l + 1) && C.n == V.nc;
+      launch_restrict_sum (V.rptr, V.ridx, V.r, C.b, V.nc, st, rides ? C.x : nullptr);
+      ml_cycle (H, l + 1, st, rides);
       launch_prolong_add (V.cmap, C.xnow (), V.xnow (), V.n, H.omega, st);
    }
    for (int s = 0; s < nu; s++) gs_sweep (H, V, true, fused, st);
@@ -78,8 +86,9 @@
 void ml_apply (MlHierarchy &H, const double *r, double *z, hipStream_t st)
 {
    MlLevel &V = H.lev[0];
-   launch_gather (H.perm0, r, V.b, V.n, st);
-   ml_cycle (H, 0, st);
+   const bool rides = ml_zero_rides (H, 0);
+   launch_gather (H.perm0, r, V.b, V.n, st, rides ? V.x : nullptr);
+   ml_cycle (H, 0, st, rides);
    launch_scatter (H.perm0, V.xnow (), z, V.n, st);
 }
 
diff --git a/nk_ocn_tracer_jacobian_precond_amd/csrc/nkp_dev.h b/nk_ocn_tracer_jacobian_precond_amd/csrc/nkp_dev.h
--- a/nk_ocn_tracer_jacobian_precond_amd/csrc/nkp_dev.h
+++ b/nk_ocn_tracer_jacobian_precond_amd/csrc/nkp_dev.h
@@ -238,13 +238,25 @@
 #define NKP_RED_BLOCKS 1024
 #define NKP_DOT_CHUNK 8
 
-void launch_multi_dot (const void *V, int v_f32, int64_t ld, int k, const double *w, int64_t n, double *partial, double *out, hipStream_t st);
-void launch_update_w (const void *V, int v_f32, int64_t ld, int k, const double *h, double *w, int64_t n, double *partial, double *out_nrm2, hipStream_t st);
+void launch_multi_dot (const void *V, int v_f32, int64_t ld, int k, const double *w, int64_t n, double *partial, double *out, hipStream_t st,
+                       unsigned *tickets = nullptr);
+struct ColumnMirror {
+   double *col = nullptr;
+   unsigned long long *seq_word = nullptr;
+   unsigned long long seq = 0;
+};
+struct ColumnFinish {
+   unsigned *ticket;
+   double *hcol, *inv;
+   ColumnMirror mirror;
+};
+void launch_update_w (const void *V, int v_f32, int64_t ld, int k, const double *h, double *w, int64_t n, double *partial, double *out_nrm2, hipStream_t st,
+                      const ColumnFinish *fin = nullptr);
 void launch_scale_to (const double *x, const double *alpha_dev, double *y, float *yf, int64_t n, hipStream_t st);
 void launch_axpy_multi (const double *Z, int64_t ld, int k, const double *c, double *x, int64_t n, hipStream_t st);
 void launch_dot (const double *x, const double *y, int64_t n, double *partial, double *out, hipStream_t st);
 void launch_berr (const double *r, const double *den, int64_t n, double *partial, double *out, hipStream_t st);
-void launch_finish_column (double *h, const double *h2, int k, const double *nrm2, double *inv, hipStream_t st);
+void launch_finish_column (double *h, const double *h2, int k, const double *nrm2, double *inv, hipStream_t st, const ColumnMirror *mirror = nullptr);
 void launch_finish_column_pythagoras (double *h, int k, double *inv, hipStream_t st);
 struct GsGroup {
    const double *V[NKP_BATCH_MAX];
@@ -261,9 +273,9 @@
 void launch_vmul (const double *x, const double *w, double *y, int64_t n, hipStream_t st);
 void launch_fill (double *y, double v, int64_t n, hipStream_t st);
 
-void launch_restrict_sum (const int *rptr, const int *ridx, const double *fine, double *coarse, int64_t nc, hipStream_t st);
+void launch_restrict_sum (const int *rptr, const int *ridx, const double *fine, double *coarse, int64_t nc, hipStream_t st, double *zero = nullptr);
 void launch_prolong_add (const int *cmap, const double *coarse, double *fine, int64_t nf, double omega, hipStream_t st);
-void launch_gather (const int *perm, const double *in, double *out, int64_t n, hipStream_t st);
+void launch_gather (const int *perm, const double *in, double *out, int64_t n, hipStream_t st, double *zero = nullptr);
 void launch_scatter (const int *perm, const double *in, double *out, int64_t n, hipStream_t st);
 void launch_dense_matvec (const double *Minv, const double *x, double *y, int n, hipStream_t st);
 void launch_dense_matvec_f32 (const float *Minv, int ld, const double *x, double *y, int n, hipStream_t st);
diff --git a/nk_ocn_tracer_jacobian_precond_amd/csrc/solver.hip b/nk_ocn_tracer_jacobian_precond_amd/csrc/solver.hip
--- a/nk_ocn_tracer_jacobian_precond_amd/csrc/solver.hip
+++ b/nk_ocn_tracer_jacobian_precond_amd/csrc/solver.hip
@@ -15,7 +15,7 @@
 {
    if (!s) return;
    if (s->borrowed) {
-      void *own[] = { s->V, s->vcur, s->Z, s->w, s->r, s->x, s->b, s->t1, s->t2, s->p1, s->p2, s->eqtmp, s->partial, s->dscal, s->dint };
+      void *own[] = { s->V, s->vcur, s->Z, s->w, s->r, s->x, s->b, s->t1, s->t2, s->p1, s->p2, s->eqtmp, s->partial, s->dscal, s->dint, s->tickets };
       for (void *p : own)
          if (p) (void) hipFree (p);
       for (MlLevel &L : s->ml.lev) {
@@ -26,6 +26,7 @@
       valgrad_release (s);
       valprod_release (s);
       if (s->hpin) (void) hipHostFree (s->hpin);
+      if (s->hcol) (void) hipHostFree (s->hcol);
       if (s->own_stream && s->stream) (void) hipStreamDestroy (s->stream);
       s->shared->clones--;
       delete s;
@@ -40,7 +41,7 @@
    for (double *p : { s->bvin, s->bz, s->bw })
       if (p) (void) hipFree (p);
    void *ptrs[] = { s->A.rowptr, s->A.colind, s->A.val, s->A.rowblk, s->A.codes, s->A.dict, s->A.dict_ptr, s->A.dg_ptr, s->A.dg_key, s->A.dg_voff, s->A.dg_vald, s->A.dg_tile, s->A.dg_gptr, s->A.dg_grp, s->B.blk_start, s->B.fac, s->B.grp_b0, s->B.grp_nb, s->B.grp_maxlen, s->B.grp_base, s->B.grp_row0, s->B.col_slot, s->B.fac_t, s->B.gs_rb_ptr, s->B.gs_rb, s->V, s->vcur, s->Z, s->w, s->r,
-                    s->x, s->b, s->t1, s->t2, s->p1, s->p2, s->partial, s->dscal, s->dint, s->rscale, s->rinv, s->eqtmp };
+                    s->x, s->b, s->t1, s->t2, s->p1, s->p2, s->partial, s->dscal, s->dint, s->tickets, s->rscale, s->rinv, s->eqtmp };
    for (void *p : ptrs)
       if (p) (void) hipFree (p);
    delete s->B.grp_cols;
@@ -62,6 +63,7 @@
    if (s->dist.ev_halo) (void) hipEventDestroy (s->dist.ev_halo);
    if (s->dist.comm_stream) (void) hipStreamDestroy (s->dist.comm_stream);
    if (s->hpin) (void) hipHostFree (s->hpin);
+   if (s->hcol) (void) hipHostFree (s->hcol);
    if (s->own_stream && s->stream) (void) hipStreamDestroy (s->stream);
    delete s;
 }
diff --git a/nk_ocn_tracer_jacobian_precond_amd/csrc/solver_impl.h b/nk_ocn_tracer_jacobian_precond_amd/csrc/solver_impl.h
--- a/nk_ocn_tracer_jacobian_precond_amd/csrc/solver_impl.h
+++ b/nk_ocn_tracer_jacobian_precond_amd/csrc/solver_impl.h
@@ -76,6 +76,11 @@
    double *dscal = nullptr;
    double *hpin = nullptr;
    int *dint = nullptr;
+   unsigned *tickets = nullptr;
+   double *hcol = nullptr, *hcol_dev = nullptr;
+   unsigned long long col_seq = 0;
+   unsigned *update_ticket () { return tickets + NKP_MAX_K / NKP_DOT_CHUNK; }
+   unsigned long long *hcol_seq_word () { return reinterpret_cast<unsigned long long *> (hcol + (m + 3)); }
    std::vector<nkp_solver *> batch_members;
    double *bvin = nullptr, *bz = nullptr, *bw = nullptr;
    int batch_K = 0;
@@ -227,11 +232,11 @@
 NKP_PRIVATE void apply_precond (nkp_solver *s, const double *rin, double *zout);
 NKP_PRIVATE void spmv_op (nkp_solver *s, const double *x, double *y, const double *b, int mode);
 NKP_PRIVATE void arnoldi_apply (nkp_solver *s, int j);
-NKP_PRIVATE void arnoldi_orthogonalise (nkp_solver *s, int j);
-NKP_PRIVATE void arnoldi_step_device (nkp_solver *s, int j);
+NKP_PRIVATE void arnoldi_orthogonalise (nkp_solver *s, int j, const ColumnMirror *mirror = nullptr);
+NKP_PRIVATE void arnoldi_step_device (nkp_solver *s, int j, const ColumnMirror *mirror = nullptr);
 NKP_PRIVATE int fg_begin (nkp_solver *s, FgmresState &F);
 NKP_PRIVATE int fg_restart (nkp_solver *s, FgmresState &F);
-NKP_PRIVATE bool fg_post_step (nkp_solver *s, FgmresState &F);
+NKP_PRIVATE bool fg_post_step (nkp_solver *s, FgmresState &F, const double *col = nullptr);
 NKP_PRIVATE int fg_end_cycle (nkp_solver *s, FgmresState &F);
 NKP_PRIVATE int backward_error (nkp_solver *s, double *berr);
 NKP_PRIVATE const char *batch_unsupported (const nkp_solver *s);
diff --git a/nk_ocn_tracer_jacobian_precond_amd/csrc/tuning.cpp b/nk_ocn_tracer_jacobian_precond_amd/csrc/tuning.cpp
--- a/nk_ocn_tracer_jacobian_precond_amd/csrc/tuning.cpp
+++ b/nk_ocn_tracer_jacobian_precond_amd/csrc/tuning.cpp
@@ -59,6 +59,7 @@
    t->rhs_batch = 1; t->batch_spmv_rows = 1; t->precond_steps = 0; t->equil = -1; t->dist_overlap = 1; t->dist_ras = 1; t->dist_one_reduce = 0; t->force_dist = 0; t->setup_threads = 0; t->plan_times = 0;
    t->ml_drop_intertracer = 0; t->ml_huge_from = -1; t->dist_ras_rings = 1; t->ml_diag = 32; t->spmv_diag = 32;
    t->ml_lane_fused = 50000;
+   t->iter_fold = 5;
 }
 
 const nkp_tuning &nkp_builtin_tuning ()
@@ -103,6 +104,7 @@
    ENV_INT ("NKP_ML_DIAG", ml_diag);
    ENV_INT ("NKP_SPMV_DIAG", spmv_diag);
    ENV_INT ("NKP_ML_LANE_FUSED", ml_lane_fused);
+   ENV_INT ("NKP_ITER_FOLD", iter_fold);
 #undef ENV_INT
 #undef ENV_POS
 #undef ENV_FLAG
diff --git a/nk_ocn_tracer_jacobian_precond_amd/solver.py b/nk_ocn_tracer_jacobian_precond_amd/solver.py
--- a/nk_ocn_tracer_jacobian_precond_amd/solver.py
+++ b/nk_ocn_tracer_jacobian_precond_amd/solver.py
@@ -52,6 +52,7 @@
         ("rhs_batch", C.c_int), ("precond_steps", C.c_int), ("equil", C.c_int), ("dist_overlap", C.c_int), ("dist_ras", C.c_int), ("force_dist", C.c_int),
         ("setup_threads", C.c_int), ("plan_times", C.c_int), ("ml_drop_intertracer", C.c_int), ("dist_one_reduce", C.c_int), ("ml_huge_from", C.c_int), ("col_ldsres_min", C.c_int), ("col_sort_groups", C.c_int), ("batch_spmv_rows", C.c_int),
         ("dist_ras_rings", C.c_int), ("ml_diag", C.c_int), ("spmv_diag", C.c_int), ("ml_lane_fused", C.c_int),
+        ("iter_fold", C.c_int),
     ]
 
 
```
